# GuanLab/seekmer

Hardware: AMD Instinct MI355X
Metric: paired reads/sec mapped+quantified (higher is better)
Workload: dtype u64+f64; 1 GPU; configs[1]: synthetic ~190k-tx index (stand-in for ENSEMBL GRCh38 cDNA), 10000000 2x100bp synthetic pairs per GPU, map+classes+EM to the reference stop rule; transcripts=190402, kmer_slots=134217728, units_per_gpu=10000000, read_len=100, paired=True, classes=851072, class_map_rows=4208693, parallelism=reads sharded x1, RCCL all-reduce f64[T] per EM step, rccl_ranks=0

## Files before the change

### include/seekmer_hip.h

```cpp
#ifndef SEEKMER_HIP_H
#define SEEKMER_HIP_H

#include <stddef.h>
#include <stdint.h>

#ifdef __cplusplus
extern "C" {
#endif

#define SKM_OK 0
#define SKM_ERR_ARG 1
#define SKM_ERR_HIP 2
#define SKM_ERR_NO_DEVICE 3
#define SKM_ERR_COLLISION 4
#define SKM_ERR_STATE 5
#define SKM_ERR_IO 6
#define SKM_ERR_UNDEFINED 7
#define SKM_ERR_COMM 8

#define SKM_KMER_SIZE 25
#define SKM_MAX_FRAGMENT_LENGTH 2000


const char *skm_last_error(void);
// ... 26 lines not shown
int skm_mapper_create(skm_index *index, skm_mapper **out);
int skm_mapper_destroy(skm_mapper *mapper);

int skm_mapper_map_batch(skm_mapper *mapper, const char *bases,
                         const int64_t *offsets, int64_t n_units, int paired);
int skm_mapper_map_batch_async(skm_mapper *mapper, const char *bases,
                               const int64_t *offsets, int64_t n_units, int paired,
                               int64_t first_unit);
int skm_mapper_map_batch_uniform_async(skm_mapper *mapper, const char *bases, int32_t read_len,
                                       int64_t n_units, int paired, int64_t first_unit);
int skm_mapper_sync(skm_mapper *mapper);
int skm_mapper_expect_units(skm_mapper *mapper, int64_t n_units);
#define SKM_PACKED_CUT (-1)
typedef struct skm_packed_reads {
    int32_t stream;
    int32_t code_words;
    int64_t first_read;
    int64_t n_reads;
    int64_t read_stride;
    int64_t uniform_len;
    const uint64_t *codes;
    const uint32_t *lengths;
    int64_t n_exceptions;
    const uint32_t *exception_reads;
    const uint32_t *exception_masks;
    const char *names;
    const int64_t *name_offsets;
} skm_packed_reads;
int skm_mapper_push_packed(skm_mapper *mapper, const skm_packed_reads *piece, int paired);
typedef int (*skm_packed_source)(void *context, skm_packed_reads *piece);
int skm_mapper_map_packed_source(skm_mapper *mapper, skm_packed_source next, void *context,
                                 int paired, int64_t *n_pieces);
int skm_mapper_map_batch_device(skm_mapper *mapper, const void *d_bases,
                                const void *d_offsets, int64_t n_units,
                                int paired, int32_t max_read_len);
int skm_mapper_last_batch(skm_mapper *mapper, int32_t *begin, int32_t *end,
                          int32_t *anchor_entry, int32_t *anchor_offset,
                          int32_t *counts, int32_t *entries,
                          int64_t cap_entries, int64_t *n_entries);
int skm_mapper_keep_spans(skm_mapper *mapper, int enable);
#define SKM_STRAND_NONE 0
#define SKM_STRAND_FR 1
#define SKM_STRAND_RF 2
int skm_mapper_set_strand(skm_mapper *mapper, int mode);
int skm_mapper_set_length_weights(skm_mapper *mapper, const double *p);
int skm_mapper_set_bias(skm_mapper *mapper, int enable);
int skm_mapper_bias_observed(skm_mapper *mapper, int64_t out[4096]);
int skm_mapper_summary(skm_mapper *mapper, int64_t summary[4]);
int skm_mapper_export(skm_mapper *mapper, int64_t *class_offsets,
                      int32_t *class_targets, int64_t *class_counts,
                      int64_t *first_seen, int64_t *fld);
int skm_mapper_merge(skm_mapper *mapper, int64_t n_classes,
                     const int64_t *class_offsets, const int32_t *class_targets,
                     const int64_t *class_counts, const int64_t *first_seen,
                     int64_t unaligned, const int64_t *fld);
typedef struct skm_device_table {
    int32_t device;
    int64_t n_classes, n_ids;
    const int64_t *class_start;
    const int64_t *class_len;
    const double *class_count;
    const uint64_t *first_seen;
    const int32_t *ids;
    int64_t unaligned, units, first_seen_bound;
    const uint64_t *fld;
} skm_device_table;
int skm_mapper_device_table(skm_mapper *mapper, skm_device_table *out);
int skm_mapper_merge_device(skm_mapper *mapper, const skm_device_table *table);
int skm_mapper_clear(skm_mapper *mapper);
int skm_mapper_reset(skm_mapper *mapper);
int skm_mapper_timing(skm_mapper *mapper, double stats[8]);
int skm_mapper_set_stats(skm_mapper *mapper, int enable);
int skm_mapper_access_stats(skm_mapper *mapper, int64_t out[48]);

typedef struct skm_sample_set skm_sample_set;
int skm_sample_set_create(skm_index *index, int paired, skm_sample_set **out);
int skm_sample_set_destroy(skm_sample_set *set);
int skm_sample_set_set_strand(skm_sample_set *set, int mode);
int skm_sample_set_set_length_weights(skm_sample_set *set, const double *p);
int skm_sample_set_add_packed(skm_sample_set *set, int64_t sample, int64_t first_unit,
                              const skm_packed_reads *mate1, const skm_packed_reads *mate2);
int skm_sample_set_add_batch(skm_sample_set *set, int64_t sample, int64_t first_unit,
                             const char *bases, const int64_t *offsets, int64_t n_units);
int skm_sample_set_sync(skm_sample_set *set);
int skm_sample_set_summary(skm_sample_set *set, int64_t cap_samples, int64_t *n_samples,
                           int64_t *summary);
int skm_sample_set_export(skm_sample_set *set, int64_t *sample_class_offsets,
                          int64_t *class_offsets, int32_t *class_targets, int64_t *class_counts,
                          int64_t *first_seen);
int skm_sample_set_histogram(skm_sample_set *set, int64_t *fld);
int skm_sample_set_keep_histograms(skm_sample_set *set, int enable);
int skm_sample_set_histograms(skm_sample_set *set, int64_t cap_samples, int64_t *fld);
int skm_sample_set_plan(int64_t n_segments, const int32_t *sample, const int64_t *n_units,
                        int64_t max_units, int64_t cap_entries, int64_t *n_entries,
                        int64_t *entry_global, int64_t *entry_local, int32_t *entry_sample);
int skm_sample_set_split(int64_t n_entries, const int64_t *entry_global, const int64_t *entry_local,
                         const int32_t *entry_sample, int64_t n_samples, int64_t n_classes,
                         const int64_t *first_seen, int32_t *class_sample, int64_t *class_local,
                         int64_t *order, int64_t *sample_class_offsets);

int skm_effective_lengths(int device, const int64_t *fld, const double *lengths,
                          int64_t n_tx, double *out);
int skm_effective_lengths_many(int device, int64_t n, const int64_t *fld, const double *lengths,
                               int64_t n_tx, double *out);
int skm_effective_lengths_weights(int device, int64_t n, const double *p, const double *lengths,
                                  int64_t n_tx, double *out);

int skm_bias_correct(skm_index *index, int strand, const int64_t *observed, const double *tpm, const double *eff,
                     int64_t n_tx, double *expected_out, double *b_out, double *eff_out);

typedef struct skm_quant skm_quant;
int skm_quant_create(int device, int64_t n_tx, int64_t n_classes,
                     const int64_t *class_offsets, const int32_t *class_targets,
                     const double *class_counts, skm_quant **out);
int skm_quant_create_from_mapper(skm_mapper *mapper, int64_t n_tx, skm_quant **out);
int skm_quant_destroy(skm_quant *quant);
int skm_quant_em(skm_quant *quant, double *x, const double *l, double rel_tol,
                 double x_floor, int64_t max_iters, int64_t fixed_iters,
                 int64_t *iters);
int skm_quant_bootstrap(skm_quant *quant, int64_t n_boot, uint64_t seed,
                        const double *x0, const double *l, double rel_tol,
                        double x_floor, int64_t max_iters, double *out,
                        int64_t *counts_out, int64_t *iters_out);
int skm_quant_bootstrap_tpm(skm_quant *quant, int64_t n_boot, uint64_t seed,
                            const double *x0, const double *l, double rel_tol,
                            double x_floor, int64_t max_iters, double *out,
                            int64_t *iters_out);
int skm_quant_bootstrap_share_tpm(skm_quant *quant, int64_t n_boot, int64_t first, int64_t step,
                                  uint64_t seed, const double *x0, const double *l, double rel_tol,
                                  double x_floor, int64_t max_iters, double *out,
                                  int64_t *iters_out);
int skm_quant_set_counts(skm_quant *quant, const double *class_counts);
int skm_quant_em_many(skm_quant *quant, int64_t n_sets, const double *counts, const double *x0,
                      const double *l, double rel_tol, double x_floor, int tpm, double *out,
                      int64_t *iters_out);
int skm_quant_em_blend(skm_quant *quant, int64_t n_cells, const int32_t *class_cell,
                       const double *weight, const double *cell_total, const double *x0,
                       const double *l, double rel_tol, double x_floor, int tpm, double *out,
                       int64_t *iters_out, double *counts_out);
int skm_quant_em_tables(int device, int64_t n_tx, int64_t n_tables, const int64_t *table_class_offsets,
                        const int64_t *class_offsets, const int32_t *class_targets,
                        const double *class_counts, const double *x0, const double *l, double rel_tol,
                        double x_floor, int64_t max_iters, int tpm, double *out, int64_t *iters);
int skm_set_quant_groups(int64_t n_tables, int64_t n_tx, const int64_t *table_classes,
                         const int64_t *table_ids, int64_t max_slots, int64_t *n_groups,
                         int64_t *group_first);
int skm_sample_set_quantify(skm_sample_set *set, const double *lengths, int64_t n_tx, double rel_tol,
                            double x_floor, int64_t max_iters, int64_t cap_samples,
                            int64_t *n_samples, double *tpm, double *effective_lengths,
                            int64_t *iters);
int skm_quant_components(skm_quant *quant, int64_t info[8], int32_t *tx_label, int32_t *tx_tile,
                         int32_t *class_tile);
int skm_quant_timing(skm_quant *quant, double timing[4]);

typedef struct skm_comm skm_comm;
int skm_comm_unique_id(void *id128);
int skm_comm_create(int device, const void *id128, int rank, int world, skm_comm **out);
int skm_comm_count(skm_comm *comm, int *count);
int skm_comm_destroy(skm_comm *comm);
int skm_mapper_exchange_tables(skm_mapper *send, int send_to, skm_mapper *recv, int recv_from, skm_comm *comm);
int skm_quant_set_comm(skm_quant *quant, skm_comm *comm);

int skm_quant_infer(skm_mapper *mapper, skm_comm *comm, const double *lengths, int64_t n_tx,
                    double rel_tol, double x_floor, int64_t max_iters,
                    double *tpm, double *effective_lengths, int64_t *iters);


typedef struct skm_built skm_built;
int skm_build_index(const char *pool, const int64_t *seq_offsets, int64_t n_seqs,
                    int n_threads, skm_built **out);
int skm_built_sizes(const skm_built *b, int64_t sizes[4]);
int skm_built_copy(const skm_built *b, void *kmers, void *contigs,
                   char *sequences, void *targets);
int skm_built_free(skm_built *b);

typedef struct skm_fastq skm_fastq;
int skm_fastq_open(const char *const *paths, int n_paths, int paired,
                   int64_t batch_units, skm_fastq **out);
int skm_fastq_set_allocator(skm_fastq *reader, void *(*alloc)(size_t), void (*release)(void *));
int skm_fastq_set_parallel(skm_fastq *reader, int n_threads, int *enabled);
int skm_fastq_set_shard(skm_fastq *reader, int rank, int world);
int skm_fastq_batch_index(const skm_fastq *reader, int64_t *index);
int skm_fastq_batch_read_length(const skm_fastq *reader, int64_t *read_len);
int skm_fastq_next(skm_fastq *reader, int64_t *n_units, const char **bases,
                   const int64_t **offsets, const char **names,
                   const int64_t **name_offsets);
typedef struct skm_fastq_slab skm_fastq_slab;
int skm_fastq_detach(skm_fastq *reader, skm_fastq_slab **slab);
int skm_fastq_recycle(skm_fastq *reader, skm_fastq_slab *slab);
int skm_fastq_close(skm_fastq *reader);

int skm_fastq_cache_bytes(int64_t bytes);
int skm_fastq_wait_unmapped(void);
typedef struct skm_fastq_prefault skm_fastq_prefault;
int skm_fastq_prefault_start(const char *const *paths, int n_paths, int n_threads, skm_fastq_prefault **out);
int skm_fastq_prefault_finish(skm_fastq_prefault *handle);

typedef struct skm_fastq_packed skm_fastq_packed;
int skm_fastq_packed_open(const char *const *paths, int n_paths, int paired, int n_threads,
                          int64_t chunk_bytes, int want_names, skm_fastq_packed **out);
int skm_fastq_packed_open_ranges(const char *const *paths, int n_paths, int paired, int n_threads,
                                 int64_t chunk_bytes, int want_names, const int64_t *begin,
                                 const int64_t *end, int64_t first_unit, skm_fastq_packed **out);
int skm_fastq_count_newlines(const char *path, int64_t chunk_bytes, int64_t first_chunk,
                             int64_t chunk_step, int n_threads, int64_t *counts, int64_t n_chunks,
                             int *last_line_open);
int skm_fastq_locate_line(const char *path, int64_t chunk_bytes, const int64_t *counts,
                          int64_t n_chunks, int64_t line, int64_t *byte_offset);
int skm_fastq_packed_set_allocator(skm_fastq_packed *reader, void *(*alloc)(size_t),
                                   void (*release)(void *));
int skm_fastq_packed_next(void *reader, skm_packed_reads *piece);
int skm_fastq_packed_stats(const skm_fastq_packed *reader, int64_t stats[8]);
int skm_fastq_packed_estimate(const skm_fastq_packed *reader, int64_t *units);
int skm_fastq_packed_close(skm_fastq_packed *reader);
int skm_pack_reads(const char *bases, const int64_t *offsets, int64_t n_reads, int32_t code_words,
                   uint64_t *codes, uint32_t *lengths, uint32_t *exception_reads,
                   uint32_t *exception_masks, int64_t cap_exceptions, int64_t *n_exceptions,
                   int variant);
int skm_pack_set_variant(int variant);

int skm_synth_transcriptome(uint64_t seed, int64_t n_genes, int64_t *n_tx,
                            char **pool, int64_t **offsets);
int skm_synth_free(void *p);
int skm_synth_reads(uint64_t seed, const char *pool, const int64_t *tx_offsets,
                    int64_t n_tx, int64_t first_unit, int64_t n_units,
                    int read_len, int paired, int n_threads, char *bases);

int skm_synth_fastq_write(const char *bases, int64_t n_units, int read_len, int paired,
                          int64_t first_unit, const char *path1, const char *path2,
                          int n_threads);

#ifdef __cplusplus
}
#endif
#endif
```

### seekmer_amd/_native.py

```python
import ctypes
import os

_HERE = os.path.dirname(os.path.abspath(__file__))
HIP_LIB_PATH = os.environ.get('SKM_HIP_LIB') or os.path.join(_HERE, 'libseekmer_hip.so')
HOST_LIB_PATH = os.path.join(_HERE, 'libseekmer_host.so')

SKM_OK = 0
SKM_ERR_ARG = 1
SKM_ERR_HIP = 2
SKM_ERR_NO_DEVICE = 3
SKM_ERR_COLLISION = 4
SKM_ERR_STATE = 5
SKM_ERR_IO = 6
SKM_ERR_UNDEFINED = 7
SKM_ERR_COMM = 8

SKM_STRAND_NONE = 0
SKM_STRAND_FR = 1
SKM_STRAND_RF = 2

c_void_pp = ctypes.POINTER(ctypes.c_void_p)
c_i64p = ctypes.POINTER(ctypes.c_int64)
c_i32p = ctypes.POINTER(ctypes.c_int32)
c_f64p = ctypes.POINTER(ctypes.c_double)
c_i64 = ctypes.c_int64
c_u32p = ctypes.POINTER(ctypes.c_uint32)
c_u64p = ctypes.POINTER(ctypes.c_uint64)


class PackedReads(ctypes.Structure):
    _fields_ = [('stream', ctypes.c_int32), ('code_words', ctypes.c_int32), ('first_read', ctypes.c_int64),
                ('n_reads', ctypes.c_int64), ('read_stride', ctypes.c_int64), ('uniform_len', ctypes.c_int64),
                ('codes', ctypes.c_void_p), ('lengths', ctypes.c_void_p), ('n_exceptions', ctypes.c_int64),
                ('exception_reads', ctypes.c_void_p), ('exception_masks', ctypes.c_void_p),
                ('names', ctypes.c_void_p), ('name_offsets', ctypes.c_void_p)]


class DeviceTable(ctypes.Structure):
    _fields_ = [('device', ctypes.c_int32), ('n_classes', ctypes.c_int64), ('n_ids', ctypes.c_int64),
                ('class_start', ctypes.c_void_p), ('class_len', ctypes.c_void_p), ('class_count', ctypes.c_void_p),
                ('first_seen', ctypes.c_void_p), ('ids', ctypes.c_void_p), ('unaligned', ctypes.c_int64),
                ('units', ctypes.c_int64), ('first_seen_bound', ctypes.c_int64), ('fld', ctypes.c_void_p)]


HIP_SYMBOLS = {
    'skm_last_error': (ctypes.c_char_p, []),
    'skm_device_count': (ctypes.c_int, [ctypes.POINTER(ctypes.c_int)]),
    'skm_device_malloc': (ctypes.c_int, [ctypes.c_int, c_i64, c_void_pp]),
    'skm_device_free': (ctypes.c_int, [ctypes.c_int, ctypes.c_void_p]),
    'skm_device_upload': (ctypes.c_int, [ctypes.c_int, ctypes.c_void_p, ctypes.c_void_p, c_i64]),
    'skm_device_download': (ctypes.c_int, [ctypes.c_int, ctypes.c_void_p, ctypes.c_void_p, c_i64]),
    'skm_device_synchronize': (ctypes.c_int, [ctypes.c_int]),
    'skm_device_gather_ceiling': (ctypes.c_int, [ctypes.c_int, c_i64, ctypes.c_int, ctypes.c_int,
                                                 ctypes.c_int, c_f64p]),
    'skm_pinned_alloc': (ctypes.c_void_p, [ctypes.c_size_t]),
    'skm_pinned_free': (None, [ctypes.c_void_p]),
    'skm_pinned_set_device': (ctypes.c_int, [ctypes.c_int]),
    'skm_index_create': (ctypes.c_int, [ctypes.c_void_p, c_i64, ctypes.c_void_p, c_i64,
                                        ctypes.c_void_p, c_i64, ctypes.c_void_p, c_i64,
                                        ctypes.c_int, c_void_pp]),
    'skm_index_destroy': (ctypes.c_int, [ctypes.c_void_p]),
    'skm_index_info': (ctypes.c_int, [ctypes.c_void_p, c_i64p]),
    'skm_index_layout': (ctypes.c_int, [ctypes.c_void_p, c_i64p]),
    'skm_index_build_transcripts': (ctypes.c_int, [ctypes.c_void_p, c_f64p, c_i64]),
    'skm_index_transcript_bases': (ctypes.c_int, [ctypes.c_void_p, ctypes.c_void_p, ctypes.c_void_p]),
    'skm_mapper_create': (ctypes.c_int, [ctypes.c_void_p, c_void_pp]),
    'skm_mapper_destroy': (ctypes.c_int, [ctypes.c_void_p]),
    'skm_mapper_map_batch': (ctypes.c_int, [ctypes.c_void_p, ctypes.c_void_p, c_i64p, c_i64,
                                            ctypes.c_int]),
    'skm_mapper_map_batch_async': (ctypes.c_int, [ctypes.c_void_p, ctypes.c_void_p, c_i64p, c_i64,
                                                  ctypes.c_int, c_i64]),
    'skm_mapper_map_batch_uniform_async': (ctypes.c_int, [ctypes.c_void_p, ctypes.c_void_p, ctypes.c_int32, c_i64,
                                                          ctypes.c_int, c_i64]),
    'skm_mapper_sync': (ctypes.c_int, [ctypes.c_void_p]),
    'skm_mapper_expect_units': (ctypes.c_int, [ctypes.c_void_p, c_i64]),
    'skm_mapper_push_packed': (ctypes.c_int, [ctypes.c_void_p, ctypes.POINTER(PackedReads), ctypes.c_int]),
    'skm_mapper_map_packed_source': (ctypes.c_int, [ctypes.c_void_p, ctypes.c_void_p, ctypes.c_void_p, ctypes.c_int,
                                                    c_i64p]),
    'skm_mapper_map_batch_device': (ctypes.c_int, [ctypes.c_void_p, ctypes.c_void_p,
                                                   ctypes.c_void_p, c_i64, ctypes.c_int,
                                                   ctypes.c_int32]),
    'skm_mapper_last_batch': (ctypes.c_int, [ctypes.c_void_p, c_i32p, c_i32p, c_i32p, c_i32p,
                                             c_i32p, c_i32p, c_i64, c_i64p]),
    'skm_mapper_keep_spans': (ctypes.c_int, [ctypes.c_void_p, ctypes.c_int]),
    'skm_mapper_set_strand': (ctypes.c_int, [ctypes.c_void_p, ctypes.c_int]),
    'skm_mapper_set_length_weights': (ctypes.c_int, [ctypes.c_void_p, c_f64p]),
    'skm_mapper_set_bias': (ctypes.c_int, [ctypes.c_void_p, ctypes.c_int]),
    'skm_mapper_bias_observed': (ctypes.c_int, [ctypes.c_void_p, c_i64p]),
    'skm_mapper_summary': (ctypes.c_int, [ctypes.c_void_p, c_i64p]),
    'skm_mapper_export': (ctypes.c_int, [ctypes.c_void_p, c_i64p, c_i32p, c_i64p, c_i64p, c_i64p]),
    'skm_mapper_merge': (ctypes.c_int, [ctypes.c_void_p, c_i64, c_i64p, c_i32p, c_i64p, c_i64p,
                                        c_i64, c_i64p]),
    'skm_mapper_device_table': (ctypes.c_int, [ctypes.c_void_p, ctypes.POINTER(DeviceTable)]),
    'skm_mapper_merge_device': (ctypes.c_int, [ctypes.c_void_p, ctypes.POINTER(DeviceTable)]),
    'skm_mapper_clear': (ctypes.c_int, [ctypes.c_void_p]),
    'skm_mapper_reset': (ctypes.c_int, [ctypes.c_void_p]),
    'skm_mapper_timing': (ctypes.c_int, [ctypes.c_void_p, c_f64p]),
    'skm_mapper_set_stats': (ctypes.c_int, [ctypes.c_void_p, ctypes.c_int]),
    'skm_mapper_access_stats': (ctypes.c_int, [ctypes.c_void_p, c_i64p]),
    'skm_effective_lengths': (ctypes.c_int, [ctypes.c_int, c_i64p, c_f64p, c_i64, c_f64p]),
    'skm_effective_lengths_many': (ctypes.c_int, [ctypes.c_int, c_i64, c_i64p, c_f64p, c_i64, c_f64p]),
    'skm_effective_lengths_weights': (ctypes.c_int, [ctypes.c_int, c_i64, c_f64p, c_f64p, c_i64, c_f64p]),
    'skm_bias_correct': (ctypes.c_int, [ctypes.c_void_p, ctypes.c_int, c_i64p, c_f64p, c_f64p, c_i64, c_f64p, c_f64p, c_f64p]),
    'skm_sample_set_create': (ctypes.c_int, [ctypes.c_void_p, ctypes.c_int, c_void_pp]),
    'skm_sample_set_destroy': (ctypes.c_int, [ctypes.c_void_p]),
    'skm_sample_set_set_strand': (ctypes.c_int, [ctypes.c_void_p, ctypes.c_int]),
    'skm_sample_set_set_length_weights': (ctypes.c_int, [ctypes.c_void_p, c_f64p]),
    'skm_sample_set_add_packed': (ctypes.c_int, [ctypes.c_void_p, c_i64, c_i64, ctypes.POINTER(PackedReads),
                                                 ctypes.POINTER(PackedReads)]),
    'skm_sample_set_add_batch': (ctypes.c_int, [ctypes.c_void_p, c_i64, c_i64, ctypes.c_void_p, c_i64p, c_i64]),
    'skm_sample_set_sync': (ctypes.c_int, [ctypes.c_void_p]),
    'skm_sample_set_summary': (ctypes.c_int, [ctypes.c_void_p, c_i64, c_i64p, c_i64p]),
    'skm_sample_set_export': (ctypes.c_int, [ctypes.c_void_p, c_i64p, c_i64p, c_i32p, c_i64p, c_i64p]),
    'skm_sample_set_histogram': (ctypes.c_int, [ctypes.c_void_p, c_i64p]),
    'skm_sample_set_keep_histograms': (ctypes.c_int, [ctypes.c_void_p, ctypes.c_int]),
    'skm_sample_set_histograms': (ctypes.c_int, [ctypes.c_void_p, c_i64, c_i64p]),
    'skm_sample_set_plan': (ctypes.c_int, [c_i64, c_i32p, c_i64p, c_i64, c_i64, c_i64p, c_i64p, c_i64p, c_i32p]),
    'skm_sample_set_split': (ctypes.c_int, [c_i64, c_i64p, c_i64p, c_i32p, c_i64, c_i64, c_i64p, c_i32p, c_i64p, c_i64p,
                                            c_i64p]),
    'skm_quant_create': (ctypes.c_int, [ctypes.c_int, c_i64, c_i64, c_i64p, c_i32p, c_f64p,
                                        c_void_pp]),
    'skm_quant_create_from_mapper': (ctypes.c_int, [ctypes.c_void_p, c_i64, c_void_pp]),
    'skm_quant_destroy': (ctypes.c_int, [ctypes.c_void_p]),
    'skm_quant_em': (ctypes.c_int, [ctypes.c_void_p, c_f64p, c_f64p, ctypes.c_double,
                                    ctypes.c_double, c_i64, c_i64, c_i64p]),
    'skm_quant_bootstrap': (ctypes.c_int, [ctypes.c_void_p, c_i64, ctypes.c_uint64, c_f64p,
                                           c_f64p, ctypes.c_double, ctypes.c_double, c_i64,
                                           c_f64p, c_i64p, c_i64p]),
    'skm_quant_bootstrap_tpm': (ctypes.c_int, [ctypes.c_void_p, c_i64, ctypes.c_uint64, c_f64p,
                                               c_f64p, ctypes.c_double, ctypes.c_double, c_i64,
                                               c_f64p, c_i64p]),
    'skm_quant_bootstrap_share_tpm': (ctypes.c_int, [ctypes.c_void_p, c_i64, c_i64, c_i64, ctypes.c_uint64, c_f64p,
                                                     c_f64p, ctypes.c_double, ctypes.c_double, c_i64,
                                                     c_f64p, c_i64p]),
    'skm_quant_set_counts': (ctypes.c_int, [ctypes.c_void_p, c_f64p]),
    'skm_quant_em_many': (ctypes.c_int, [ctypes.c_void_p, c_i64, c_f64p, c_f64p, c_f64p, ctypes.c_double,
                                         ctypes.c_double, ctypes.c_int, c_f64p, c_i64p]),
    'skm_quant_em_blend': (ctypes.c_int, [ctypes.c_void_p, c_i64, c_i32p, c_f64p, c_f64p, c_f64p, c_f64p,
                                          ctypes.c_double, ctypes.c_double, ctypes.c_int, c_f64p, c_i64p, c_f64p]),
    'skm_quant_em_tables': (ctypes.c_int, [ctypes.c_int, c_i64, c_i64, c_i64p, c_i64p, c_i32p, c_f64p, c_f64p, c_f64p,
                                           ctypes.c_double, ctypes.c_double, c_i64, ctypes.c_int, c_f64p, c_i64p]),
    'skm_set_quant_groups': (ctypes.c_int, [c_i64, c_i64, c_i64p, c_i64p, c_i64, c_i64p, c_i64p]),
    'skm_sample_set_quantify': (ctypes.c_int, [ctypes.c_void_p, c_f64p, c_i64, ctypes.c_double, ctypes.c_double, c_i64,
                                               c_i64, c_i64p, c_f64p, c_f64p, c_i64p]),
    'skm_quant_timing': (ctypes.c_int, [ctypes.c_void_p, c_f64p]),
    'skm_quant_components': (ctypes.c_int, [ctypes.c_void_p, c_i64p, c_i32p, c_i32p, c_i32p]),
    'skm_comm_unique_id': (ctypes.c_int, [ctypes.c_void_p]),
    'skm_comm_create': (ctypes.c_int, [ctypes.c_int, ctypes.c_void_p, ctypes.c_int, ctypes.c_int,
                                       c_void_pp]),
    'skm_comm_count': (ctypes.c_int, [ctypes.c_void_p, ctypes.POINTER(ctypes.c_int)]),
    'skm_comm_destroy': (ctypes.c_int, [ctypes.c_void_p]),
    'skm_mapper_exchange_tables': (ctypes.c_int, [ctypes.c_void_p, ctypes.c_int, ctypes.c_void_p, ctypes.c_int,
                                                  ctypes.c_void_p]),
    'skm_quant_set_comm': (ctypes.c_int, [ctypes.c_void_p, ctypes.c_void_p]),
    'skm_quant_infer': (ctypes.c_int, [ctypes.c_void_p, ctypes.c_void_p, c_f64p, c_i64, ctypes.c_double,
                                       ctypes.c_double, c_i64, c_f64p, c_f64p, c_i64p]),
}

HOST_SYMBOLS = {
    'skm_build_index': (ctypes.c_int, [ctypes.c_void_p, c_i64p, c_i64, ctypes.c_int, c_void_pp]),
    'skm_built_sizes': (ctypes.c_int, [ctypes.c_void_p, c_i64p]),
    'skm_built_copy': (ctypes.c_int, [ctypes.c_void_p, ctypes.c_void_p, ctypes.c_void_p,
                                      ctypes.c_void_p, ctypes.c_void_p]),
    'skm_built_free': (ctypes.c_int, [ctypes.c_void_p]),
    'skm_fastq_open': (ctypes.c_int, [ctypes.POINTER(ctypes.c_char_p), ctypes.c_int, ctypes.c_int,
                                      c_i64, c_void_pp]),
    'skm_fastq_set_allocator': (ctypes.c_int, [ctypes.c_void_p, ctypes.c_void_p, ctypes.c_void_p]),
    'skm_fastq_set_parallel': (ctypes.c_int, [ctypes.c_void_p, ctypes.c_int, ctypes.POINTER(ctypes.c_int)]),
    'skm_fastq_set_shard': (ctypes.c_int, [ctypes.c_void_p, ctypes.c_int, ctypes.c_int]),
    'skm_fastq_batch_read_length': (ctypes.c_int, [ctypes.c_void_p, c_i64p]),
    'skm_fastq_batch_index': (ctypes.c_int, [ctypes.c_void_p, c_i64p]),
    'skm_fastq_next': (ctypes.c_int, [ctypes.c_void_p, c_i64p, c_void_pp, c_void_pp, c_void_pp,
                                      c_void_pp]),
    'skm_fastq_detach': (ctypes.c_int, [ctypes.c_void_p, c_void_pp]),
    'skm_fastq_recycle': (ctypes.c_int, [ctypes.c_void_p, ctypes.c_void_p]),
    'skm_fastq_close': (ctypes.c_int, [ctypes.c_void_p]),
    'skm_fastq_cache_bytes': (ctypes.c_int, [c_i64]),
    'skm_fastq_wait_unmapped': (ctypes.c_int, []),
    'skm_fastq_packed_open': (ctypes.c_int, [ctypes.POINTER(ctypes.c_char_p), ctypes.c_int, ctypes.c_int,
                                             ctypes.c_int, c_i64, ctypes.c_int, c_void_pp]),
    'skm_fastq_packed_open_ranges': (ctypes.c_int, [ctypes.POINTER(ctypes.c_char_p), ctypes.c_int, ctypes.c_int,
                                                    ctypes.c_int, c_i64, ctypes.c_int, c_i64p, c_i64p, c_i64, c_void_pp]),
    'skm_fastq_count_newlines': (ctypes.c_int, [ctypes.c_char_p, c_i64, c_i64, c_i64, ctypes.c_int, c_i64p, c_i64,
                                                ctypes.POINTER(ctypes.c_int)]),
    'skm_fastq_locate_line': (ctypes.c_int, [ctypes.c_char_p, c_i64, c_i64p, c_i64, c_i64, c_i64p]),
    'skm_fastq_packed_set_allocator': (ctypes.c_int, [ctypes.c_void_p, ctypes.c_void_p, ctypes.c_void_p]),
    'skm_fastq_packed_next': (ctypes.c_int, [ctypes.c_void_p, ctypes.POINTER(PackedReads)]),
    'skm_fastq_packed_stats': (ctypes.c_int, [ctypes.c_void_p, c_i64p]),
    'skm_fastq_prefault_start': (ctypes.c_int, [ctypes.POINTER(ctypes.c_char_p), ctypes.c_int, ctypes.c_int, c_void_pp]),
    'skm_fastq_prefault_finish': (ctypes.c_int, [ctypes.c_void_p]),
    'skm_fastq_packed_estimate': (ctypes.c_int, [ctypes.c_void_p, c_i64p]),
    'skm_fastq_packed_close': (ctypes.c_int, [ctypes.c_void_p]),
    'skm_pack_reads': (ctypes.c_int, [ctypes.c_void_p, c_i64p, c_i64, ctypes.c_int32, ctypes.c_void_p,
                                      ctypes.c_void_p, ctypes.c_void_p, ctypes.c_void_p, c_i64, c_i64p,
                                      ctypes.c_int]),
    'skm_pack_set_variant': (ctypes.c_int, [ctypes.c_int]),
    'skm_synth_transcriptome': (ctypes.c_int, [ctypes.c_uint64, c_i64, c_i64p, c_void_pp,
                                               c_void_pp]),
    'skm_synth_free': (ctypes.c_int, [ctypes.c_void_p]),
    'skm_synth_fastq_write': (ctypes.c_int, [ctypes.c_void_p, c_i64, ctypes.c_int, ctypes.c_int, c_i64,
                                             ctypes.c_char_p, ctypes.c_char_p, ctypes.c_int]),
    'skm_synth_reads': (ctypes.c_int, [ctypes.c_uint64, ctypes.c_void_p, c_i64p, c_i64, c_i64,
                                       c_i64, ctypes.c_int, ctypes.c_int, ctypes.c_int,
                                       ctypes.c_void_p]),
}


class NativeError(RuntimeError):

    def __init__(self, code, message):
        super().__init__('seekmer_hip error %d: %s' % (code, message))
        self.code = code


def _bind(path, symbols):
    if not os.path.exists(path):
        raise ImportError(
            '%s is missing: build it with `python -c "import __graft_entry__ as g; g.build()"` '
            'or `make -C seekmer_amd/csrc` (there is no CPU fallback)' % path)
    lib = ctypes.CDLL(path, mode=ctypes.RTLD_GLOBAL)
    for name, (restype, argtypes) in symbols.items():
        fn = getattr(lib, name)
        fn.restype = restype
        fn.argtypes = argtypes
    return lib


_hip = None
_host = None


def hip():
    global _hip
    if _hip is None:
        _hip = _bind(HIP_LIB_PATH, HIP_SYMBOLS)
    return _hip


def host():
    global _host
    if _host is None:
        _host = _bind(HOST_LIB_PATH, HOST_SYMBOLS)
    return _host


def check(code):
    if code == SKM_OK:
        return
    message = hip().skm_last_error().decode(errors='replace')
    if code == SKM_ERR_ARG:
        raise ValueError(message)
    raise NativeError(code, message)


def check_host(code, what):
    if code == SKM_OK:
        return
    if code == SKM_ERR_ARG:
        raise ValueError('%s: bad argument' % what)
    if code == SKM_ERR_IO:
        raise OSError('%s: cannot open input' % what)
    raise NativeError(code, what)


def device_count():
    n = ctypes.c_int(0)
    code = hip().skm_device_count(ctypes.byref(n))
    if code == SKM_ERR_NO_DEVICE:
        return 0
    check(code)
    return n.value


def ptr(array, ctype):
    return array.ctypes.data_as(ctype)
```

### seekmer_amd/csrc/skm_abi.hip

```cpp
#include "../../include/seekmer_hip.h"
#include "skm_kernels.h"
#include "skm_pool.h"
#include "skm_bias.h"

#include <dlfcn.h>
#include <algorithm>
#include <cmath>
#include <cstdarg>
#include <cstdio>
#include <cstdlib>
#include <cstring>
#include <chrono>
#include <condition_variable>
#include <atomic>
#include <deque>
#include <functional>
#include <map>
#include <memory>
#include <unordered_map>
#include <mutex>
#include <thread>
#include <numeric>
#include <string>
#include <utility>
// ... 2783 lines not shown
    std::copy(log.local.begin(), log.local.end(), entry_local);
    std::copy(log.sample.begin(), log.sample.end(), entry_sample);
    return SKM_OK;
}

extern "C" int skm_sample_set_split(int64_t n_entries, const int64_t *entry_global, const int64_t *entry_local,
                                    const int32_t *entry_sample, int64_t n_samples, int64_t n_classes,
                                    const int64_t *first_seen, int32_t *class_sample, int64_t *class_local, int64_t *order,
                                    int64_t *sample_class_offsets)
{
    if (n_entries < 0 || n_samples < 0 || n_classes < 0 || !sample_class_offsets
            || (n_entries && (!entry_global || !entry_local || !entry_sample))
            || (n_classes && (!first_seen || !class_sample || !class_local || !order)))
        return fail(SKM_ERR_ARG, "bad argument");
    if (n_classes && (n_entries == 0 || entry_global[0] != 0)) return fail(SKM_ERR_ARG, "the log does not start at unit 0");
    for (int64_t i = 0; i < n_entries; ++i)
        if (entry_sample[i] < 0 || entry_sample[i] >= n_samples || (i && entry_global[i] <= entry_global[i - 1]))
            return fail(SKM_ERR_ARG, "bad log entry %lld", (long long)i);
    for (int64_t k = 0; k < n_classes; ++k) {
        if (first_seen[k] < 0) return fail(SKM_ERR_ARG, "negative first-seen unit");
        const int64_t e = segment_find(entry_global, n_entries, first_seen[k]);
        class_sample[k] = entry_sample[e];
        class_local[k] = entry_local[e] + (first_seen[k] - entry_global[e]);
    }
    set_split_order(n_samples, n_classes, class_sample, class_local, order, sample_class_offsets);
    return SKM_OK;
}

extern "C" int skm_effective_lengths(int device, const int64_t *fld, const double *lengths,
                                     int64_t n_tx, double *out)
{
    if (!fld || !lengths || !out || n_tx < 0) return fail(SKM_ERR_ARG, "bad argument");
    int n_dev = 0;
    SKM_TRY(skm_device_count(&n_dev));
    if (device < 0 || device >= n_dev) return fail(SKM_ERR_ARG, "device %d out of range", device);
    SKM_TRY(set_device(device));
    if (n_tx == 0) return SKM_OK;
    DBuf<unsigned long long> d_fld; DBuf<double> d_len, d_out;
    auto drain = on_exit([&]() { (void)hipStreamSynchronize(nullptr); });
    SKM_TRY(d_fld.ensure(MAX_FRAGMENT_LENGTH)); SKM_TRY(d_len.ensure(n_tx)); SKM_TRY(d_out.ensure(n_tx));
    HIP_TRY(hipMemcpy(d_fld.p, fld, MAX_FRAGMENT_LENGTH * 8, hipMemcpyHostToDevice));
    HIP_TRY(hipMemcpy(d_len.p, lengths, n_tx * 8, hipMemcpyHostToDevice));
    launch_effective_lengths(d_fld.p, d_len.p, n_tx, d_out.p, nullptr);
    HIP_TRY(hipGetLastError());
    HIP_TRY(hipMemcpy(out, d_out.p, n_tx * 8, hipMemcpyDeviceToHost));
    drain.dismiss();
    return SKM_OK;
}

namespace {

int64_t effective_lengths_group(int64_t n, int64_t n_tx)
{
    int64_t group = std::min<int64_t>((int64_t)(1LL << 25) / n_tx, (int64_t)(1LL << 25) / MAX_FRAGMENT_LENGTH);
    if (const char *v = getenv("SKM_EFF_MANY_GROUP"))
        if (atoll(v) > 0) group = std::min<int64_t>(group, atoll(v));
    return std::max<int64_t>(1, std::min(group, n));
}

}

extern "C" int skm_effective_lengths_many(int device, int64_t n, const int64_t *fld, const double *lengths,
                                          int64_t n_tx, double *out)
{
    if (n < 0 || n_tx < 0 || (n && (!fld || (n_tx && (!lengths || !out))))) return fail(SKM_ERR_ARG, "bad argument");
    int n_dev = 0;
    SKM_TRY(skm_device_count(&n_dev));
    if (device < 0 || device >= n_dev) return fail(SKM_ERR_ARG, "device %d out of range", device);
    SKM_TRY(set_device(device));
    if (n == 0 || n_tx == 0) return SKM_OK;
    const int64_t group = effective_lengths_group(n, n_tx);
    DBuf<unsigned long long> d_fld; DBuf<double> d_len, d_out;
    auto drain = on_exit([&]() { (void)hipStreamSynchronize(nullptr); });
    SKM_TRY(d_fld.ensure((size_t)group * MAX_FRAGMENT_LENGTH)); SKM_TRY(d_len.ensure(n_tx)); SKM_TRY(d_out.ensure((size_t)(group * n_tx)));
    HIP_TRY(hipMemcpy(d_len.p, lengths, n_tx * 8, hipMemcpyHostToDevice));
    for (int64_t first = 0; first < n; first += group) {
        const int64_t here = std::min(group, n - first);
        HIP_TRY(hipMemcpy(d_fld.p, fld + first * MAX_FRAGMENT_LENGTH, (size_t)here * MAX_FRAGMENT_LENGTH * 8, hipMemcpyHostToDevice));
        launch_effective_lengths_many(d_fld.p, here, d_len.p, n_tx, d_out.p, nullptr);
        HIP_TRY(hipGetLastError());
        HIP_TRY(hipMemcpy(out + first * n_tx, d_out.p, (size_t)(here * n_tx) * 8, hipMemcpyDeviceToHost));
    }
    drain.dismiss();
    return SKM_OK;
}

extern "C" int skm_effective_lengths_weights(int device, int64_t n, const double *p, const double *lengths,
                                             int64_t n_tx, double *out)
{
    if (n < 0 || n_tx < 0 || !p || !lengths || !out) return fail(SKM_ERR_ARG, "bad argument");
    if (!length_weights_valid(p, n * MAX_FRAGMENT_LENGTH))
        return fail(SKM_ERR_ARG, "a fragment-length weight is negative or not finite");
    int n_dev = 0;
    SKM_TRY(skm_device_count(&n_dev));
    if (device < 0 || device >= n_dev) return fail(SKM_ERR_ARG, "device %d out of range", device);
    SKM_TRY(set_device(device));
    if (n == 0 || n_tx == 0) return SKM_OK;
    const int64_t group = effective_lengths_group(n, n_tx);
    DBuf<double> d_p, d_len, d_out;
    auto drain = on_exit([&]() { (void)hipStreamSynchronize(nullptr); });
    SKM_TRY(d_p.ensure((size_t)group * MAX_FRAGMENT_LENGTH)); SKM_TRY(d_len.ensure(n_tx)); SKM_TRY(d_out.ensure((size_t)(group * n_tx)));
    HIP_TRY(hipMemcpy(d_len.p, lengths, n_tx * 8, hipMemcpyHostToDevice));
    for (int64_t first = 0; first < n; first += group) {
        const int64_t here = std::min(group, n - first);
        HIP_TRY(hipMemcpy(d_p.p, p + first * MAX_FRAGMENT_LENGTH, (size_t)here * MAX_FRAGMENT_LENGTH * 8, hipMemcpyHostToDevice));
        launch_effective_lengths_weights(d_p.p, here, d_len.p, n_tx, d_out.p, nullptr);
        HIP_TRY(hipGetLastError());
        HIP_TRY(hipMemcpy(out + first * n_tx, d_out.p, (size_t)(here * n_tx) * 8, hipMemcpyDeviceToHost));
    }
    drain.dismiss();
    return SKM_OK;
}

namespace {

bool em_components_enabled() { return getenv("SKM_EM_NO_COMPONENTS") == nullptr; }
bool em_tiles_possible(bool several_ranks)
{
    static const bool unfused = getenv("SKM_EM_UNFUSED") != nullptr;
    return !several_ranks && !unfused && em_components_enabled();
}

int quant_alloc(skm_quant *q, int device, int64_t n_tx, int64_t n_classes, int64_t n_ids, bool several_ranks = false)
{
    STALE_CHECK("quant_alloc entry");
    q->device = device;
    q->n_tx = n_tx;
    q->n_classes = n_classes;
    q->n_ids = n_ids;
    HIP_TRY(pool_stream_acquire(q->stream.out()));
    for (auto &e : q->ev) HIP_TRY(pool_event_acquire(e.out(), true));
    for (auto &e : q->chunk_ev) HIP_TRY(pool_event_acquire(e.out(), false));
    HIP_TRY(pool_pinned_acquire((void **)q->pinned.out()));
    const size_t C = (size_t)std::max<int64_t>(n_classes, 1), M = (size_t)std::max<int64_t>(n_ids, 1);
    const size_t T = (size_t)std::max<int64_t>(n_tx, 1);
    const size_t R = (size_t)quant_rows_upper_bound(n_tx, n_ids);
    SKM_TRY(q->cls_offset.ensure(C + 1));
    SKM_TRY(q->cls_count.ensure(C));
    SKM_TRY(q->inner.ensure(C));
    SKM_TRY(q->ids.ensure(M));
    SKM_TRY(q->perm.ensure(C));
    SKM_TRY(q->tx_cls.ensure(M));
    SKM_TRY(q->tx_row.ensure(T + 1));
    SKM_TRY(q->row_start.ensure(R + 1));
    SKM_TRY(q->row_tx.ensure(R));
    SKM_TRY(q->row_sum.ensure(R));
    SKM_TRY(q->eff_len.ensure(T));
    SKM_TRY(q->x0.ensure(T));
    SKM_TRY(q->x1.ensure(T));
    SKM_TRY(q->acc.ensure(T));
    SKM_TRY(q->ctl.ensure(16));
    SKM_TRY(q->part_max.ensure(EM_FINAL_BLOCKS));
    SKM_TRY(q->part_flags.ensure(EM_FINAL_BLOCKS));
    SKM_TRY(q->arrivals.ensure(T));
    HIP_TRY(hipMemsetAsync(q->arrivals.p, 0, T * sizeof(unsigned int), q->stream));
    if (em_tiles_possible(several_ranks)) {
        auto &t = q->tiles;
        SKM_TRY(t.tile_tx.ensure(T + 2)); SKM_TRY(t.tile_cls.ensure(T + 2));
        SKM_TRY(t.cls_pair.ensure(C + 1)); SKM_TRY(t.tx_pair.ensure(T + 1));
        SKM_TRY(t.tx_list.ensure(T)); SKM_TRY(t.cls_list.ensure(C));
        SKM_TRY(t.tx_label.ensure(T)); SKM_TRY(t.tx_tile.ensure(T)); SKM_TRY(t.cls_tile.ensure(C));
        SKM_TRY(t.cls_tx.ensure(M)); SKM_TRY(t.tx_cls.ensure(M));
    }
    STALE_CHECK("quant_alloc exit");
    return SKM_OK;
}

QuantBuild quant_build_view(skm_quant *q)
{
    QuantBuild b{};
    b.n_tx = q->n_tx;
    b.n_classes = q->n_classes;
    b.n_ids = q->n_ids;
    b.cls_offset = q->cls_offset.p;
    b.ids = q->ids.p;
    b.cls_count = q->cls_count.p;
    b.tx_cls = q->tx_cls.p;
    b.tx_row = q->tx_row.p;
    b.row_start = q->row_start.p;
    b.row_tx = q->row_tx.p;
    b.n_rows_cap = (int64_t)q->row_tx.cap;
    if (q->tiles.tile_tx.p) {
        auto &t = q->tiles;
        b.tile_tx = t.tile_tx.p; b.tile_cls = t.tile_cls.p;
        b.tx_list = t.tx_list.p; b.cls_list = t.cls_list.p;
        b.cls_pair = t.cls_pair.p; b.tx_pair = t.tx_pair.p;
        b.tile_cls_tx = t.cls_tx.p; b.tile_tx_cls = t.tx_cls.p;
        b.tx_label = t.tx_label.p; b.tx_tile = t.tx_tile.p; b.cls_tile = t.cls_tile.p;
    }
    return b;
}

int quant_finish_setup(skm_quant *q, const ClassTable *table, int64_t units_seen = -1)
{
    STALE_CHECK("quant_finish_setup");
    QuantBuild b = quant_build_view(q);
    b.first_seen_bound = units_seen > 0 ? units_seen : 0;
    const int64_t rows = quant_setup(table, b, q->perm.p, q->stream);
    if (rows < 0) return fail(SKM_ERR_HIP, "building the class views failed (%lld): %s", (long long)rows, quant_setup_failure());
    q->n_rows = rows;
    if (b.tile_tx) {
        q->tiles.built = true;
        q->tiles.n_tiles = b.tile_info[0];
        q->tiles.n_oversize = b.tile_info[1];
        if (q->tiles.n_tiles > 0) {
            SKM_TRY(q->tiles.step_max.ensure((size_t)(EM_CHUNK_MAX * q->tiles.n_tiles)));
            SKM_TRY(q->tiles.step_flags.ensure((size_t)(EM_CHUNK_MAX * q->tiles.n_tiles)));
            SKM_TRY(q->tiles.snap.ensure((size_t)EM_CHUNK_MAX * (size_t)q->n_tx));
        }
        if (q->tiles.n_oversize > 0 && q->tiles.n_tiles > 0) {
            auto &r = q->tiles.residual;
            int64_t counts[3] = {0, 0, 0};
            if (quant_residual_count(b, counts, q->stream))
                return fail(SKM_ERR_HIP, "sizing the residual EM problem failed: %s", quant_setup_failure());
            r.n_classes = counts[0]; r.n_ids = counts[1]; r.n_rows = counts[2];
            SKM_TRY(r.cls_offset.ensure((size_t)r.n_classes + 1)); SKM_TRY(r.ids.ensure((size_t)std::max<int64_t>(r.n_ids, 1)));
            SKM_TRY(r.cls_src.ensure((size_t)std::max<int64_t>(r.n_classes, 1)));
            SKM_TRY(r.row_start.ensure((size_t)r.n_rows + 1)); SKM_TRY(r.row_tx.ensure((size_t)std::max<int64_t>(r.n_rows, 1)));
            SKM_TRY(r.tx_cls.ensure((size_t)std::max<int64_t>(r.n_ids, 1))); SKM_TRY(r.tx_row.ensure((size_t)q->n_tx + 1));
            SKM_TRY(r.cls_count.ensure((size_t)std::max<int64_t>(r.n_classes, 1)));
            SKM_TRY(r.inner.ensure((size_t)std::max<int64_t>(r.n_classes, 1)));
            SKM_TRY(r.row_sum.ensure((size_t)std::max<int64_t>(r.n_rows, 1)));
            QuantResidual out{};
            out.n_classes = r.n_classes; out.n_ids = r.n_ids; out.n_rows = r.n_rows;
            out.cls_offset = r.cls_offset.p; out.ids = r.ids.p; out.cls_src = r.cls_src.p;
            out.row_start = r.row_start.p; out.row_tx = r.row_tx.p; out.tx_cls = r.tx_cls.p; out.tx_row = r.tx_row.p;
            if (quant_residual_build(b, out, q->stream))
                return fail(SKM_ERR_HIP, "building the residual EM problem failed: %s", quant_setup_failure());
            r.built = true;
        }
    }
    return SKM_OK;
}

struct Rccl {
    void *lib = nullptr;
    int (*GetUniqueId)(void *) = nullptr;
    int (*AllReduce)(const void *, void *, size_t, int, int, void *, hipStream_t) = nullptr;
    int (*CommDestroy)(void *) = nullptr;
    int (*CommCount)(void *, int *) = nullptr;
    const char *(*GetErrorString)(int) = nullptr;
    int (*Send)(const void *, size_t, int, int, void *, hipStream_t) = nullptr;
    int (*Recv)(void *, size_t, int, int, void *, hipStream_t) = nullptr;
    int (*GroupStart)() = nullptr;
    int (*GroupEnd)() = nullptr;
};
struct UniqueId { char internal[128]; };
typedef int (*comm_init_fn)(void **, int, UniqueId, int);
Rccl g_rccl;
comm_init_fn g_comm_init = nullptr;

int load_rccl()
{
    if (g_rccl.lib) return SKM_OK;
    void *lib = dlopen("librccl.so", RTLD_NOW | RTLD_GLOBAL);
    if (!lib) lib = dlopen("librccl.so.1", RTLD_NOW | RTLD_GLOBAL);
    if (!lib) lib = dlopen("/opt/rocm/lib/librccl.so", RTLD_NOW | RTLD_GLOBAL);
    if (!lib) return fail(SKM_ERR_COMM, "cannot load librccl.so: %s", dlerror());
    g_rccl.GetUniqueId = (int (*)(void *))dlsym(lib, "ncclGetUniqueId");
    g_comm_init = (comm_init_fn)dlsym(lib, "ncclCommInitRank");
    g_rccl.AllReduce = (int (*)(const void *, void *, size_t, int, int, void *, hipStream_t))dlsym(lib, "ncclAllReduce");
    g_rccl.CommDestroy = (int (*)(void *))dlsym(lib, "ncclCommDestroy");
    g_rccl.CommCount = (int (*)(void *, int *))dlsym(lib, "ncclCommCount");
    g_rccl.GetErrorString = (const char *(*)(int))dlsym(lib, "ncclGetErrorString");
    g_rccl.Send = (int (*)(const void *, size_t, int, int, void *, hipStream_t))dlsym(lib, "ncclSend");
    g_rccl.Recv = (int (*)(void *, size_t, int, int, void *, hipStream_t))dlsym(lib, "ncclRecv");
    g_rccl.GroupStart = (int (*)())dlsym(lib, "ncclGroupStart");
    g_rccl.GroupEnd = (int (*)())dlsym(lib, "ncclGroupEnd");
    if (!g_rccl.GetUniqueId || !g_comm_init || !g_rccl.AllReduce || !g_rccl.CommDestroy)
        return fail(SKM_ERR_COMM, "librccl.so lacks a required symbol");
    g_rccl.lib = lib;
    return SKM_OK;
}

constexpr int NCCL_FLOAT64 = 8, NCCL_UINT64 = 5, NCCL_INT32 = 2, NCCL_SUM = 0;

#define NCCL_TRY(call)                                                                   \
    do {                                                                                 \
        int r_ = (call);                                                                 \
        if (r_ != 0)                                                                     \
            return fail(SKM_ERR_COMM, "%s failed: %s", #call,                            \
                        g_rccl.GetErrorString ? g_rccl.GetErrorString(r_) : "?");        \
    } while (0)

EmProblem em_problem(skm_quant *q, double rel_tol, double x_floor, int64_t max_iters,
                     int64_t fixed_iters)
{
    EmProblem p{};
    p.n_tx = q->n_tx;
    p.n_classes = q->n_classes;
    p.n_rows = q->n_rows;
    p.cls_offset = q->cls_offset.p;
    p.ids = q->ids.p;
    p.cls_count = q->cls_count.p;
    p.inner = q->inner.p;
    p.row_start = q->row_start.p;
    p.row_tx = q->row_tx.p;
    p.tx_cls = q->tx_cls.p;
    p.tx_row = q->tx_row.p;
    p.row_sum = q->row_sum.p;
    p.eff_len = q->eff_len.p;
    p.x[0] = q->x0.p;
    p.x[1] = q->x1.p;
    p.acc = q->acc.p;
    p.n_total = q->n_total;
    p.rel_tol = rel_tol;
    p.x_floor = x_floor;
    p.ctl = q->ctl.p;
    p.part_max = q->part_max.p;
    p.part_flags = q->part_flags.p;
    p.max_iters = max_iters;
    p.fixed_iters = fixed_iters;
    static const bool unfused = getenv("SKM_EM_UNFUSED") != nullptr;
    p.fused = q->comm || unfused ? 0 : 1;
    p.arrivals = q->arrivals.p;
    return p;
}

bool em_uses_tiles(const skm_quant *q)
{
    return em_tiles_possible(q->comm != nullptr) && q->tiles.built && q->tiles.n_tiles > 0 &&
           (q->tiles.n_oversize == 0 || q->tiles.residual.built);
}
// ... 21 lines not shown
    auto &t = q->tiles;
    EmTiles tl{};
    tl.n_tiles = t.n_tiles;
    tl.tile_tx = t.tile_tx.p; tl.tile_cls = t.tile_cls.p;
    tl.tx_list = t.tx_list.p; tl.cls_list = t.cls_list.p;
    tl.cls_pair = t.cls_pair.p; tl.tx_pair = t.tx_pair.p;
    tl.cls_tx = t.cls_tx.p; tl.tx_cls = t.tx_cls.p;
    tl.step_max = t.step_max.p; tl.step_flags = t.step_flags.p;
    tl.snap = t.snap.p;
    const bool mixed = t.n_oversize > 0;
    EmProblem pr = p;
    if (mixed) {
        auto &r = t.residual;
        pr.n_classes = r.n_classes; pr.n_rows = r.n_rows;
        pr.cls_offset = r.cls_offset.p; pr.ids = r.ids.p; pr.cls_count = r.cls_count.p; pr.inner = r.inner.p;
        pr.row_start = r.row_start.p; pr.row_tx = r.row_tx.p; pr.tx_cls = r.tx_cls.p; pr.tx_row = r.tx_row.p;
        pr.row_sum = r.row_sum.p;
        pr.fused = 1;
        pr.extra_max = t.step_max.p; pr.extra_flags = t.step_flags.p; pr.n_extra = t.n_tiles;
        launch_permute_f64(q->cls_count.p, r.cls_src.p, r.n_classes, r.cls_count.p, false, q->stream);
    }
    int64_t queued = 0;
    auto enqueue_chunk = [&](int slot) -> int {
        launch_em_local_chunk(p, tl, queued == 0 ? q->x0.p : t.snap.p + (chunk - 1) * q->n_tx, (int)chunk, queued * chunk, q->stream);
        if (mixed) {
            pr.extra_first = queued * chunk;
            for (int64_t i = 0, k = queued * chunk; i < chunk; ++i, ++k) {
                launch_em_inner(pr, (int)(k & 1), i > 0, k, q->stream);
                launch_em_rows_finalize(pr, (int)(k & 1), q->stream);
            }
            launch_em_decide(pr, (queued + 1) * chunk, q->stream);
            q->launches += 2 * chunk + 2;
        } else {
            launch_em_local_decide(p, tl, queued * chunk, (int)chunk, q->stream);
            q->launches += 2;
        }
        ++queued;
        HIP_TRY(hipGetLastError());
        HIP_TRY(hipMemcpyAsync(q->pinned + 8 * slot, q->ctl.p, 8 * sizeof(unsigned long long),
                               hipMemcpyDeviceToHost, q->stream));
        return SKM_OK;
    };
    unsigned long long ctl[8] = {0};
    SKM_TRY(em_run_chunks_ahead(q, ctl, enqueue_chunk, em_ctl_done));
    if (ctl[CTL_TILE_FAULT]) {
        HIP_TRY(hipStreamSynchronize(q->stream));
        return fail(SKM_ERR_STATE, "a component tile exceeds the tile capacity: the class views of this handle are damaged");
    }
    const int64_t steps = (int64_t)ctl[CTL_ITERS];
    HIP_TRY(hipEventRecord(q->ev[1], q->stream));
    HIP_TRY(hipEventSynchronize(q->ev[1]));
    float ms = 0;
    HIP_TRY(hipEventElapsedTime(&ms, q->ev[0], q->ev[1]));
    q->t_em_ns += ms * 1e6;
    q->iters_total += (double)steps;
    if (iters_out) *iters_out = steps;
    if (ctl[CTL_UNDEFINED]) return fail(SKM_ERR_UNDEFINED, "no abundance above x_floor: numpy raises on max() of an empty selection");
    return SKM_OK;
}

int em_run(skm_quant *q, double rel_tol, double x_floor, int64_t max_iters, int64_t fixed_iters,
           int64_t *iters_out, int64_t chunk_steps = 16)
{
    double n_total = q->n_total;
    if (q->comm && !q->n_total_reduced) {
        HIP_TRY(hipMemcpyAsync(q->acc.p, &n_total, 8, hipMemcpyHostToDevice, q->stream));
        NCCL_TRY(g_rccl.AllReduce(q->acc.p, q->acc.p, 1, NCCL_FLOAT64, NCCL_SUM, q->comm, q->stream));
        HIP_TRY(hipMemcpyAsync(&n_total, q->acc.p, 8, hipMemcpyDeviceToHost, q->stream));
        HIP_TRY(hipStreamSynchronize(q->stream));
    }
    EmProblem p = em_problem(q, rel_tol, x_floor, max_iters, fixed_iters);
    p.n_total = n_total;
    HIP_TRY(hipMemsetAsync(q->ctl.p, 0, 16 * 8, q->stream));
    int64_t k = 0;
    const int64_t chunk = fixed_iters > 0 ? std::min<int64_t>(fixed_iters, chunk_steps) : chunk_steps;
    HIP_TRY(hipEventRecord(q->ev[0], q->stream));
    if (em_uses_tiles(q) && chunk <= EM_CHUNK_MAX) return em_run_tiles(q, p, chunk, iters_out);
    static const bool unfused_rows = getenv("SKM_EM_UNFUSED") != nullptr;
    auto enqueue_chunk = [&](int slot) -> int {
        for (int64_t i = 0; i < chunk; ++i, ++k) {
            launch_em_inner(p, (int)(k & 1), i > 0, k, q->stream);
            if (q->comm) {
                if (unfused_rows) {
                    launch_em_rows(p, (int)(k & 1), q->stream);
                    launch_em_rows_to_acc(p, q->stream);
                } else {
                    launch_em_rows_acc(p, (int)(k & 1), q->stream);
                }
                NCCL_TRY(g_rccl.AllReduce(q->acc.p, q->acc.p, (size_t)q->n_tx, NCCL_FLOAT64, NCCL_SUM,
                                          q->comm, q->stream));
                launch_em_finalize(p, (int)(k & 1), true, q->stream);
            } else if (p.fused) {
                launch_em_rows_finalize(p, (int)(k & 1), q->stream);
            } else {
                launch_em_rows(p, (int)(k & 1), q->stream);
                launch_em_finalize(p, (int)(k & 1), false, q->stream);
            }
            q->launches += q->comm ? (unfused_rows ? 4 : 3) : (p.fused ? 2 : 3);
        }
        launch_em_decide(p, k, q->stream);
        q->launches += 1;
        HIP_TRY(hipGetLastError());
        HIP_TRY(hipMemcpyAsync(q->pinned + 8 * slot, q->ctl.p, 8 * sizeof(unsigned long long),
                               hipMemcpyDeviceToHost, q->stream));
        return SKM_OK;
    };
    unsigned long long ctl[8] = {0};
    SKM_TRY(em_run_chunks_ahead(q, ctl, enqueue_chunk, em_ctl_done));
    HIP_TRY(hipStreamSynchronize(q->stream));
    HIP_TRY(hipEventRecord(q->ev[1], q->stream));
    HIP_TRY(hipEventSynchronize(q->ev[1]));
    float ms = 0;
    HIP_TRY(hipEventElapsedTime(&ms, q->ev[0], q->ev[1]));
    q->t_em_ns += ms * 1e6;
    q->iters_total += (double)ctl[CTL_ITERS];
    if (iters_out) *iters_out = (int64_t)ctl[CTL_ITERS];
    if (ctl[CTL_UNDEFINED]) return fail(SKM_ERR_UNDEFINED, "no abundance above x_floor: numpy raises on max() of an empty selection");
    return SKM_OK;
}

}

namespace {

double np_pairwise_host(const double *a, int64_t n)
{
    if (n < 8) {
        double r = 0.0;
        for (int64_t i = 0; i < n; ++i) r += a[i];
        return r;
    }
    if (n <= 128) {
        double r[8];
        for (int j = 0; j < 8; ++j) r[j] = a[j];
        int64_t i = 8;
        for (; i < n - (n % 8); i += 8)
            for (int j = 0; j < 8; ++j) r[j] += a[i + j];
        double res = ((r[0] + r[1]) + (r[2] + r[3])) + ((r[4] + r[5]) + (r[6] + r[7]));
        for (; i < n; ++i) res += a[i];
        return res;
    }
    int64_t n2 = n / 2;
    n2 -= n2 % 8;
    return np_pairwise_host(a, n2) + np_pairwise_host(a + n2, n - n2);
}

double np_sum_host(const double *a, int64_t n)
{
    double acc = 0.0;
    for (int64_t i = 0; i < n; i += 8192) acc += np_pairwise_host(a + i, std::min<int64_t>(8192, n - i));
    return acc;
}

}

extern "C" int skm_quant_create(int device, int64_t n_tx, int64_t n_classes,
                                const int64_t *class_offsets, const int32_t *class_targets,
                                const double *class_counts, skm_quant **out)
{
    if (!out || n_tx <= 0 || n_classes < 0) return fail(SKM_ERR_ARG, "bad argument");
    if (n_classes && (!class_offsets || !class_targets || !class_counts))
        return fail(SKM_ERR_ARG, "NULL class arrays");
    int n_dev = 0;
    SKM_TRY(skm_device_count(&n_dev));
    if (device < 0 || device >= n_dev) return fail(SKM_ERR_ARG, "device %d out of range", device);
    const int64_t M = n_classes ? class_offsets[n_classes] - class_offsets[0] : 0;
    for (int64_t c = 0; c < n_classes; ++c)
        if (class_offsets[c + 1] < class_offsets[c]) return fail(SKM_ERR_ARG, "class offsets are not monotone");
    const double total = np_sum_host(class_counts, n_classes);
    for (int64_t j = 0; j < M; ++j) {
        const int32_t t = class_targets[class_offsets[0] + j];
        if (t < 0 || t >= n_tx) return fail(SKM_ERR_ARG, "class target %d outside [0, n_tx)", t);
    }
    SKM_TRY(set_device(device));
    std::unique_ptr<skm_quant> q(new skm_quant());
    SKM_TRY(quant_alloc(q.get(), device, n_tx, n_classes, M));
    std::vector<int64_t> rebased(n_classes + 1, 0);
    for (int64_t c = 0; c <= n_classes && n_classes; ++c) rebased[c] = class_offsets[c] - class_offsets[0];
    HIP_TRY(hipMemcpy(q->cls_offset.p, rebased.data(), (n_classes + 1) * 8, hipMemcpyHostToDevice));
    if (n_classes) {
        HIP_TRY(hipMemcpy(q->cls_count.p, class_counts, n_classes * 8, hipMemcpyHostToDevice));
        if (M) HIP_TRY(hipMemcpy(q->ids.p, class_targets + class_offsets[0], M * 4, hipMemcpyHostToDevice));
    }
    q->n_total = total;
    SKM_TRY(quant_finish_setup(q.get(), nullptr));
    *out = q.release();
    return SKM_OK;
}

extern "C" int skm_quant_create_from_mapper(skm_mapper *m, int64_t n_tx, skm_quant **out)
{
    if (!m || !out || n_tx <= 0) return fail(SKM_ERR_ARG, "bad argument");
    SKM_TRY(wait_jobs(m, 0, false));
    std::lock_guard<std::mutex> lock(m->mu);
    SKM_TRY(set_device(m->ix->device));
    const int64_t C = m->host_classes, M = m->host_arena_used;
    std::unique_ptr<skm_quant> q(new skm_quant());
    SKM_TRY(quant_alloc(q.get(), m->ix->device, n_tx, C, M));
    unsigned long long ctr[4];
    HIP_TRY(hipMemcpy(ctr, m->counters.p, sizeof(ctr), hipMemcpyDeviceToHost));
    q->n_total = (double)(ctr[CTR_UNITS] - ctr[CTR_UNALIGNED]);
    SKM_TRY(quant_finish_setup(q.get(), &m->t, m->first_seen_bound));
    *out = q.release();
    return SKM_OK;
}

extern "C" int skm_quant_infer(skm_mapper *m, skm_comm *comm, const double *lengths, int64_t n_tx,
                               double rel_tol, double x_floor, int64_t max_iters,
                               double *tpm, double *effective_lengths, int64_t *iters)
{
    if (!m || !lengths || n_tx <= 0) return fail(SKM_ERR_ARG, "bad argument");
    SKM_TRY(wait_jobs(m, 0, false));
    std::lock_guard<std::mutex> lock(m->mu);
    if (comm && comm->device != m->ix->device)
        return fail(SKM_ERR_ARG, "communicator and mapper live on different GPUs");
    SKM_TRY(set_device(m->ix->device));
    const int64_t C = m->host_classes, M = m->host_arena_used;
    static const bool trace = getenv("SKM_TRACE_INFER") != nullptr;
    auto t_last = std::chrono::steady_clock::now();
    auto lap = [&](const char *what) {
        if (!trace) return;
        const auto now = std::chrono::steady_clock::now();
        fprintf(stderr, "[skm_quant_infer] %-12s %8.1f us\n", what,
                std::chrono::duration<double, std::micro>(now - t_last).count());
        t_last = now;
    };
    DBuf<unsigned long long> fld;
    DBuf<double> sums;
    std::unique_ptr<skm_quant> q(new skm_quant());
    SKM_TRY(quant_alloc(q.get(), m->ix->device, n_tx, C, M, comm != nullptr));
    if (comm) { q->comm = comm->comm; q->rank = comm->rank; q->world = comm->world; }
    lap("alloc");
    const int64_t n_blocks = (n_tx + 8191) / 8192;
    SKM_TRY(fld.ensure(MAX_FRAGMENT_LENGTH + 1));
    SKM_TRY(sums.ensure(n_blocks + 2));
    double *const total = sums.p + n_blocks;
    unsigned long long ctr[4] = {0, 0, m->host_unaligned, m->host_units};
    if (!m->host_totals_valid)
        HIP_TRY(hipMemcpy(ctr, m->counters.p, sizeof(ctr), hipMemcpyDeviceToHost));
    unsigned long long aligned = ctr[CTR_UNITS] - ctr[CTR_UNALIGNED];
    HIP_TRY(hipMemcpyAsync(fld.p, m->counters.p + CTR_FLD, MAX_FRAGMENT_LENGTH * 8,
                           hipMemcpyDeviceToDevice, q->stream));
    if (q->comm) {
        q->pinned[32] = aligned;
        HIP_TRY(hipMemcpyAsync(fld.p + MAX_FRAGMENT_LENGTH, q->pinned + 32, 8, hipMemcpyHostToDevice, q->stream));
        NCCL_TRY(g_rccl.AllReduce(fld.p, fld.p, MAX_FRAGMENT_LENGTH + 1, NCCL_UINT64, NCCL_SUM, q->comm,
                                  q->stream));
        HIP_TRY(hipMemcpyAsync(q->pinned + 32, fld.p + MAX_FRAGMENT_LENGTH, 8, hipMemcpyDeviceToHost, q->stream));
        HIP_TRY(hipStreamSynchronize(q->stream));
        aligned = q->pinned[32];
        q->n_total_reduced = true;
        if (const char *v = getenv("SKM_TEST_ALIGNED_GLOBAL")) aligned += strtoull(v, nullptr, 10);
    }
    q->n_total = (double)aligned;
    HIP_TRY(hipMemcpyAsync(q->x1.p, lengths, n_tx * 8, hipMemcpyHostToDevice, q->stream));
    if (m->use_length_weights)
        launch_effective_lengths_weights(m->length_weights.p, 1, q->x1.p, n_tx, q->eff_len.p, q->stream);
    else
        launch_effective_lengths(fld.p, q->x1.p, n_tx, q->eff_len.p, q->stream);
    if (q->comm ? aligned == 0 : C == 0) {
        if (effective_lengths)
            HIP_TRY(hipMemcpyAsync(effective_lengths, q->eff_len.p, n_tx * 8, hipMemcpyDeviceToHost, q->stream));
        HIP_TRY(hipStreamSynchronize(q->stream));
        if (tpm) memset(tpm, 0, (size_t)n_tx * 8);
        if (iters) *iters = 0;
        return SKM_OK;
    }
    launch_reciprocal(q->eff_len.p, n_tx, q->x0.p, q->stream);
    launch_np_sum(q->x0.p, n_tx, 1.0, sums.p, total, q->stream);
    launch_divide(q->x0.p, n_tx, total, false, 0.0, q->stream);
    lap("start vector");
    SKM_TRY(quant_finish_setup(q.get(), &m->t, m->first_seen_bound));
    lap("setup");
    if (trace) fprintf(stderr, "[skm_quant_infer] %lld classes, %lld transcripts, %lld rows\n", (long long)C, (long long)n_tx,
                       (long long)q->n_rows);
    int64_t it = 0;
    SKM_TRY(em_run(q.get(), rel_tol, x_floor, max_iters, 0, &it));
    lap("em");
    m->t_em_ns += q->t_em_ns;
    m->em_iters += (double)it;
    double *const x = (it & 1) ? q->x1.p : q->x0.p;
    launch_np_sum(x, n_tx, 1000000.0, sums.p, total, q->stream);
    launch_divide(x, n_tx, total + 1, true, 0.001, q->stream);
    launch_np_sum(x, n_tx, 1000000.0, sums.p, total, q->stream);
    launch_divide(x, n_tx, total + 1, false, 0.0, q->stream);
    HIP_TRY(hipGetLastError());
    if (tpm) HIP_TRY(hipMemcpyAsync(tpm, x, n_tx * 8, hipMemcpyDeviceToHost, q->stream));
    if (effective_lengths)
        HIP_TRY(hipMemcpyAsync(effective_lengths, q->eff_len.p, n_tx * 8, hipMemcpyDeviceToHost, q->stream));
    HIP_TRY(hipStreamSynchronize(q->stream));
    lap("tpm");
    if (iters) *iters = it;
    q.reset();
    lap("destroy");
    return SKM_OK;
}

extern "C" int skm_quant_destroy(skm_quant *q)
{
    if (!q) return SKM_OK;
    STALE_CHECK("quant_destroy entry");
    delete q;
    STALE_CHECK("quant_destroy exit");
    return SKM_OK;
}

extern "C" int skm_quant_em(skm_quant *q, double *x, const double *l, double rel_tol, double x_floor,
                            int64_t max_iters, int64_t fixed_iters, int64_t *iters)
{
    if (!q || !x || !l) return fail(SKM_ERR_ARG, "NULL argument");
    std::lock_guard<std::mutex> lock(q->mu);
    SKM_TRY(set_device(q->device));
    HIP_TRY(hipMemcpyAsync(q->x0.p, x, q->n_tx * 8, hipMemcpyHostToDevice, q->stream));
    HIP_TRY(hipMemcpyAsync(q->eff_len.p, l, q->n_tx * 8, hipMemcpyHostToDevice, q->stream));
    int64_t it = 0;
    SKM_TRY(em_run(q, rel_tol, x_floor, max_iters, fixed_iters, &it));
    HIP_TRY(hipMemcpy(x, (it & 1) ? q->x1.p : q->x0.p, q->n_tx * 8, hipMemcpyDeviceToHost));
    if (iters) *iters = it;
    return SKM_OK;
}

extern "C" int skm_quant_components(skm_quant *q, int64_t info[8], int32_t *tx_label, int32_t *tx_tile,
                                    int32_t *class_tile)
{
    if (!q || !info) return fail(SKM_ERR_ARG, "NULL argument");
    std::lock_guard<std::mutex> lock(q->mu);
    SKM_TRY(set_device(q->device));
    const auto &t = q->tiles;
    info[0] = t.built ? 1 : 0;
    info[1] = t.n_tiles;
    info[2] = t.n_oversize;
    info[3] = em_uses_tiles(q) ? 1 : 0;
    info[4] = EM_TILE_PAIRS; info[5] = EM_TILE_CLASSES; info[6] = EM_TILE_TX; info[7] = 0;
    if (!t.built) {
        if (tx_label || tx_tile || class_tile) return fail(SKM_ERR_ARG, "no component tiles were built for this handle");
        return SKM_OK;
    }
    HIP_TRY(hipStreamSynchronize(q->stream));
    if (tx_label) HIP_TRY(hipMemcpy(tx_label, t.tx_label.p, q->n_tx * 4, hipMemcpyDeviceToHost));
    if (tx_tile) HIP_TRY(hipMemcpy(tx_tile, t.tx_tile.p, q->n_tx * 4, hipMemcpyDeviceToHost));
    if (class_tile && q->n_classes) {
        std::vector<int32_t> tile(q->n_classes), perm(q->n_classes);
        HIP_TRY(hipMemcpy(tile.data(), t.cls_tile.p, q->n_classes * 4, hipMemcpyDeviceToHost));
        HIP_TRY(hipMemcpy(perm.data(), q->perm.p, q->n_classes * 4, hipMemcpyDeviceToHost));
        for (int64_t k = 0; k < q->n_classes; ++k) class_tile[perm[k]] = tile[k];
    }
    return SKM_OK;
}

extern "C" int skm_quant_set_counts(skm_quant *q, const double *class_counts)
{
    if (!q || (!class_counts && q->n_classes)) return fail(SKM_ERR_ARG, "NULL argument");
    std::lock_guard<std::mutex> lock(q->mu);
    SKM_TRY(set_device(q->device));
    const double total = np_sum_host(class_counts, q->n_classes);
    if (q->n_classes) {
        SKM_TRY(q->cls_count_saved.ensure(q->n_classes));
        HIP_TRY(hipMemcpyAsync(q->cls_count_saved.p, class_counts, q->n_classes * 8, hipMemcpyHostToDevice, q->stream));
        launch_permute_f64(q->cls_count_saved.p, q->perm.p, q->n_classes, q->cls_count.p, false, q->stream);
        HIP_TRY(hipGetLastError());
        HIP_TRY(hipStreamSynchronize(q->stream));
    }
    q->n_total = total;
    return SKM_OK;
}

namespace {

template <class Fill>
int em_group_run(skm_quant *q, int64_t n_problems, Fill &&fill, bool batched, int64_t slot_cap, const double *x0,
                 const double *l, double rel_tol, double x_floor, int64_t max_iters, double *out, int64_t *iters_out,
                 bool tpm)
{
    const int64_t C = q->n_classes, T = q->n_tx;
    skm_quant::Batch &w = q->batch;
    const int64_t group = std::max<int64_t>(1, std::min<int64_t>(n_problems, (int64_t)(1LL << 28) / T));
    const int64_t by_counts = std::max<int64_t>(1, (int64_t)((1LL << 31) / (8 * std::max<int64_t>(C, 1))));
    int64_t slots = batched ? std::max<int64_t>(1, std::min(group, by_counts)) : 1;
    if (slot_cap > 0) slots = std::min(slots, slot_cap);
    SKM_TRY(q->cls_count_saved.ensure(C));
    SKM_TRY(q->x_start.ensure(T));
    SKM_TRY(q->boot_out.ensure((size_t)(slots * T)));
    SKM_TRY(w.totals.ensure((size_t)(2 * slots)));
    HIP_TRY(hipMemcpyAsync(q->cls_count_saved.p, q->cls_count.p, C * 8, hipMemcpyDeviceToDevice, q->stream));
    HIP_TRY(hipMemcpyAsync(q->eff_len.p, l, T * 8, hipMemcpyHostToDevice, q->stream));
    HIP_TRY(hipMemcpyAsync(q->x_start.p, x0, T * 8, hipMemcpyHostToDevice, q->stream));
    const double saved_total = q->n_total;
    int rc = SKM_OK;
    DBuf<double> sums;
    auto restore = on_exit([&]() {
        (void)hipMemcpyAsync(q->cls_count.p, q->cls_count_saved.p, C * 8, hipMemcpyDeviceToDevice, q->stream);
        (void)hipStreamSynchronize(q->stream);
        q->n_total = saved_total;
    });
    auto problem_checked = [&](int64_t b, int64_t *it_out, double *dst) -> int {
        SKM_TRY(fill(b, (int64_t)1, q->cls_count.p, w.totals.p));
        HIP_TRY(hipGetLastError());
        double total = 0.0;
        HIP_TRY(hipMemcpyAsync(&total, w.totals.p, 8, hipMemcpyDeviceToHost, q->stream));
        HIP_TRY(hipMemcpyAsync(q->x0.p, q->x_start.p, T * 8, hipMemcpyDeviceToDevice, q->stream));
        HIP_TRY(hipStreamSynchronize(q->stream));
        q->n_total = total;
        SKM_TRY(em_run(q, rel_tol, x_floor, max_iters, 0, it_out, 8));
        HIP_TRY(hipMemcpyAsync(dst, (*it_out & 1) ? q->x1.p : q->x0.p, T * 8, hipMemcpyDeviceToDevice, q->stream));
        if (iters_out) iters_out[b] = *it_out;
        return SKM_OK;
    };
    auto scale = [&](double *results, int64_t count) -> int {
        if (!tpm || count <= 0) return SKM_OK;
        const int64_t n_blocks = (T + 8191) / 8192;
        SKM_TRY(sums.ensure((size_t)(count * (n_blocks + 2))));
        double *const totals = sums.p + count * n_blocks;
        launch_np_sum_many(results, T, count, T, 1000000.0, sums.p, totals, q->stream);
        launch_divide_many(results, T, count, T, totals + 1, true, 0.001, q->stream);
        launch_np_sum_many(results, T, count, T, 1000000.0, sums.p, totals, q->stream);
        launch_divide_many(results, T, count, T, totals + 1, false, 0.0, q->stream);
        HIP_TRY(hipGetLastError());
        return SKM_OK;
    };
    auto send_home = [&](int64_t first, int64_t count) -> int {
        if (count <= 0) return SKM_OK;
        SKM_TRY(scale(q->boot_out.p, count));
        HIP_TRY(hipMemcpyAsync(out + first * T, q->boot_out.p, (size_t)count * T * 8, hipMemcpyDeviceToHost, q->stream));
        HIP_TRY(hipStreamSynchronize(q->stream));
        return SKM_OK;
    };
    if (!batched) {
        for (int64_t b = 0; b < n_problems; ++b) {
            int64_t it = 0;
            SKM_TRY(problem_checked(b, &it, q->boot_out.p));
            SKM_TRY(send_home(b, 1));
        }
        return rc;
    }
    SKM_TRY(w.cls_count.ensure((size_t)C * EM_BATCH)); SKM_TRY(w.inner.ensure((size_t)C * EM_BATCH));
    SKM_TRY(w.row_sum.ensure((size_t)std::max<int64_t>(q->n_rows, 1) * EM_BATCH));
    SKM_TRY(w.x0.ensure((size_t)T * EM_BATCH)); SKM_TRY(w.x1.ensure((size_t)T * EM_BATCH));
// ... 767 lines not shown
```

### seekmer_amd/csrc/skm_em.hip

```cpp
#include "skm_em_core.h"

namespace skm {

__device__ bool em_evaluate(const EmProblem &p, int n_parts, int64_t steps_done, bool publish);

struct EmWholeTable {
    const EmProblem &p;
    __device__ __forceinline__ int64_t cls_first() const { return 0; }
    __device__ __forceinline__ int64_t cls_end() const { return p.n_classes; }
    __device__ __forceinline__ int64_t row_first() const { return 0; }
    __device__ __forceinline__ int64_t row_end() const { return p.n_rows; }
    __device__ __forceinline__ double n_total() const { return p.n_total; }
    __device__ __forceinline__ bool done() const { return p.ctl[CTL_DONE] != 0; }
    __device__ __forceinline__ bool judge(int eval_parts, int64_t steps_done) const { return em_evaluate(p, eval_parts, steps_done, true); }
    __device__ __forceinline__ int64_t part() const { return blockIdx.x; }
};

__global__ void __launch_bounds__(256)
em_inner_kernel(EmProblem p, int parity, int eval_parts, int64_t steps_done)
{
    em_inner_body(p, EmWholeTable{p}, parity, eval_parts > 0 && blockIdx.x == 0, eval_parts, steps_done, blockIdx.x * (int64_t)blockDim.x + threadIdx.x,
                  (int64_t)gridDim.x * blockDim.x);
}

// ... 453 lines not shown
    __syncthreads();
    const uint32_t mass = local_cum[n - 1];
    const unsigned int draws = tile_total[blockIdx.x];
    if (draws) {
        const int shift = MnGuide::shift_for(mass);
        mn_fill_guide(local_cum, n, shift, guide);
        __syncthreads();
        const uint32_t reject_below = (uint32_t)(0u - mass) % mass;
        MnStream rng(seed, stream_id, 1 + blockIdx.x);
        const unsigned int n_pairs = (unsigned int)(((unsigned long long)draws + 1) >> 1);
        for (unsigned int p = threadIdx.x; p < n_pairs; p += blockDim.x) {
            const uint64_t w = rng.words(p);
            const uint32_t r0 = mn_bounded((uint32_t)(w >> 32), mass, reject_below, rng, p, 0u);
            atomicAdd(&count[mn_find(local_cum, guide, shift, r0)], 1u);
            if (2ull * p + 1 < draws) {
                const uint32_t r1 = mn_bounded((uint32_t)w, mass, reject_below, rng, p, 1u);
                atomicAdd(&count[mn_find(local_cum, guide, shift, r1)], 1u);
            }
        }
        __syncthreads();
    }
    for (int i = threadIdx.x; i < n; i += blockDim.x) counts[(first_class + i) * stride] = (double)count[i];
}

__global__ void __launch_bounds__(256)
em_result_kernel(const unsigned long long *__restrict__ ctl, const double *__restrict__ x0,
                 const double *__restrict__ x1, int64_t n, double *__restrict__ out)
{
    const double *__restrict__ x = (ctl[CTL_ITERS] & 1ULL) ? x1 : x0;
    for (int64_t i = blockIdx.x * (int64_t)blockDim.x + threadIdx.x; i < n;
         i += (int64_t)gridDim.x * blockDim.x) out[i] = x[i];
}

__global__ void __launch_bounds__(256)
permute_f64_kernel(const double *__restrict__ x, const int32_t *__restrict__ perm, int64_t n,
                   double *__restrict__ y, bool scatter)
{
    for (int64_t i = blockIdx.x * (int64_t)blockDim.x + threadIdx.x; i < n;
         i += (int64_t)gridDim.x * blockDim.x) {
        if (scatter) y[perm[i]] = x[i]; else y[i] = x[perm[i]];
    }
}

__global__ void __launch_bounds__(256)
u64_to_double_kernel(const unsigned long long *__restrict__ in, int64_t n, double *__restrict__ out)
{
    for (int64_t i = blockIdx.x * (int64_t)blockDim.x + threadIdx.x; i < n;
         i += (int64_t)gridDim.x * blockDim.x)
        out[i] = (double)in[i];
}

__global__ void __launch_bounds__(256)
double_to_cum_u64_kernel(const double *__restrict__ in, int64_t n, unsigned long long *__restrict__ out)
{
    for (int64_t i = blockIdx.x * (int64_t)blockDim.x + threadIdx.x; i < n;
         i += (int64_t)gridDim.x * blockDim.x)
        out[i] = (unsigned long long)in[i];
}

__global__ void __launch_bounds__(256)
pack_sequences_kernel(const char *__restrict__ bases, int64_t n_bases, uint64_t *__restrict__ seq2,
                      int64_t n_words)
{
    for (int64_t w = blockIdx.x * (int64_t)blockDim.x + threadIdx.x; w < n_words;
         w += (int64_t)gridDim.x * blockDim.x) {
        uint64_t c = 0;
        const int64_t first = w * 32;
        for (int i = 0; i < 32 && first + i < n_bases; ++i)
            c |= (uint64_t)two_bit_encode((uint8_t)bases[first + i]) << (62 - 2 * i);
        seq2[w] = c;
    }
}

static inline unsigned grid_for(int64_t n, int64_t cap = 256 * 16)
{
    int64_t blocks = (n + 255) / 256;
    if (blocks < 1) blocks = 1;
    if (blocks > cap) blocks = cap;
    return (unsigned)blocks;
}

static inline unsigned chip_grid(int64_t work_items, int items_per_block)
{
    int64_t blocks = (work_items + items_per_block - 1) / items_per_block;
    if (blocks < 1) blocks = 1;
    if (blocks > 256 * 8) blocks = 256 * 8;
    return (unsigned)blocks;
}

int em_final_blocks(const EmProblem &p)
{
    int64_t blocks = p.fused ? (p.n_rows + 31) / 32 : (p.n_tx + 255) / 256;
    if (blocks < 1) blocks = 1;
    if (blocks > EM_FINAL_BLOCKS) blocks = EM_FINAL_BLOCKS;
    return (int)blocks;
}

void launch_em_inner(const EmProblem &p, int parity, bool judge_previous, int64_t steps_done, hipStream_t stream)
{
    hipLaunchKernelGGL(em_inner_kernel, dim3(chip_grid(p.n_classes, 256)), dim3(256), 0, stream, p, parity,
                       judge_previous ? em_final_blocks(p) : 0, steps_done);
}

void launch_em_decide(const EmProblem &p, int64_t steps_done, hipStream_t stream)
{
    hipLaunchKernelGGL(em_decide_kernel, dim3(1), dim3(256), 0, stream, p, em_final_blocks(p), steps_done);
}

void launch_em_rows(const EmProblem &p, int parity, hipStream_t stream)
{
    hipLaunchKernelGGL(em_rows_kernel, dim3(chip_grid(p.n_rows, 32)), dim3(256), 0, stream, p, parity);
}

void launch_em_rows_finalize(const EmProblem &p, int parity, hipStream_t stream)
{
    hipLaunchKernelGGL(em_rows_finalize_kernel<false>, dim3((unsigned)em_final_blocks(p)), dim3(256), 0, stream, p, parity);
}

void launch_em_rows_acc(const EmProblem &p, int parity, hipStream_t stream)
{
    EmProblem fused = p;
    fused.fused = 1;
    hipLaunchKernelGGL(em_rows_finalize_kernel<true>, dim3((unsigned)em_final_blocks(fused)), dim3(256), 0, stream, p, parity);
}

void launch_em_local_chunk(const EmProblem &p, const EmTiles &tiles, const double *x_in, int n_steps, int64_t first_step,
                           hipStream_t stream)
{
    if (tiles.n_tiles <= 0 || n_steps <= 0) return;
    hipLaunchKernelGGL(em_local_chunk_kernel, dim3((unsigned)tiles.n_tiles), dim3(256), 0, stream, p, tiles, x_in,
                       std::min(n_steps, EM_CHUNK_MAX), first_step);
}

void launch_em_local_decide(const EmProblem &p, const EmTiles &tiles, int64_t first_step, int n_steps, hipStream_t stream)
{
    hipLaunchKernelGGL(em_local_decide_kernel, dim3(1), dim3(64 * EM_CHUNK_MAX), 0, stream, p, tiles, first_step,
                       std::min(n_steps, EM_CHUNK_MAX));
}

void launch_em_rows_to_acc(const EmProblem &p, hipStream_t stream)
{
    hipLaunchKernelGGL(em_rows_to_acc_kernel, dim3(chip_grid(p.n_tx, 256)), dim3(256), 0, stream, p);
}

void launch_em_finalize(const EmProblem &p, int parity, bool from_acc, hipStream_t stream)
{
    const int blocks = em_final_blocks(p);
    if (from_acc)
        hipLaunchKernelGGL(em_finalize_kernel<true>, dim3((unsigned)blocks), dim3(256), 0, stream, p, parity);
    else
        hipLaunchKernelGGL(em_finalize_kernel<false>, dim3((unsigned)blocks), dim3(256), 0, stream, p, parity);
}

constexpr int NP_MAX_LEAVES = 160;

__device__ __forceinline__ double np_leaf_sum(const double *a, int n)
{
    if (n < 8) {
        double r = 0.0;
        for (int i = 0; i < n; ++i) r += a[i];
        return r;
    }
    double r[8];
    for (int j = 0; j < 8; ++j) r[j] = a[j];
    int i = 8;
    for (; i < n - (n % 8); i += 8)
        for (int j = 0; j < 8; ++j) r[j] += a[i + j];
    double res = ((r[0] + r[1]) + (r[2] + r[3])) + ((r[4] + r[5]) + (r[6] + r[7]));
    for (; i < n; ++i) res += a[i];
    return res;
}

template <int LEVELS>
__device__ __attribute__((noinline)) void np_list_leaves(int lo, int n, int *leaf_lo, int *leaf_n, int *count)
{
    if (n <= 128) {
        if (*count < NP_MAX_LEAVES) { leaf_lo[*count] = lo; leaf_n[*count] = n; }
        ++*count;
        return;
    }
    int n2 = n / 2;
    n2 -= n2 % 8;
    np_list_leaves<LEVELS - 1>(lo, n2, leaf_lo, leaf_n, count);
    np_list_leaves<LEVELS - 1>(lo + n2, n - n2, leaf_lo, leaf_n, count);
}
template <>
__device__ __attribute__((noinline)) void np_list_leaves<0>(int, int, int *, int *, int *count)
{
    *count = NP_MAX_LEAVES + 1;
}

template <int LEVELS>
__device__ __attribute__((noinline)) double np_combine(int n, const double *leaf_sum, int *next)
{
    if (n <= 128) return leaf_sum[(*next)++];
    int n2 = n / 2;
    n2 -= n2 % 8;
    const double left = np_combine<LEVELS - 1>(n2, leaf_sum, next);
    const double right = np_combine<LEVELS - 1>(n - n2, leaf_sum, next);
    return left + right;
}
template <>
__device__ __attribute__((noinline)) double np_combine<0>(int, const double *, int *) { return 0.0; }

__device__ __forceinline__ void np_sum_full_block(const double *__restrict__ a, double *__restrict__ out)
{
    __shared__ double leaf[64];
    const int l = threadIdx.x >> 3, j = threadIdx.x & 7;
    const double *p = a + l * 128 + j;
    double r = p[0];
#pragma unroll
    for (int i = 1; i < 16; ++i) r += p[8 * i];
    r += __shfl_xor(r, 1, 8);
    r += __shfl_xor(r, 2, 8);
    r += __shfl_xor(r, 4, 8);
    if (j == 0) leaf[l] = r;
    __syncthreads();
    if (threadIdx.x < 64) {
        double s = leaf[threadIdx.x];
        for (int d = 1; d < 64; d <<= 1) s += __shfl_xor(s, d, 64);
        if (threadIdx.x == 0) *out = s;
    }
}

__global__ void __launch_bounds__(512)
np_sum_blocks_kernel(const double *__restrict__ a, int64_t n, double *__restrict__ block_sums, int64_t stride)
{
    a += blockIdx.y * stride;
    block_sums += blockIdx.y * (int64_t)gridDim.x;
    const int64_t first = blockIdx.x * (int64_t)8192;
    const int len = (int)min((int64_t)8192, n - first);
    if (len == 8192) {
        np_sum_full_block(a + first, block_sums + blockIdx.x);
        return;
    }
    __shared__ double staged[8192];
    __shared__ int leaf_lo[NP_MAX_LEAVES], leaf_n[NP_MAX_LEAVES], n_leaves;
    __shared__ double leaf_sum[NP_MAX_LEAVES];
    for (int i = threadIdx.x; i < len; i += blockDim.x) staged[i] = a[first + i];
    if (threadIdx.x == 0) {
        int count = 0;
        np_list_leaves<8>(0, len, leaf_lo, leaf_n, &count);
        n_leaves = count;
    }
    __syncthreads();
    if (n_leaves > NP_MAX_LEAVES) {
        if (threadIdx.x == 0) {
            double r = 0.0;
            for (int i = 0; i < len; ++i) r += staged[i];
            block_sums[blockIdx.x] = r;
        }
        return;
    }
    if ((int)threadIdx.x < n_leaves)
        leaf_sum[threadIdx.x] = np_leaf_sum(staged + leaf_lo[threadIdx.x], leaf_n[threadIdx.x]);
    __syncthreads();
    if (threadIdx.x == 0) {
        int next = 0;
        block_sums[blockIdx.x] = np_combine<8>(len, leaf_sum, &next);
    }
}

__global__ void np_sum_final_kernel(const double *block_sums, int64_t n_blocks, double divisor, double *out)
{
    if (threadIdx.x != 0) return;
    block_sums += blockIdx.x * n_blocks;
    out += blockIdx.x * 2;
    double acc = 0.0;
    for (int64_t b = 0; b < n_blocks; ++b) acc += block_sums[b];
    out[0] = acc;
    out[1] = acc / divisor;
}

__global__ void __launch_bounds__(256)
reciprocal_kernel(const double *__restrict__ l, int64_t n, double *__restrict__ x)
{
    for (int64_t i = blockIdx.x * (int64_t)blockDim.x + threadIdx.x; i < n;
         i += (int64_t)gridDim.x * blockDim.x) x[i] = 1.0 / l[i];
}

__global__ void __launch_bounds__(256)
divide_kernel(double *__restrict__ x, int64_t n, const double *__restrict__ s, bool threshold, double floor,
              int64_t stride)
{
    x += blockIdx.y * stride;
    const double d = s[blockIdx.y * 2];
    for (int64_t i = blockIdx.x * (int64_t)blockDim.x + threadIdx.x; i < n;
         i += (int64_t)gridDim.x * blockDim.x) {
        double v = x[i] / d;
        if (threshold && v < floor) v = 0.0;
        x[i] = v;
    }
}

void launch_np_sum(const double *a, int64_t n, double divisor, double *block_sums, double *out,
                   hipStream_t stream)
{
    const int64_t n_blocks = (n + 8191) / 8192;
    if (n_blocks)
        hipLaunchKernelGGL(np_sum_blocks_kernel, dim3((unsigned)n_blocks), dim3(512), 0, stream,
                           a, n, block_sums, (int64_t)0);
    hipLaunchKernelGGL(np_sum_final_kernel, dim3(1), dim3(1), 0, stream, block_sums, n_blocks, divisor, out);
}

void launch_np_sum_many(const double *a, int64_t n, int64_t count, int64_t stride, double divisor,
                        double *block_sums, double *out, hipStream_t stream)
{
    const int64_t n_blocks = (n + 8191) / 8192;
    for (int64_t v0 = 0; v0 < count; v0 += 32768) {
        const unsigned here = (unsigned)std::min<int64_t>(32768, count - v0);
        if (n_blocks)
            hipLaunchKernelGGL(np_sum_blocks_kernel, dim3((unsigned)n_blocks, here), dim3(512), 0, stream,
                               a + v0 * stride, n, block_sums + v0 * n_blocks, stride);
        hipLaunchKernelGGL(np_sum_final_kernel, dim3(here), dim3(1), 0, stream, block_sums + v0 * n_blocks, n_blocks,
                           divisor, out + 2 * v0);
    }
}

void launch_reciprocal(const double *l, int64_t n, double *x, hipStream_t stream)
{
    hipLaunchKernelGGL(reciprocal_kernel, dim3(grid_for(n)), dim3(256), 0, stream, l, n, x);
}

void launch_divide(double *x, int64_t n, const double *s, bool threshold, double floor, hipStream_t stream)
{
    hipLaunchKernelGGL(divide_kernel, dim3(grid_for(n)), dim3(256), 0, stream, x, n, s, threshold, floor, (int64_t)0);
}

void launch_divide_many(double *x, int64_t n, int64_t count, int64_t stride, const double *s, bool threshold,
                        double floor, hipStream_t stream)
{
    for (int64_t v0 = 0; v0 < count; v0 += 32768) {
        const unsigned here = (unsigned)std::min<int64_t>(32768, count - v0);
        hipLaunchKernelGGL(divide_kernel, dim3(std::min<unsigned>(grid_for(n), 64u), here), dim3(256), 0, stream,
                           x + v0 * stride, n, s + 2 * v0, threshold, floor, stride);
    }
}

void launch_effective_lengths(const unsigned long long *fld, const double *lengths, int64_t n_tx,
                              double *out, hipStream_t stream)
{
    hipLaunchKernelGGL(effective_lengths_kernel, dim3(grid_for(n_tx)), dim3(256), 0, stream, fld,
                       lengths, n_tx, out);
}

static unsigned effective_lengths_blocks_per_row(int64_t n, int64_t n_tx)
{
    return std::min<unsigned>(grid_for(n_tx), n >= 64 ? 16u : 256u);
}

void launch_effective_lengths_many(const unsigned long long *fld, int64_t n, const double *lengths, int64_t n_tx,
                                   double *out, hipStream_t stream)
{
    hipLaunchKernelGGL(effective_lengths_kernel, dim3(effective_lengths_blocks_per_row(n, n_tx), (unsigned)n), dim3(256), 0,
                       stream, fld, lengths, n_tx, out);
}

void launch_effective_lengths_weights(const double *p, int64_t n, const double *lengths, int64_t n_tx, double *out,
                                      hipStream_t stream)
{
    const unsigned per_row = n == 1 ? (unsigned)grid_for(n_tx) : effective_lengths_blocks_per_row(n, n_tx);
    hipLaunchKernelGGL(effective_lengths_weights_kernel, dim3(per_row, (unsigned)n), dim3(256), 0, stream, p, lengths, n_tx, out);
}

int multinomial_tile(int64_t n_classes)
{
    int tile = 1;
    while ((n_classes + tile - 1) / tile > MN_TILES) tile <<= 1;
    return tile;
}

bool launch_multinomial(const unsigned long long *cum, int64_t n_classes, int64_t n_draws,
                        uint64_t seed, uint64_t stream_id, unsigned int *tile_total, double *counts,
                        int stride, hipStream_t stream)
{
    if (n_classes <= 0) return true;
    const int tile = multinomial_tile(n_classes);
    if (tile > MN_TILES || n_draws >= (1LL << 32)) return false;
    const int n_tiles = (int)((n_classes + tile - 1) / tile);
    (void)hipMemsetAsync(tile_total, 0, MN_TILES * sizeof(unsigned int), stream);
    if (n_draws > 0)
        hipLaunchKernelGGL(multinomial_tiles_kernel, dim3(512), dim3(1024), 0, stream, cum, n_classes, tile,
                           n_tiles, n_draws, seed, stream_id, tile_total);
    hipLaunchKernelGGL(multinomial_classes_kernel, dim3((unsigned)n_tiles), dim3(1024), 0, stream, cum, n_classes,
                       tile, tile_total, seed, stream_id, counts, stride);
    return true;
}

void launch_em_result(const unsigned long long *ctl, const double *x0, const double *x1, int64_t n, double *out,
                      hipStream_t stream)
{
    hipLaunchKernelGGL(em_result_kernel, dim3(grid_for(n)), dim3(256), 0, stream, ctl, x0, x1, n, out);
}

void launch_permute_f64(const double *x, const int32_t *perm, int64_t n, double *y, bool scatter,
                        hipStream_t stream)
{
    if (n <= 0) return;
    hipLaunchKernelGGL(permute_f64_kernel, dim3(grid_for(n)), dim3(256), 0, stream, x, perm, n, y, scatter);
}

void launch_u64_to_double(const unsigned long long *in, int64_t n, double *out, hipStream_t stream)
{
    if (n <= 0) return;
    hipLaunchKernelGGL(u64_to_double_kernel, dim3(grid_for(n)), dim3(256), 0, stream, in, n, out);
}

void launch_double_to_u64(const double *in, int64_t n, unsigned long long *out, hipStream_t stream)
{
    if (n <= 0) return;
    hipLaunchKernelGGL(double_to_cum_u64_kernel, dim3(grid_for(n)), dim3(256), 0, stream, in, n, out);
}

void launch_pack_sequences(const char *bases, int64_t n_bases, uint64_t *seq2, int64_t n_words,
                           hipStream_t stream)
{
    hipLaunchKernelGGL(pack_sequences_kernel, dim3(grid_for(n_words)), dim3(256), 0, stream, bases,
                       n_bases, seq2, n_words);
}

void warm_code_em()
{
    hipFuncAttributes attributes;
    (void)hipFuncGetAttributes(&attributes, reinterpret_cast<const void *>(&em_inner_kernel));
}

}

namespace skm {
__global__ void __launch_bounds__(256)
gather_probe_kernel(const uint4 *__restrict__ table, uint64_t slot_mask, int per_lane, int chain,
                    unsigned long long *sink)
{
    uint64_t x = mix64(blockIdx.x * (uint64_t)blockDim.x + threadIdx.x + 1);
    unsigned long long acc = 0;
    if (chain) {
        for (int i = 0; i < per_lane; ++i) {
            const uint4 v = table[x & slot_mask];
            acc += v.x;
            x = mix64(x + v.y + i);
        }
    } else {
        for (int i = 0; i < per_lane; i += 4) {
            const uint64_t a = mix64(x + i), b2 = mix64(x + i + 1), c = mix64(x + i + 2), d = mix64(x + i + 3);
            const uint4 v0 = table[a & slot_mask], v1 = table[b2 & slot_mask], v2 = table[c & slot_mask],
                        v3 = table[d & slot_mask];
            acc += v0.x + v1.x + v2.x + v3.x;
        }
    }
    if (acc == 0x123456789ULL) *sink = acc;
}

void launch_gather_probe(const void *table, uint64_t n_slots, int blocks, int per_lane, int chain,
                         unsigned long long *sink, hipStream_t stream)
{
    hipLaunchKernelGGL(gather_probe_kernel, dim3(blocks), dim3(256), 0, stream, (const uint4 *)table,
                       n_slots - 1, per_lane, chain, sink);
}
}
```

### seekmer_amd/csrc/skm_kernels.h

```cpp
#pragma once
#include "skm_device.h"

namespace skm {

struct MapBatch {
    const uint32_t *records;
    int64_t n_units;
    int32_t words_per_read;
    int32_t record_words;
    int32_t paired;
    int32_t *workspace;
    int32_t *rec_unit;
    uint64_t *rec_key;
    unsigned long long *rec_tuple;
    int32_t keep_spans;
    int32_t *unit_begin, *unit_end;
    Coord *unit_anchor;
    int32_t *unit_entries;
    int64_t ids_capacity;
    unsigned long long *ids_cursor;
    unsigned long long *fld;
    unsigned long long *stats;
    int32_t vote[8];
};
// ... 132 lines not shown
    const int64_t *tx_row;
    double *row_sum;
    const double *eff_len;
    double *x[2];
    double *acc;
    double n_total;
    double rel_tol, x_floor;
    unsigned long long *ctl;
    double *part_max;
    unsigned int *part_flags;
    int64_t max_iters, fixed_iters;
    int fused;
    unsigned int *arrivals;
    const double *extra_max;
    const unsigned int *extra_flags;
    int64_t n_extra, extra_first;
};
enum { CTL_DONE = 0, CTL_ITERS = 1, CTL_UNDEFINED = 3, CTL_TILE_FAULT = 4 };
#ifndef SKM_EM_FINAL_BLOCKS
#define SKM_EM_FINAL_BLOCKS 2048
#endif
constexpr int EM_FINAL_BLOCKS = SKM_EM_FINAL_BLOCKS;
void launch_em_inner(const EmProblem &p, int parity, bool judge_previous, int64_t steps_done, hipStream_t stream);
void launch_em_decide(const EmProblem &p, int64_t steps_done, hipStream_t stream);
void launch_em_rows(const EmProblem &p, int parity, hipStream_t stream);
void launch_em_rows_finalize(const EmProblem &p, int parity, hipStream_t stream);
void launch_em_rows_acc(const EmProblem &p, int parity, hipStream_t stream);
void launch_em_rows_to_acc(const EmProblem &p, hipStream_t stream);
void launch_em_finalize(const EmProblem &p, int parity, bool from_acc, hipStream_t stream);
void launch_em_result(const unsigned long long *ctl, const double *x0, const double *x1, int64_t n, double *out,
                      hipStream_t stream);

constexpr int EM_TILE_PAIRS = 2048, EM_TILE_CLASSES = 512, EM_TILE_TX = 128;
#ifndef SKM_EM_TILE_SEGMENT
#define SKM_EM_TILE_SEGMENT 128
#endif
constexpr int EM_TILE_SEGMENT = SKM_EM_TILE_SEGMENT;
constexpr int EM_CHUNK_MAX = 16;
constexpr int EM_TILE_CLASS_BATCH = 4;
struct EmTiles {
    int64_t n_tiles;
    const int64_t *tile_tx;
    const int64_t *tile_cls;
    const int32_t *tx_list;
    const int32_t *cls_list;
    const int64_t *cls_pair;
    const int64_t *tx_pair;
    const uint16_t *cls_tx;
    const uint16_t *tx_cls;
    double *step_max;
    unsigned int *step_flags;
    double *snap;
};
void launch_em_local_chunk(const EmProblem &p, const EmTiles &tiles, const double *x_in, int n_steps, int64_t first_step,
                           hipStream_t stream);
void launch_em_local_decide(const EmProblem &p, const EmTiles &tiles, int64_t first_step, int n_steps, hipStream_t stream);

constexpr int EM_BATCH = 8;
struct EmBatchProblem {
    int64_t n_tx, n_classes, n_rows;
    const int64_t *cls_offset;
    const int32_t *ids;
    const int64_t *row_start;
    const int32_t *row_tx;
    const int32_t *tx_cls;
    const int64_t *tx_row;
    const double *eff_len;
    const double *cls_count;
    double *inner;
    double *row_sum;
    double *x[2];
    double *place_total;
    double rel_tol, x_floor;
    unsigned long long *ctl;
    double *part_max;
    unsigned int *part_flags;
    int managed;
    unsigned long long *mgr;
    int64_t *iters_out;
    int fused;
    unsigned int *arrivals;
};
enum { BCTL_ALL_DONE = 0, BCTL_LAST_STEP = 1, BCTL_DONE = 8, BCTL_ITERS = 16, BCTL_UNDEFINED = 24 };
enum { MGR_NEXT = 0, MGR_COUNT = 1, MGR_FINISHED = 2, MGR_UNDEFINED = 3, MGR_REP = 8, MGR_SINCE = 16, MGR_TAKE = 24,
       MGR_PUT = 32 };
void launch_em_batch_manage_init(const EmBatchProblem &p, unsigned long long *mgr, unsigned long long *host_pinned64,
                                 int64_t n_reps, const double *counts_all, const double *totals, const double *x_start,
                                 double *out_all, hipStream_t stream);
void launch_em_batch_manage(const EmBatchProblem &p, unsigned long long *mgr, const double *counts_all, const double *totals,
                            const double *x_start, double *out_all, int64_t *iters_out, int64_t step, bool planned,
                            hipStream_t stream);
void launch_em_batch_step(const EmBatchProblem &p, int64_t step, hipStream_t stream);
void launch_em_batch_decide(const EmBatchProblem &p, int64_t steps_done, hipStream_t stream);
void launch_em_batch_take(const double *x, int64_t n_tx, int r, double *out, hipStream_t stream);
void launch_em_batch_ctl(unsigned long long *ctl, unsigned int idle, hipStream_t stream);
void launch_blend_counts(const double *own, const int32_t *class_cell, const double *weight, const double *cell_total,
                         int64_t n_cells, int64_t first, int64_t n_rows, int64_t n_classes, double *rows, hipStream_t stream);
void launch_permute_rows_f64(const double *x, const int32_t *perm, int64_t n, int64_t n_rows, double *y, hipStream_t stream);
struct EmSetSlot {
    int64_t cls_first, cls_end;
    int64_t row_first, row_end;
    double n_total;
    unsigned long long done;
    unsigned long long iters;
    unsigned long long undefined;
};
struct EmSetProblem {
    const int64_t *cls_offset;
    const int32_t *ids;
    const double *cls_count;
    double *inner;
    const int64_t *row_start;
    const int32_t *row_tx;
    const int32_t *tx_cls;
    const int64_t *tx_row;
    double *row_sum;
    const double *eff_len;
    double *x[2];
    double rel_tol, x_floor;
    int64_t max_iters;
    EmSetSlot *slots;
    int n_slots;
    int n_parts;
    double *part_max;
    unsigned int *part_flags;
    unsigned int *arrivals;
};
int em_set_parts(int64_t largest_rows);
void launch_em_set_step(const EmSetProblem &p, int64_t largest_classes, int64_t step, bool judge_previous, hipStream_t stream);
void launch_em_set_decide(const EmSetProblem &p, int64_t steps_done, unsigned long long *running, hipStream_t stream);
void launch_em_set_result(const EmSetSlot *slots, int n_slots, const double *x0, const double *x1, int64_t n_tx, double *out,
                          hipStream_t stream);
void launch_stack_tuples(const int64_t *src, const int64_t *dst, const int32_t *add, int64_t n_classes, const int32_t *arena,
                         int32_t *ids, hipStream_t stream);
void launch_repeat_row(double *x, int64_t n_tx, int64_t n, hipStream_t stream);

struct QuantBuild {
    int64_t n_tx, n_classes, n_ids;
    int64_t *cls_offset;
    int32_t *ids;
    double *cls_count;
    int32_t *tx_cls;
    int64_t *tx_row;
    int64_t *row_start;
    int32_t *row_tx;
    int64_t n_rows_cap;
    int64_t first_seen_bound;
    int64_t *tile_tx, *tile_cls;
    int32_t *tx_list, *cls_list;
    int64_t *cls_pair, *tx_pair;
    uint16_t *tile_cls_tx, *tile_tx_cls;
    int32_t *tx_label, *tx_tile, *cls_tile;
    int64_t tile_info[2];
};
int64_t quant_setup(const ClassTable *table, QuantBuild &q, int32_t *perm, hipStream_t stream);
struct QuantResidual {
    int64_t n_classes, n_ids, n_rows;
    int64_t *cls_offset;
    int32_t *ids;
    int32_t *cls_src;
    int64_t *row_start;
    int32_t *row_tx;
    int32_t *tx_cls;
    int64_t *tx_row;
};
int quant_residual_count(const QuantBuild &q, int64_t counts[3], hipStream_t stream);
int quant_residual_build(const QuantBuild &q, QuantResidual &r, hipStream_t stream);
void launch_permute_f64(const double *x, const int32_t *perm, int64_t n, double *y, bool scatter,
                        hipStream_t stream);
const char *quant_setup_failure();
int64_t quant_rows_upper_bound(int64_t n_tx, int64_t n_ids);

void launch_np_sum(const double *a, int64_t n, double divisor, double *block_sums, double *out,
                   hipStream_t stream);
void launch_np_sum_many(const double *a, int64_t n, int64_t count, int64_t stride, double divisor,
                        double *block_sums, double *out, hipStream_t stream);
void launch_reciprocal(const double *l, int64_t n, double *x, hipStream_t stream);
void launch_divide(double *x, int64_t n, const double *s, bool threshold, double floor, hipStream_t stream);
void launch_divide_many(double *x, int64_t n, int64_t count, int64_t stride, const double *s, bool threshold,
                        double floor, hipStream_t stream);
void launch_effective_lengths(const unsigned long long *fld, const double *lengths, int64_t n_tx,
                              double *out, hipStream_t stream);
void launch_effective_lengths_many(const unsigned long long *fld, int64_t n, const double *lengths, int64_t n_tx,
                                   double *out, hipStream_t stream);
void launch_effective_lengths_weights(const double *p, int64_t n, const double *lengths, int64_t n_tx, double *out,
                                      hipStream_t stream);
bool launch_multinomial(const unsigned long long *cum, int64_t n_classes, int64_t n_draws,
                        uint64_t seed, uint64_t stream_id, unsigned int *tile_total, double *counts,
                        int stride, hipStream_t stream);
void launch_u64_to_double(const unsigned long long *in, int64_t n, double *out, hipStream_t stream);
void launch_double_to_u64(const double *in, int64_t n, unsigned long long *out, hipStream_t stream);

void warm_code_map();
void warm_code_classes();
void warm_code_em();
void warm_code_em_batch();
void warm_code_em_set();
void warm_code_quant_setup();

}
```

### seekmer_amd/csrc/skm_quant_setup.hip

```cpp
#include "skm_kernels.h"
#include "skm_pool.h"

#include <algorithm>
#include <cstdio>
#include <vector>

namespace skm {

namespace {

struct Scratch {
    hipStream_t stream;
    std::vector<void *> held;
    explicit Scratch(hipStream_t s) : stream(s) {}
    template <class T>
    T *alloc(size_t n)
    {
        void *p = nullptr;
        if (pool_alloc(&p, std::max<size_t>(n, 1) * sizeof(T)) != hipSuccess) return nullptr;
        held.push_back(p);
        return static_cast<T *>(p);
    }
    ~Scratch()
    {
        (void)hipStreamSynchronize(stream);
        for (void *p : held) pool_free(p);
    }
};
thread_local char g_setup_failure[160] = "";
#define QB_ALLOC(var, type, n) type *var = scratch.alloc<type>(n); \
    if (!var) { snprintf(g_setup_failure, sizeof(g_setup_failure), "no memory for %s", #var); return -1; }

#define QB_TRY(call) do { const hipError_t qb_e = (call); if (qb_e != hipSuccess) { \
    snprintf(g_setup_failure, sizeof(g_setup_failure), "%s: %s", #call, hipGetErrorString(qb_e)); return -1; } } while (0)

__global__ void __launch_bounds__(256)
iota_kernel(int32_t *out, int64_t n)
{
    for (int64_t i = blockIdx.x * (int64_t)blockDim.x + threadIdx.x; i < n;
         i += (int64_t)gridDim.x * blockDim.x) out[i] = (int32_t)i;
}

__global__ void __launch_bounds__(256)
table_dump_kernel(ClassTable t, int64_t n_classes, int64_t *arena_off, int64_t *len, double *count,
                  unsigned long long *first_seen, uint32_t *min_id)
{
    for (int64_t k = blockIdx.x * (int64_t)blockDim.x + threadIdx.x; k < n_classes;
         k += (int64_t)gridDim.x * blockDim.x) {
        const int64_t i = t.class_list[k];
        const ClassSlot s = t.slots[i];
        const int64_t off = s.tuple < 0 ? -1 : tuple_offset(s.tuple);
        const int64_t n = s.tuple < 0 ? 0 : tuple_len(s.tuple);
        arena_off[k] = off;
        len[k] = n;
        count[k] = (double)s.count;
        first_seen[k] = s.first_seen;
        if (min_id) {
            uint32_t m = 0xffffffffu;
            for (int64_t j = 0; j < n; ++j) m = min(m, (uint32_t)t.arena[off + j]);
            min_id[k] = m;
        }
    }
}

__global__ void __launch_bounds__(256)
mark_first_seen_kernel(const unsigned long long *first_seen, int64_t n_classes, uint64_t bound,
                       uint32_t *bits, unsigned int *duplicate)
{
    for (int64_t k = blockIdx.x * (int64_t)blockDim.x + threadIdx.x; k < n_classes;
         k += (int64_t)gridDim.x * blockDim.x) {
        const unsigned long long f = first_seen[k];
        if (f >= bound) { atomicOr(duplicate, 2u); continue; }
        const uint32_t bit = 1u << (f & 31);
        if (atomicOr(&bits[f >> 5], bit) & bit) atomicOr(duplicate, 1u);
    }
}

__global__ void __launch_bounds__(256)
word_popcount_kernel(const uint32_t *bits, int64_t n_words, int64_t *count)
{
    for (int64_t w = blockIdx.x * (int64_t)blockDim.x + threadIdx.x; w < n_words;
         w += (int64_t)gridDim.x * blockDim.x) count[w] = __popc(bits[w]);
}

__global__ void __launch_bounds__(256)
first_seen_rank_kernel(const unsigned long long *first_seen, const uint32_t *min_id, int64_t n_classes,
                       uint64_t bound, const uint32_t *bits, const int64_t *word_base, int32_t *by_rank,
                       uint32_t *key_by_rank)
{
    for (int64_t k = blockIdx.x * (int64_t)blockDim.x + threadIdx.x; k < n_classes;
         k += (int64_t)gridDim.x * blockDim.x) {
        const unsigned long long f = first_seen[k];
        if (f >= bound) continue;
        const int64_t r = word_base[f >> 5] + __popc(bits[f >> 5] & ((1u << (f & 31)) - 1u));
        if (r >= n_classes) continue;
        by_rank[r] = (int32_t)k;
        key_by_rank[r] = min_id[k];
    }
}

__global__ void __launch_bounds__(256)
gather_by_rank_kernel(const int32_t *perm, const int32_t *by_rank, int64_t n, const int64_t *len_in,
                      const double *count_in, const int64_t *arena_off_in, int64_t *len_out,
                      double *count_out, int64_t *arena_off_out)
{
    for (int64_t j = blockIdx.x * (int64_t)blockDim.x + threadIdx.x; j < n;
         j += (int64_t)gridDim.x * blockDim.x) {
        const int32_t k = by_rank[perm[j]];
        len_out[j] = len_in[k];
        count_out[j] = count_in[k];
        arena_off_out[j] = arena_off_in[k];
    }
}

__global__ void __launch_bounds__(256)
copy_tuples_direct_kernel(int64_t n, const int64_t *src_off, const int32_t *arena, const int64_t *cls_offset,
                          int32_t *ids)
{
    for (int64_t j = blockIdx.x * (int64_t)blockDim.x + threadIdx.x; j < n;
         j += (int64_t)gridDim.x * blockDim.x) {
        const int64_t src = src_off[j];
        const int64_t dst = cls_offset[j];
        const int64_t len = cls_offset[j + 1] - dst;
        for (int64_t i = 0; i < len; i += 8) {
            int32_t v[8];
#pragma unroll
            for (int k = 0; k < 8; ++k) v[k] = i + k < len ? arena[src + i + k] : 0;
#pragma unroll
            for (int k = 0; k < 8; ++k) if (i + k < len) ids[dst + i + k] = v[k];
        }
    }
}

__global__ void __launch_bounds__(256)
gather_classes_kernel(const int32_t *perm, int64_t n, const int64_t *len_in, const double *count_in,
                      int64_t *len_out, double *count_out)
{
    for (int64_t k = blockIdx.x * (int64_t)blockDim.x + threadIdx.x; k < n;
         k += (int64_t)gridDim.x * blockDim.x) {
        const int32_t src = perm[k];
        len_out[k] = len_in[src];
        count_out[k] = count_in[src];
    }
}

__global__ void __launch_bounds__(256)
copy_tuples_kernel(const int32_t *perm, int64_t n, const int64_t *arena_off, const int32_t *arena,
                   const int64_t *cls_offset, int32_t *ids)
{
    for (int64_t k = blockIdx.x * (int64_t)blockDim.x + threadIdx.x; k < n;
         k += (int64_t)gridDim.x * blockDim.x) {
        const int64_t src = arena_off[perm[k]];
        const int64_t dst = cls_offset[k];
        const int64_t len = cls_offset[k + 1] - dst;
        for (int64_t j = 0; j < len; ++j) ids[dst + j] = arena[src + j];
    }
}

__global__ void __launch_bounds__(256)
set_last_offset_kernel(int64_t *offsets, const int64_t *lens, int64_t n)
{
    if (blockIdx.x == 0 && threadIdx.x == 0) offsets[n] = n ? offsets[n - 1] + lens[n - 1] : 0;
}

__global__ void __launch_bounds__(256)
pair_class_kernel(const int64_t *cls_offset, int64_t n_classes, int32_t *pair_cls)
{
    for (int64_t c = blockIdx.x * (int64_t)blockDim.x + threadIdx.x; c < n_classes;
         c += (int64_t)gridDim.x * blockDim.x)
        for (int64_t j = cls_offset[c]; j < cls_offset[c + 1]; ++j) pair_cls[j] = (int32_t)c;
}

__global__ void __launch_bounds__(256)
segment_starts_kernel(const int32_t *sorted_tx, int64_t n_pairs, int64_t n_tx, int64_t *tx_offset)
{
    for (int64_t j = blockIdx.x * (int64_t)blockDim.x + threadIdx.x; j <= n_pairs;
         j += (int64_t)gridDim.x * blockDim.x) {
        const int64_t lo = j == 0 ? -1 : sorted_tx[j - 1];
        const int64_t hi = j == n_pairs ? n_tx : sorted_tx[j];
        for (int64_t t = lo + 1; t <= hi; ++t) tx_offset[t] = j;
    }
}

__global__ void __launch_bounds__(256)
row_count_kernel(const int64_t *tx_offset, int64_t n_tx, int64_t *rows)
{
    for (int64_t t = blockIdx.x * (int64_t)blockDim.x + threadIdx.x; t < n_tx;
         t += (int64_t)gridDim.x * blockDim.x) {
        const int64_t degree = tx_offset[t + 1] - tx_offset[t];
        rows[t] = degree > 0 ? (degree + EM_ROW_CAP - 1) / EM_ROW_CAP : 1;
    }
}

__global__ void __launch_bounds__(256)
row_fill_kernel(const int64_t *tx_offset, const int64_t *tx_row, int64_t n_tx, int64_t n_pairs,
                int64_t *row_start, int32_t *row_tx)
{
    for (int64_t t = blockIdx.x * (int64_t)blockDim.x + threadIdx.x; t < n_tx;
         t += (int64_t)gridDim.x * blockDim.x) {
        int64_t pos = tx_offset[t];
        for (int64_t r = tx_row[t]; r < tx_row[t + 1]; ++r) {
            row_start[r] = pos;
            row_tx[r] = (int32_t)t;
            pos += EM_ROW_CAP;
        }
        if (t == n_tx - 1) row_start[tx_row[n_tx]] = n_pairs;
    }
}

__global__ void __launch_bounds__(256)
class_min_id_kernel(const int64_t *cls_offset, const int32_t *ids, int64_t n_classes, uint32_t *key,
                    int64_t *len)
{
    for (int64_t c = blockIdx.x * (int64_t)blockDim.x + threadIdx.x; c < n_classes;
         c += (int64_t)gridDim.x * blockDim.x) {
        uint32_t m = 0xffffffffu;
        for (int64_t j = cls_offset[c]; j < cls_offset[c + 1]; ++j) m = min(m, (uint32_t)ids[j]);
        key[c] = m;
        len[c] = cls_offset[c + 1] - cls_offset[c];
    }
}

__global__ void __launch_bounds__(256)
copy_tuples_by_offset_kernel(const int32_t *perm, int64_t n, const int64_t *src_offset, const int32_t *src,
                             const int64_t *dst_offset, int32_t *dst)
{
    for (int64_t k = blockIdx.x * (int64_t)blockDim.x + threadIdx.x; k < n;
         k += (int64_t)gridDim.x * blockDim.x) {
        const int64_t from = src_offset[perm[k]];
        const int64_t to = dst_offset[k];
        const int64_t len = dst_offset[k + 1] - to;
        for (int64_t j = 0; j < len; ++j) dst[to + j] = src[from + j];
    }
}

inline unsigned blocks_for(int64_t n)
{
    int64_t b = (n + 255) / 256;
    if (b < 1) b = 1;
    if (b > 256 * 16) b = 256 * 16;
    return (unsigned)b;
}

constexpr int SCAN_TILE = 2048;

template <class T>
__global__ void __launch_bounds__(256)
scan_tile_sums_kernel(const T *__restrict__ in, int64_t n, T *__restrict__ tile_sums)
{
    __shared__ T s_wave[4];
    const int64_t base = blockIdx.x * (int64_t)SCAN_TILE + threadIdx.x * 8;
    T sum = 0;
#pragma unroll
    for (int k = 0; k < 8; ++k) sum += base + k < n ? in[base + k] : (T)0;
    for (int d = 32; d > 0; d >>= 1) sum += __shfl_xor(sum, d, 64);
    if ((threadIdx.x & 63) == 0) s_wave[threadIdx.x >> 6] = sum;
    __syncthreads();
    if (threadIdx.x == 0) tile_sums[blockIdx.x] = s_wave[0] + s_wave[1] + s_wave[2] + s_wave[3];
}

template <class T>
__global__ void __launch_bounds__(1024)
scan_of_sums_kernel(T *tile_sums, int64_t n_tiles, T *total)
{
    __shared__ T s_part[1024];
    const int64_t per = (n_tiles + 1023) / 1024;
    const int64_t first = threadIdx.x * per, last = min(n_tiles, first + per);
    T sum = 0;
    for (int64_t i = first; i < last; ++i) sum += tile_sums[i];
    s_part[threadIdx.x] = sum;
    __syncthreads();
    for (int step = 1; step < 1024; step <<= 1) {
        const T add = (int)threadIdx.x >= step ? s_part[threadIdx.x - step] : (T)0;
        __syncthreads();
        s_part[threadIdx.x] += add;
        __syncthreads();
    }
    T at = s_part[threadIdx.x] - sum;
    for (int64_t i = first; i < last; ++i) { const T v = tile_sums[i]; tile_sums[i] = at; at += v; }
    if (total && threadIdx.x == 1023) *total = s_part[1023];
}

template <class T>
__global__ void __launch_bounds__(256)
scan_tiles_kernel(const T *__restrict__ in, int64_t n, const T *__restrict__ tile_base, T *__restrict__ out)
{
    __shared__ T s_wave[4];
    const int64_t base = blockIdx.x * (int64_t)SCAN_TILE + threadIdx.x * 8;
    T v[8], sum = 0;
#pragma unroll
    for (int k = 0; k < 8; ++k) { v[k] = base + k < n ? in[base + k] : (T)0; sum += v[k]; }
    T incl = sum;
    const int lane = threadIdx.x & 63, wave = threadIdx.x >> 6;
#pragma unroll
    for (int d = 1; d < 64; d <<= 1) {
        const T up = __shfl_up(incl, d, 64);
        if (lane >= d) incl += up;
    }
    if (lane == 63) s_wave[wave] = incl;
    __syncthreads();
    T at = tile_base[blockIdx.x] + incl - sum;
    for (int w = 0; w < wave; ++w) at += s_wave[w];
#pragma unroll
    for (int k = 0; k < 8; ++k) {
        if (base + k < n) out[base + k] = at;
        at += v[k];
    }
}

template <class T>
int exclusive_scan(Scratch &scratch, const T *in, T *out, int64_t n, T *total)
{
    hipStream_t stream = scratch.stream;
    if (n <= 0) {
        if (total) QB_TRY(hipMemsetAsync(total, 0, sizeof(T), stream));
        return 0;
    }
    const int64_t n_tiles = (n + SCAN_TILE - 1) / SCAN_TILE;
    QB_ALLOC(tile_sums, T, n_tiles);
    hipLaunchKernelGGL(scan_tile_sums_kernel<T>, dim3((unsigned)n_tiles), dim3(256), 0, stream, in, n, tile_sums);
    hipLaunchKernelGGL(scan_of_sums_kernel<T>, dim3(1), dim3(1024), 0, stream, tile_sums, n_tiles, total);
    hipLaunchKernelGGL(scan_tiles_kernel<T>, dim3((unsigned)n_tiles), dim3(256), 0, stream, in, n, tile_sums, out);
    return 0;
}

int exclusive_scan_with_total(Scratch &scratch, const int64_t *in, int64_t *out, int64_t n)
{
    if (n >= (1LL << 40)) return -2;
    return exclusive_scan<int64_t>(scratch, in, out, n, out + n);
}

constexpr int RS_BITS = 9, RS_BINS = 1 << RS_BITS, RS_ITEMS = 16, RS_TILE = 256 * RS_ITEMS;

template <class K>
__global__ void __launch_bounds__(256)
radix_hist_kernel(const K *__restrict__ keys, int64_t n, int shift, uint32_t *__restrict__ hist, int64_t n_tiles)
{
    __shared__ uint32_t h[RS_BINS];
    for (int d = threadIdx.x; d < RS_BINS; d += 256) h[d] = 0;
    __syncthreads();
    const int64_t base = blockIdx.x * (int64_t)RS_TILE;
#pragma unroll 4
    for (int i = 0; i < RS_ITEMS; ++i) {
        const int64_t at = base + i * 256 + threadIdx.x;
        if (at < n) atomicAdd(&h[(uint32_t)((unsigned long long)keys[at] >> shift) & (RS_BINS - 1)], 1u);
    }
    __syncthreads();
    for (int d = threadIdx.x; d < RS_BINS; d += 256) hist[d * n_tiles + blockIdx.x] = h[d];
}

__global__ void __launch_bounds__(256)
radix_digit_scan_kernel(uint32_t *hist, int64_t n_tiles, uint32_t *digit_total)
{
    __shared__ uint32_t s_wave[4];
    __shared__ uint32_t s_carry;
    uint32_t *row = hist + blockIdx.x * n_tiles;
    const int lane = threadIdx.x & 63, wave = threadIdx.x >> 6;
    if (threadIdx.x == 0) s_carry = 0;
    __syncthreads();
    for (int64_t base = 0; base < n_tiles; base += 256 * 4) {
        const int64_t at = base + threadIdx.x * 4;
        uint32_t v[4], sum = 0;
#pragma unroll
        for (int k = 0; k < 4; ++k) { v[k] = at + k < n_tiles ? row[at + k] : 0u; sum += v[k]; }
        uint32_t incl = sum;
#pragma unroll
        for (int d = 1; d < 64; d <<= 1) {
            const uint32_t up = __shfl_up(incl, d, 64);
            if (lane >= d) incl += up;
        }
        if (lane == 63) s_wave[wave] = incl;
        __syncthreads();
        uint32_t run = s_carry + incl - sum;
        for (int w = 0; w < wave; ++w) run += s_wave[w];
#pragma unroll
        for (int k = 0; k < 4; ++k) {
            if (at + k < n_tiles) row[at + k] = run;
            run += v[k];
        }
        __syncthreads();
        if (threadIdx.x == 255) s_carry = run;
        __syncthreads();
    }
    if (threadIdx.x == 0) digit_total[blockIdx.x] = s_carry;
}

template <class K>
__global__ void __launch_bounds__(256)
radix_scatter_kernel(const K *__restrict__ keys_in, const int32_t *__restrict__ vals_in, K *__restrict__ keys_out,
                     int32_t *__restrict__ vals_out, int64_t n, int shift, const uint32_t *__restrict__ offsets,
                     const uint32_t *__restrict__ digit_total, int64_t n_tiles)
{
    __shared__ uint32_t wave_base[4][RS_BINS];
    __shared__ uint32_t tile_start[RS_BINS + 1];
    __shared__ uint32_t s_scan[256];
    __shared__ uint32_t digit_base[RS_BINS];
    __shared__ K s_keys[RS_TILE];
    __shared__ int32_t s_vals[RS_TILE];
    const int lane = threadIdx.x & 63, wave = threadIdx.x >> 6;
    for (int d = threadIdx.x; d < 4 * RS_BINS; d += 256) (&wave_base[0][0])[d] = 0;
    {
        const uint32_t t0 = digit_total[2 * threadIdx.x], t1 = digit_total[2 * threadIdx.x + 1];
        uint32_t incl = t0 + t1;
#pragma unroll
        for (int d = 1; d < 64; d <<= 1) {
            const uint32_t up = __shfl_up(incl, d, 64);
            if (lane >= d) incl += up;
        }
        if (lane == 63) s_scan[wave] = incl;
        __syncthreads();
        uint32_t at = incl - (t0 + t1);
        for (int w = 0; w < wave; ++w) at += s_scan[w];
        digit_base[2 * threadIdx.x] = at;
        digit_base[2 * threadIdx.x + 1] = at + t0;
    }
    __syncthreads();
    const int64_t first = blockIdx.x * (int64_t)RS_TILE + wave * (RS_TILE / 4);
    K key[RS_ITEMS];
    int32_t val[RS_ITEMS];
    uint32_t digit[RS_ITEMS];
#pragma unroll
    for (int c = 0; c < RS_ITEMS; ++c) {
        const int64_t at = first + c * 64 + lane;
        const bool valid = at < n;
        key[c] = valid ? keys_in[at] : (K)0;
        val[c] = valid ? vals_in[at] : 0;
        digit[c] = (uint32_t)((unsigned long long)key[c] >> shift) & (RS_BINS - 1);
        if (valid) atomicAdd(&wave_base[wave][digit[c]], 1u);
    }
    __syncthreads();
    const int d0 = 2 * threadIdx.x;
    const uint32_t c0 = wave_base[0][d0] + wave_base[1][d0] + wave_base[2][d0] + wave_base[3][d0];
    const uint32_t c1 = wave_base[0][d0 + 1] + wave_base[1][d0 + 1] + wave_base[2][d0 + 1] + wave_base[3][d0 + 1];
    uint32_t incl = c0 + c1;
#pragma unroll
    for (int d = 1; d < 64; d <<= 1) {
        const uint32_t up = __shfl_up(incl, d, 64);
        if (lane >= d) incl += up;
    }
    if (lane == 63) s_scan[wave] = incl;
    __syncthreads();
    uint32_t at0 = incl - (c0 + c1);
    for (int w = 0; w < wave; ++w) at0 += s_scan[w];
    tile_start[d0] = at0;
    tile_start[d0 + 1] = at0 + c0;
    if (threadIdx.x == 255) tile_start[RS_BINS] = at0 + c0 + c1;
    uint32_t run0 = at0, run1 = at0 + c0;
#pragma unroll
    for (int w = 0; w < 4; ++w) {
        const uint32_t n0 = wave_base[w][d0], n1 = wave_base[w][d0 + 1];
        wave_base[w][d0] = run0; wave_base[w][d0 + 1] = run1;
        run0 += n0; run1 += n1;
    }
    __syncthreads();
#pragma unroll
    for (int c = 0; c < RS_ITEMS; ++c) {
        const bool valid = first + c * 64 + lane < n;
        unsigned long long same = __ballot(valid);
#pragma unroll
        for (int b = 0; b < RS_BITS; ++b) {
            const bool bit = (digit[c] >> b) & 1u;
            const unsigned long long with = __ballot(valid && bit);
            same &= bit ? with : ~with;
        }
        if (valid) {
            const uint32_t before = (uint32_t)__popcll(same & ((1ULL << lane) - 1ULL));
            const uint32_t place = wave_base[wave][digit[c]] + before;
            s_keys[place] = key[c];
            s_vals[place] = val[c];
            if (before == 0) wave_base[wave][digit[c]] += (uint32_t)__popcll(same);
        }
        __builtin_amdgcn_fence(__ATOMIC_RELEASE, "wavefront");
        __builtin_amdgcn_fence(__ATOMIC_ACQUIRE, "wavefront");
    }
    __syncthreads();
    const int64_t tile_first = blockIdx.x * (int64_t)RS_TILE;
    const uint32_t tile_n = (uint32_t)min((int64_t)RS_TILE, n - tile_first);
#pragma unroll 4
    for (int i = 0; i < RS_ITEMS; ++i) {
        const uint32_t j = i * 256 + threadIdx.x;
        if (j >= tile_n) continue;
        const K k = s_keys[j];
        const uint32_t d = (uint32_t)((unsigned long long)k >> shift) & (RS_BINS - 1);
        const int64_t to = (int64_t)digit_base[d] + offsets[d * n_tiles + blockIdx.x] + (j - tile_start[d]);
        keys_out[to] = k;
        vals_out[to] = s_vals[j];
    }
}

template <class K>
int sort_pairs(Scratch &scratch, const K *keys_in, K *keys_out, const int32_t *vals_in, int32_t *vals_out,
               int64_t n, int end_bit)
{
    hipStream_t stream = scratch.stream;
    if (n <= 0) return 0;
    if (n >= (1LL << 32)) return -2;
    const int passes = std::max(1, (end_bit + RS_BITS - 1) / RS_BITS);
    const int64_t n_tiles = (n + RS_TILE - 1) / RS_TILE;
    QB_ALLOC(hist, uint32_t, RS_BINS * n_tiles);
    QB_ALLOC(digit_total, uint32_t, RS_BINS);
    K *tmp_keys = nullptr;
    int32_t *tmp_vals = nullptr;
    if (passes > 1) {
        QB_ALLOC(tk, K, n); QB_ALLOC(tv, int32_t, n);
        tmp_keys = tk; tmp_vals = tv;
    }
    const K *src_k = keys_in;
    const int32_t *src_v = vals_in;
    for (int pass = 0; pass < passes; ++pass) {
        const bool to_out = ((passes - 1 - pass) & 1) == 0;
        K *dst_k = to_out ? keys_out : tmp_keys;
        int32_t *dst_v = to_out ? vals_out : tmp_vals;
        const int shift = pass * RS_BITS;
        hipLaunchKernelGGL(radix_hist_kernel<K>, dim3((unsigned)n_tiles), dim3(256), 0, stream, src_k, n, shift, hist, n_tiles);
        hipLaunchKernelGGL(radix_digit_scan_kernel, dim3(RS_BINS), dim3(256), 0, stream, hist, n_tiles, digit_total);
        hipLaunchKernelGGL(radix_scatter_kernel<K>, dim3((unsigned)n_tiles), dim3(256), 0, stream, src_k, src_v, dst_k, dst_v, n,
                           shift, hist, digit_total, n_tiles);
        src_k = dst_k;
        src_v = dst_v;
    }
    return 0;
}

}

int64_t quant_rows_upper_bound(int64_t n_tx, int64_t n_ids)
{
    return n_tx + n_ids / EM_ROW_CAP + 1;
}

namespace {

int build_from_table(Scratch &scratch, const ClassTable &t, QuantBuild &q)
{
    hipStream_t stream = scratch.stream;
    const int64_t n_classes = q.n_classes;
    if (n_classes == 0) {
        QB_TRY(hipMemsetAsync(q.cls_offset, 0, sizeof(int64_t), stream));
        return 0;
    }
    if (n_classes >= (1LL << 31) || q.n_ids >= (1LL << 31)) return -2;
    QB_ALLOC(arena_off, int64_t, n_classes); QB_ALLOC(len, int64_t, n_classes);
    QB_ALLOC(len_sorted, int64_t, n_classes); QB_ALLOC(count, double, n_classes);
    QB_ALLOC(first, unsigned long long, n_classes); QB_ALLOC(first_sorted, unsigned long long, n_classes);
    QB_ALLOC(iota, int32_t, n_classes); QB_ALLOC(perm, int32_t, n_classes);
    hipLaunchKernelGGL(table_dump_kernel, dim3(blocks_for(n_classes)), dim3(256), 0, stream,
                       t, n_classes, arena_off, len, count, first, (uint32_t *)nullptr);
    hipLaunchKernelGGL(iota_kernel, dim3(blocks_for(n_classes)), dim3(256), 0, stream, iota, n_classes);
    int first_bits = 64;
    if (q.first_seen_bound > 0) {
        first_bits = 1;
        while (first_bits < 63 && (1LL << first_bits) <= q.first_seen_bound) ++first_bits;
    }
    if (sort_pairs(scratch, first, first_sorted, iota, perm, n_classes, first_bits)) return -1;
    hipLaunchKernelGGL(gather_classes_kernel, dim3(blocks_for(n_classes)), dim3(256), 0, stream, perm,
                       n_classes, len, count, len_sorted, q.cls_count);
    if (exclusive_scan_with_total(scratch, len_sorted, q.cls_offset, n_classes)) return -1;
    hipLaunchKernelGGL(copy_tuples_kernel, dim3(blocks_for(n_classes)), dim3(256), 0, stream, perm,
                       n_classes, arena_off, t.arena, q.cls_offset, q.ids);
    return 0;
}

constexpr int64_t RANK_BITMAP_MAX_UNITS = 1LL << 31;

int build_from_table_ranked(Scratch &scratch, const ClassTable &t, QuantBuild &q, int32_t *perm)
{
    hipStream_t stream = scratch.stream;
    const int64_t C = q.n_classes;
    if (C == 0) {
        QB_TRY(hipMemsetAsync(q.cls_offset, 0, sizeof(int64_t), stream));
        return 0;
    }
    if (C >= (1LL << 31) || q.n_ids >= (1LL << 31)) return -2;
    const uint64_t bound = (uint64_t)q.first_seen_bound;
    const int64_t n_words = (int64_t)((bound + 31) / 32);
    QB_ALLOC(arena_off, int64_t, C); QB_ALLOC(len, int64_t, C); QB_ALLOC(count, double, C);
    QB_ALLOC(first, unsigned long long, C); QB_ALLOC(min_id, uint32_t, C);
    QB_ALLOC(bits, uint32_t, n_words); QB_ALLOC(duplicate, unsigned int, 1);
    QB_TRY(hipMemsetAsync(bits, 0, n_words * sizeof(uint32_t), stream));
    QB_TRY(hipMemsetAsync(duplicate, 0, sizeof(unsigned int), stream));
    hipLaunchKernelGGL(table_dump_kernel, dim3(blocks_for(C)), dim3(256), 0, stream, t, C, arena_off, len, count,
                       first, min_id);
    hipLaunchKernelGGL(mark_first_seen_kernel, dim3(blocks_for(C)), dim3(256), 0, stream, first, C, bound, bits,
                       duplicate);
    unsigned int shared_first_seen = 0;
    QB_TRY(hipMemcpyAsync(&shared_first_seen, duplicate, sizeof(unsigned int), hipMemcpyDeviceToHost, stream));
    QB_TRY(hipStreamSynchronize(stream));
    if (shared_first_seen) return 1;

    QB_ALLOC(word_count, int64_t, n_words); QB_ALLOC(word_base, int64_t, n_words + 1);
    QB_ALLOC(by_rank, int32_t, C); QB_ALLOC(key_by_rank, uint32_t, C); QB_ALLOC(key_sorted, uint32_t, C);
    QB_ALLOC(iota, int32_t, C); QB_ALLOC(len_sorted, int64_t, C); QB_ALLOC(src_off, int64_t, C);
    hipLaunchKernelGGL(word_popcount_kernel, dim3(blocks_for(n_words)), dim3(256), 0, stream, bits, n_words,
                       word_count);
    if (exclusive_scan_with_total(scratch, word_count, word_base, n_words)) return -1;
    hipLaunchKernelGGL(first_seen_rank_kernel, dim3(blocks_for(C)), dim3(256), 0, stream, first, min_id, C, bound,
                       bits, word_base, by_rank, key_by_rank);
    hipLaunchKernelGGL(iota_kernel, dim3(blocks_for(C)), dim3(256), 0, stream, iota, C);
    int end_bit = 1;
    while ((1LL << end_bit) < q.n_tx && end_bit < 32) ++end_bit;
    if (sort_pairs(scratch, key_by_rank, key_sorted, iota, perm, C, end_bit)) return -1;
    hipLaunchKernelGGL(gather_by_rank_kernel, dim3(blocks_for(C)), dim3(256), 0, stream, perm, by_rank, C, len,
                       count, arena_off, len_sorted, q.cls_count, src_off);
    if (exclusive_scan_with_total(scratch, len_sorted, q.cls_offset, C)) return -1;
    hipLaunchKernelGGL(copy_tuples_direct_kernel, dim3(blocks_for(C)), dim3(256), 0, stream, C, src_off, t.arena,
                       q.cls_offset, q.ids);
    return 0;
}

int localize(Scratch &scratch, QuantBuild &q, int32_t *perm)
{
    hipStream_t stream = scratch.stream;
    const int64_t C = q.n_classes, M = q.n_ids;
    if (C == 0) return 0;
    if (C >= (1LL << 31) || M >= (1LL << 31)) return -2;
    QB_ALLOC(key, uint32_t, C); QB_ALLOC(key_sorted, uint32_t, C); QB_ALLOC(iota, int32_t, C);
    QB_ALLOC(ids_copy, int32_t, M); QB_ALLOC(len, int64_t, C); QB_ALLOC(len_sorted, int64_t, C);
    QB_ALLOC(old_offset, int64_t, C + 1); QB_ALLOC(count_copy, double, C);
    hipLaunchKernelGGL(class_min_id_kernel, dim3(blocks_for(C)), dim3(256), 0, stream, q.cls_offset, q.ids, C,
                       key, len);
    hipLaunchKernelGGL(iota_kernel, dim3(blocks_for(C)), dim3(256), 0, stream, iota, C);
    int end_bit = 1;
    while ((1LL << end_bit) < q.n_tx && end_bit < 32) ++end_bit;
    if (sort_pairs(scratch, key, key_sorted, iota, perm, C, end_bit)) return -1;
    QB_TRY(hipMemcpyAsync(old_offset, q.cls_offset, (C + 1) * 8, hipMemcpyDeviceToDevice, stream));
    QB_TRY(hipMemcpyAsync(ids_copy, q.ids, M * 4, hipMemcpyDeviceToDevice, stream));
    QB_TRY(hipMemcpyAsync(count_copy, q.cls_count, C * 8, hipMemcpyDeviceToDevice, stream));
    hipLaunchKernelGGL(gather_classes_kernel, dim3(blocks_for(C)), dim3(256), 0, stream, perm, C, len,
                       count_copy, len_sorted, q.cls_count);
    if (exclusive_scan_with_total(scratch, len_sorted, q.cls_offset, C)) return -1;
    hipLaunchKernelGGL(copy_tuples_by_offset_kernel, dim3(blocks_for(C)), dim3(256), 0, stream, perm, C,
                       old_offset, ids_copy, q.cls_offset, q.ids);
    return 0;
}

int transpose(Scratch &scratch, QuantBuild &q)
{
    hipStream_t stream = scratch.stream;
    const int64_t C = q.n_classes, M = q.n_ids, T = q.n_tx;
    if (M >= (1LL << 31) || C >= (1LL << 31)) return -2;
    QB_ALLOC(pair_cls, int32_t, M); QB_ALLOC(sorted_tx, int32_t, M);
    QB_ALLOC(tx_offset, int64_t, T + 1); QB_ALLOC(rows, int64_t, T);
    if (M > 0) {
        hipLaunchKernelGGL(pair_class_kernel, dim3(blocks_for(C)), dim3(256), 0, stream, q.cls_offset, C,
                           pair_cls);
        int end_bit = 1;
        while ((1LL << end_bit) < T && end_bit < 31) ++end_bit;
        if (sort_pairs(scratch, q.ids, sorted_tx, pair_cls, q.tx_cls, M, end_bit)) return -1;
    }
    hipLaunchKernelGGL(segment_starts_kernel, dim3(blocks_for(M + 1)), dim3(256), 0, stream, sorted_tx, M,
                       T, tx_offset);
    hipLaunchKernelGGL(row_count_kernel, dim3(blocks_for(T)), dim3(256), 0, stream, tx_offset, T, rows);
    if (exclusive_scan_with_total(scratch, rows, q.tx_row, T)) return -1;
    hipLaunchKernelGGL(row_fill_kernel, dim3(blocks_for(T)), dim3(256), 0, stream, tx_offset, q.tx_row, T,
                       M, q.row_start, q.row_tx);
    return 0;
}

__device__ __forceinline__ int32_t cc_root(const int32_t *parent, int32_t v)
{
    int32_t p;
    while ((p = parent[v]) != v) v = p;
    return v;
}

__device__ __forceinline__ int32_t cc_root_halving(int32_t *parent, int32_t v)
{
    int32_t p = parent[v];
    while (p != v) {
        const int32_t g = parent[p];
        if (g != p) atomicMin(&parent[v], g);
        v = p;
        p = g;
    }
    return v;
}

__global__ void __launch_bounds__(256)
cc_hook_kernel(const int64_t *cls_offset, const int32_t *ids, int64_t n_classes, int32_t *parent)
{
    for (int64_t c = blockIdx.x * (int64_t)blockDim.x + threadIdx.x; c < n_classes;
         c += (int64_t)gridDim.x * blockDim.x) {
        const int64_t begin = cls_offset[c], end = cls_offset[c + 1];
        if (begin == end) continue;
        int32_t b = cc_root_halving(parent, ids[begin]);
        for (int64_t j = begin + 1; j < end; ++j) {
            int32_t a = cc_root_halving(parent, ids[j]);
            while (a != b) {
                if (a < b) { const int32_t s = a; a = b; b = s; }
                const int32_t old = atomicCAS(&parent[a], a, b);
                if (old == a) break;
                a = cc_root_halving(parent, old);
            }
            b = a < b ? a : b;
        }
    }
}

__global__ void __launch_bounds__(256)
cc_label_kernel(int32_t *parent, const int64_t *tx_row, const int64_t *row_start, int64_t n_tx,
                int32_t *label, int32_t *comp)
{
    const int lane = threadIdx.x & 63;
    const int64_t stride = (int64_t)gridDim.x * blockDim.x;
    for (int64_t t0 = blockIdx.x * (int64_t)blockDim.x + threadIdx.x - lane; t0 < n_tx; t0 += stride) {
        const int64_t t = t0 + lane;
        int32_t r = -1, degree = 0;
        if (t < n_tx) {
            r = cc_root_halving(parent, (int32_t)t);
            label[t] = r;
            degree = (int32_t)(row_start[tx_row[t + 1]] - row_start[tx_row[t]]);
        }
        unsigned long long todo = __ballot(r >= 0);
        while (todo) {
            const int leader = __ffsll((long long)todo) - 1;
            const int32_t r0 = __shfl(r, leader, 64);
            const bool mine = r == r0;
            const unsigned long long same = __ballot(mine);
            int sum = mine ? degree : 0;
            for (int d = 32; d > 0; d >>= 1) sum += __shfl_xor(sum, d, 64);
            if (lane == leader) {
                atomicAdd(&comp[3 * (int64_t)r0], (int)__popcll(same));
                atomicAdd(&comp[3 * (int64_t)r0 + 1], sum);
            }
            todo &= ~same;
        }
    }
}

__global__ void __launch_bounds__(256)
cc_classes_kernel(const int64_t *cls_offset, const int32_t *ids, int64_t n_classes, const int32_t *label,
                  int32_t *comp)
{
    const int lane = threadIdx.x & 63;
    const int64_t stride = (int64_t)gridDim.x * blockDim.x;
    for (int64_t c0 = blockIdx.x * (int64_t)blockDim.x + threadIdx.x - lane; c0 < n_classes; c0 += stride) {
        const int64_t c = c0 + lane;
        int32_t r = -1;
        if (c < n_classes) {
            const int64_t begin = cls_offset[c];
            r = label[begin < cls_offset[c + 1] ? ids[begin] : 0];
        }
        const int32_t before = __shfl_up(r, 1, 64);
        const unsigned long long heads = __ballot(lane == 0 || before != r);
        if (r >= 0 && ((heads >> lane) & 1ULL)) {
            const unsigned long long later = lane == 63 ? 0ULL : heads >> (lane + 1);
            const int run = later ? __ffsll((long long)later) : 64 - lane;
            atomicAdd(&comp[3 * (int64_t)r + 2], run);
        }
    }
}

__global__ void __launch_bounds__(256)
tile_pack_kernel(const int32_t *__restrict__ comp, int64_t n_tx, int64_t n_segments, int32_t *__restrict__ root_tile,
                 int64_t *__restrict__ seg_tiles, unsigned long long *__restrict__ oversize)
{
    for (int64_t g = blockIdx.x * (int64_t)blockDim.x + threadIdx.x; g < n_segments;
         g += (int64_t)gridDim.x * blockDim.x) {
        int tx = 0, pairs = 0, classes = 0, n = 0;
        const int64_t last = min(n_tx, (g + 1) * EM_TILE_SEGMENT);
        for (int64_t t0 = g * EM_TILE_SEGMENT; t0 < last; t0 += 8) {
            int size[24];
#pragma unroll
            for (int k = 0; k < 24; ++k) size[k] = 3 * t0 + k < 3 * n_tx ? comp[3 * t0 + k] : 0;
#pragma unroll
            for (int k = 0; k < 8; ++k) {
                const int64_t t = t0 + k;
                if (t >= last) break;
                const int c_tx = size[3 * k], c_pairs = size[3 * k + 1], c_classes = size[3 * k + 2];
                if (c_tx == 0) { root_tile[t] = -1; continue; }
                if (c_tx > EM_TILE_TX || c_pairs > EM_TILE_PAIRS || c_classes > EM_TILE_CLASSES) {
                    root_tile[t] = -2;
                    atomicAdd(oversize, 1ULL);
                    continue;
                }
                if (n == 0 || tx + c_tx > EM_TILE_TX || pairs + c_pairs > EM_TILE_PAIRS ||
                    classes + c_classes > EM_TILE_CLASSES) {
                    ++n;
                    tx = pairs = classes = 0;
                }
                tx += c_tx; pairs += c_pairs; classes += c_classes;
                root_tile[t] = n - 1;
            }
        }
        seg_tiles[g] = n;
    }
}

__global__ void __launch_bounds__(256)
tx_tile_kernel(const int32_t *label, const int32_t *root_tile, const int64_t *seg_base, int64_t n_tx,
               const int64_t *tx_row, const int64_t *row_start, int degree_bits, int32_t *tx_tile, int32_t *key)
{
    for (int64_t t = blockIdx.x * (int64_t)blockDim.x + threadIdx.x; t < n_tx;
         t += (int64_t)gridDim.x * blockDim.x) {
        const int32_t r = label[t], at = root_tile[r];
        const int32_t tile = at < 0 ? (int32_t)n_tx : (int32_t)(seg_base[r / EM_TILE_SEGMENT] + at);
        tx_tile[t] = tile;
        const int64_t turns = (row_start[tx_row[t + 1]] - row_start[tx_row[t]] + 7) >> 3;
        const int32_t longest = (1 << degree_bits) - 1;
        key[t] = (tile << degree_bits) | (longest - (int32_t)min(turns, (int64_t)longest));
    }
}

#ifndef SKM_EM_CLASS_ORDER
#define SKM_EM_CLASS_ORDER 1
#endif
__global__ void __launch_bounds__(256)
cls_tile_kernel(const int64_t *cls_offset, const int32_t *ids, int64_t n_classes, const int32_t *tx_tile,
                int length_bits, int32_t *cls_tile, int32_t *key)
{
    for (int64_t c = blockIdx.x * (int64_t)blockDim.x + threadIdx.x; c < n_classes;
         c += (int64_t)gridDim.x * blockDim.x) {
        const int64_t begin = cls_offset[c], end = cls_offset[c + 1];
        const int32_t tile = tx_tile[begin < end ? ids[begin] : 0];
        cls_tile[c] = tile;
        const int64_t turns = (end - begin + EM_TILE_CLASS_BATCH - 1) / EM_TILE_CLASS_BATCH;
        const int32_t longest = (1 << length_bits) - 1;
        key[c] = (tile << length_bits) | (longest - (int32_t)min(turns, (int64_t)longest));
    }
}

__global__ void __launch_bounds__(256)
tile_starts_kernel(const int32_t *sorted_tile, int shift, int64_t n, const int64_t *n_tiles, int64_t *first)
{
    const int64_t tiles = *n_tiles;
    for (int64_t j = blockIdx.x * (int64_t)blockDim.x + threadIdx.x; j <= n;
         j += (int64_t)gridDim.x * blockDim.x) {
        const int64_t lo = j == 0 ? -1 : min((int64_t)(sorted_tile[j - 1] >> shift), tiles);
        const int64_t hi = j == n ? tiles : min((int64_t)(sorted_tile[j] >> shift), tiles);
        for (int64_t t = lo + 1; t <= hi; ++t) first[t] = j;
    }
}

__global__ void __launch_bounds__(256)
tile_local_tx_kernel(const int32_t *list, const int32_t *tile_sorted, int shift, const int64_t *first, const int64_t *n_tiles, int64_t n,
                     const int64_t *tx_row, const int64_t *row_start, int32_t *local, int64_t *len)
{
    for (int64_t i = blockIdx.x * (int64_t)blockDim.x + threadIdx.x; i < n;
         i += (int64_t)gridDim.x * blockDim.x) {
        const int32_t t = list[i];
        local[t] = (int32_t)(i - first[min((int64_t)(tile_sorted[i] >> shift), *n_tiles)]);
        len[i] = row_start[tx_row[t + 1]] - row_start[tx_row[t]];
    }
}

__global__ void __launch_bounds__(256)
tile_local_cls_kernel(const int32_t *list, const int32_t *tile_sorted, int shift, const int64_t *first, const int64_t *n_tiles, int64_t n,
                      const int64_t *cls_offset, int32_t *local, int64_t *len)
{
    for (int64_t k = blockIdx.x * (int64_t)blockDim.x + threadIdx.x; k < n;
         k += (int64_t)gridDim.x * blockDim.x) {
        const int32_t c = list[k];
        local[c] = (int32_t)(k - first[min((int64_t)(tile_sorted[k] >> shift), *n_tiles)]);
        len[k] = cls_offset[c + 1] - cls_offset[c];
    }
}

__global__ void __launch_bounds__(256)
tile_fill_cls_kernel(const int32_t *cls_list, int64_t n_classes, const int64_t *cls_offset, const int32_t *ids,
                     const int32_t *tx_local, const int64_t *cls_pair, const int32_t *cls_tile, int32_t residual_tile,
                     uint16_t *out)
{
    for (int64_t k = blockIdx.x * (int64_t)blockDim.x + threadIdx.x; k < n_classes;
         k += (int64_t)gridDim.x * blockDim.x) {
        const int32_t c = cls_list[k];
        if (cls_tile[c] == residual_tile) continue;
        const int64_t src = cls_offset[c], n = cls_offset[c + 1] - src, dst = cls_pair[k];
        for (int64_t j = 0; j < n; ++j) out[dst + j] = (uint16_t)tx_local[ids[src + j]];
    }
}

__global__ void __launch_bounds__(256)
tile_fill_tx_kernel(const int32_t *tx_list, int64_t n_tx, const int64_t *tx_row, const int64_t *row_start,
                    const int32_t *tx_cls, const int32_t *cls_local, const int64_t *tx_pair, const int32_t *tx_tile,
                    uint16_t *out)
{
    const int sub = threadIdx.x & 7;
    for (int64_t i = (blockIdx.x * (int64_t)blockDim.x + threadIdx.x) >> 3; i < n_tx;
         i += ((int64_t)gridDim.x * blockDim.x) >> 3) {
        const int32_t t = tx_list[i];
        if (tx_tile[t] == (int32_t)n_tx) continue;
        const int64_t src = row_start[tx_row[t]], n = row_start[tx_row[t + 1]] - src, dst = tx_pair[i];
        for (int64_t j = sub; j < n; j += 8) out[dst + j] = (uint16_t)cls_local[tx_cls[src + j]];
    }
}

int build_tiles(Scratch &scratch, QuantBuild &q)
{
    hipStream_t stream = scratch.stream;
    const int64_t C = q.n_classes, M = q.n_ids, T = q.n_tx;
    if (M >= (1LL << 31) || C >= (1LL << 31) || T >= (1LL << 31) - 2) return -2;
    const int64_t n_segments = (T + EM_TILE_SEGMENT - 1) / EM_TILE_SEGMENT;
    QB_ALLOC(parent, int32_t, T); QB_ALLOC(comp, int32_t, 3 * T); QB_ALLOC(root_tile, int32_t, T);
    QB_ALLOC(seg_tiles, int64_t, n_segments); QB_ALLOC(seg_base, int64_t, n_segments + 1);
    QB_ALLOC(oversize, unsigned long long, 1);
    QB_ALLOC(iota, int32_t, std::max(T, C)); QB_ALLOC(sorted_tile, int32_t, std::max(T, C));
    QB_ALLOC(tx_local, int32_t, T); QB_ALLOC(cls_local, int32_t, C);
    QB_ALLOC(len, int64_t, std::max(T, C));
    QB_TRY(hipMemsetAsync(comp, 0, 3 * T * sizeof(int32_t), stream));
    QB_TRY(hipMemsetAsync(oversize, 0, sizeof(unsigned long long), stream));
    hipLaunchKernelGGL(iota_kernel, dim3(blocks_for(T)), dim3(256), 0, stream, parent, T);
    hipLaunchKernelGGL(cc_hook_kernel, dim3(blocks_for(C)), dim3(256), 0, stream, q.cls_offset, q.ids, C, parent);
    hipLaunchKernelGGL(cc_label_kernel, dim3(blocks_for(T)), dim3(256), 0, stream, parent, q.tx_row, q.row_start, T,
                       q.tx_label, comp);
    hipLaunchKernelGGL(cc_classes_kernel, dim3(blocks_for(C)), dim3(256), 0, stream, q.cls_offset, q.ids, C,
                       q.tx_label, comp);
    hipLaunchKernelGGL(tile_pack_kernel, dim3(blocks_for(n_segments)), dim3(256), 0, stream, comp, T, n_segments,
                       root_tile, seg_tiles, oversize);
    if (exclusive_scan_with_total(scratch, seg_tiles, seg_base, n_segments)) return -1;
    int end_bit = 1;
    while ((1LL << end_bit) < T + 1 && end_bit < 31) ++end_bit;
    const int degree_bits = end_bit + 5 <= 31 ? 5 : 0;
    QB_ALLOC(tx_key, int32_t, T);
    hipLaunchKernelGGL(tx_tile_kernel, dim3(blocks_for(T)), dim3(256), 0, stream, q.tx_label, root_tile, seg_base, T,
                       q.tx_row, q.row_start, degree_bits, q.tx_tile, tx_key);
    hipLaunchKernelGGL(iota_kernel, dim3(blocks_for(std::max(T, C))), dim3(256), 0, stream, iota, std::max(T, C));
    if (sort_pairs(scratch, tx_key, sorted_tile, iota, q.tx_list, T, end_bit + degree_bits)) return -1;
    hipLaunchKernelGGL(tile_starts_kernel, dim3(blocks_for(T + 1)), dim3(256), 0, stream, sorted_tile, degree_bits, T,
                       seg_base + n_segments, q.tile_tx);
    hipLaunchKernelGGL(tile_local_tx_kernel, dim3(blocks_for(T)), dim3(256), 0, stream, q.tx_list, sorted_tile, degree_bits,
                       q.tile_tx, seg_base + n_segments, T, q.tx_row, q.row_start, tx_local, len);
    if (exclusive_scan_with_total(scratch, len, q.tx_pair, T)) return -1;
    const int length_bits = SKM_EM_CLASS_ORDER ? degree_bits : 0;
    QB_ALLOC(cls_key, int32_t, C);
    hipLaunchKernelGGL(cls_tile_kernel, dim3(blocks_for(C)), dim3(256), 0, stream, q.cls_offset, q.ids, C, q.tx_tile,
                       length_bits, q.cls_tile, cls_key);
    if (sort_pairs(scratch, cls_key, sorted_tile, iota, q.cls_list, C, end_bit + length_bits)) return -1;
    hipLaunchKernelGGL(tile_starts_kernel, dim3(blocks_for(C + 1)), dim3(256), 0, stream, sorted_tile, length_bits, C,
                       seg_base + n_segments, q.tile_cls);
    hipLaunchKernelGGL(tile_local_cls_kernel, dim3(blocks_for(C)), dim3(256), 0, stream, q.cls_list, sorted_tile, length_bits,
                       q.tile_cls, seg_base + n_segments, C, q.cls_offset, cls_local, len);
    if (exclusive_scan_with_total(scratch, len, q.cls_pair, C)) return -1;
    hipLaunchKernelGGL(tile_fill_cls_kernel, dim3(blocks_for(C)), dim3(256), 0, stream, q.cls_list, C, q.cls_offset,
                       q.ids, tx_local, q.cls_pair, q.cls_tile, (int32_t)T, q.tile_cls_tx);
    hipLaunchKernelGGL(tile_fill_tx_kernel, dim3(blocks_for(8 * T)), dim3(256), 0, stream, q.tx_list, T, q.tx_row,
                       q.row_start, q.tx_cls, cls_local, q.tx_pair, q.tx_tile, q.tile_tx_cls);
    QB_TRY(hipMemcpyAsync(&q.tile_info[0], seg_base + n_segments, sizeof(int64_t), hipMemcpyDeviceToHost, stream));
    QB_TRY(hipMemcpyAsync(&q.tile_info[1], oversize, sizeof(int64_t), hipMemcpyDeviceToHost, stream));
    return 0;
}

}

int64_t quant_setup(const ClassTable *table, QuantBuild &q, int32_t *perm, hipStream_t stream)
{
    const bool can_rank = table && q.first_seen_bound > 0 && q.first_seen_bound <= RANK_BITMAP_MAX_UNITS;
    for (int attempt = can_rank ? 0 : 1; attempt < 2; ++attempt) {
        int64_t n_rows = -1;
        {
            Scratch scratch(stream);
            if (attempt == 0) {
                const int rc = build_from_table_ranked(scratch, *table, q, perm);
                if (rc == 1) continue;
                if (rc) return -1;
            } else {
                if (table && build_from_table(scratch, *table, q)) return -1;
                if (localize(scratch, q, perm)) return -1;
            }
            if (transpose(scratch, q)) return -1;
            if (q.tile_tx && build_tiles(scratch, q)) return -1;
            QB_TRY(hipGetLastError());
            QB_TRY(hipMemcpyAsync(&n_rows, q.tx_row + q.n_tx, sizeof(int64_t), hipMemcpyDeviceToHost, stream));
        }
        if (n_rows > q.n_rows_cap) return -3;
        return n_rows;
    }
    return -1;
}

namespace {

__global__ void __launch_bounds__(256)
residual_count_kernel(const int32_t *cls_tile, const int64_t *cls_offset, int64_t n_classes, const int32_t *tx_tile,
                      const int64_t *tx_row, int64_t n_tx, unsigned long long *counts)
{
    unsigned long long classes = 0, pairs = 0, rows = 0;
    for (int64_t i = blockIdx.x * (int64_t)blockDim.x + threadIdx.x; i < max(n_classes, n_tx);
         i += (int64_t)gridDim.x * blockDim.x) {
        if (i < n_classes && cls_tile[i] == (int32_t)n_tx) { ++classes; pairs += cls_offset[i + 1] - cls_offset[i]; }
        if (i < n_tx && tx_tile[i] == (int32_t)n_tx) rows += tx_row[i + 1] - tx_row[i];
    }
    if (classes) atomicAdd(&counts[0], classes);
    if (pairs) atomicAdd(&counts[1], pairs);
    if (rows) atomicAdd(&counts[2], rows);
}

__global__ void __launch_bounds__(256)
residual_class_sizes_kernel(const int32_t *cls_tile, const int64_t *cls_offset, int64_t n_classes, int32_t residual_tile,
                            int64_t *keep, int64_t *len)
{
    for (int64_t c = blockIdx.x * (int64_t)blockDim.x + threadIdx.x; c < n_classes;
         c += (int64_t)gridDim.x * blockDim.x) {
        const bool mine = cls_tile[c] == residual_tile;
        keep[c] = mine ? 1 : 0;
        len[c] = mine ? cls_offset[c + 1] - cls_offset[c] : 0;
    }
}

__global__ void __launch_bounds__(256)
residual_tx_sizes_kernel(const int32_t *tx_tile, const int64_t *tx_row, const int64_t *row_start, int64_t n_tx,
                         int64_t *rows, int64_t *len)
{
    for (int64_t t = blockIdx.x * (int64_t)blockDim.x + threadIdx.x; t < n_tx;
         t += (int64_t)gridDim.x * blockDim.x) {
        const bool mine = tx_tile[t] == (int32_t)n_tx;
        rows[t] = mine ? tx_row[t + 1] - tx_row[t] : 0;
        len[t] = mine ? row_start[tx_row[t + 1]] - row_start[tx_row[t]] : 0;
    }
}

__global__ void __launch_bounds__(256)
residual_fill_cls_kernel(const int32_t *cls_tile, int64_t n_classes, int32_t residual_tile, const int64_t *rank,
                         const int64_t *cls_offset, const int32_t *ids, const int64_t *new_offset,
                         int64_t *out_offset, int32_t *out_ids, int32_t *out_src, int64_t n_residual)
{
    for (int64_t c = blockIdx.x * (int64_t)blockDim.x + threadIdx.x; c < n_classes;
         c += (int64_t)gridDim.x * blockDim.x) {
        if (cls_tile[c] != residual_tile) continue;
        const int64_t k = rank[c], src = cls_offset[c], n = cls_offset[c + 1] - src, dst = new_offset[c];
        out_offset[k] = dst;
        if (k == n_residual - 1) out_offset[n_residual] = dst + n;
        out_src[k] = (int32_t)c;
        for (int64_t j = 0; j < n; ++j) out_ids[dst + j] = ids[src + j];
    }
}

__global__ void __launch_bounds__(256)
residual_fill_tx_kernel(const int32_t *tx_tile, int64_t n_tx, const int64_t *tx_row, const int64_t *row_start,
                        const int32_t *tx_cls, const int64_t *rank, const int64_t *new_pair, int32_t *out)
{
    const int sub = threadIdx.x & 7;
    for (int64_t t = (blockIdx.x * (int64_t)blockDim.x + threadIdx.x) >> 3; t < n_tx;
         t += ((int64_t)gridDim.x * blockDim.x) >> 3) {
        if (tx_tile[t] != (int32_t)n_tx) continue;
        const int64_t src = row_start[tx_row[t]], n = row_start[tx_row[t + 1]] - src, dst = new_pair[t];
        for (int64_t j = sub; j < n; j += 8) out[dst + j] = (int32_t)rank[tx_cls[src + j]];
    }
}

}

int quant_residual_count(const QuantBuild &q, int64_t counts[3], hipStream_t stream)
{
    Scratch scratch(stream);
    QB_ALLOC(sums, unsigned long long, 3);
    QB_TRY(hipMemsetAsync(sums, 0, 3 * sizeof(unsigned long long), stream));
    hipLaunchKernelGGL(residual_count_kernel, dim3(blocks_for(std::max(q.n_classes, q.n_tx))), dim3(256), 0, stream,
                       q.cls_tile, q.cls_offset, q.n_classes, q.tx_tile, q.tx_row, q.n_tx, sums);
    QB_TRY(hipGetLastError());
    QB_TRY(hipMemcpyAsync(counts, sums, 3 * sizeof(int64_t), hipMemcpyDeviceToHost, stream));
    QB_TRY(hipStreamSynchronize(stream));
    return 0;
}

int quant_residual_build(const QuantBuild &q, QuantResidual &r, hipStream_t stream)
{
    Scratch scratch(stream);
    const int64_t C = q.n_classes, T = q.n_tx;
    QB_ALLOC(keep, int64_t, C); QB_ALLOC(rank, int64_t, C + 1);
    QB_ALLOC(len, int64_t, std::max(C, T)); QB_ALLOC(new_offset, int64_t, C + 1);
    QB_ALLOC(rows, int64_t, T); QB_ALLOC(new_pair, int64_t, T + 1);
    hipLaunchKernelGGL(residual_class_sizes_kernel, dim3(blocks_for(C)), dim3(256), 0, stream, q.cls_tile, q.cls_offset, C,
                       (int32_t)T, keep, len);
    if (exclusive_scan_with_total(scratch, keep, rank, C)) return -1;
    if (exclusive_scan_with_total(scratch, len, new_offset, C)) return -1;
    hipLaunchKernelGGL(residual_fill_cls_kernel, dim3(blocks_for(C)), dim3(256), 0, stream, q.cls_tile, C, (int32_t)T, rank,
                       q.cls_offset, q.ids, new_offset, r.cls_offset, r.ids, r.cls_src, r.n_classes);
    hipLaunchKernelGGL(residual_tx_sizes_kernel, dim3(blocks_for(T)), dim3(256), 0, stream, q.tx_tile, q.tx_row,
                       q.row_start, T, rows, len);
    if (exclusive_scan_with_total(scratch, rows, r.tx_row, T)) return -1;
    if (exclusive_scan_with_total(scratch, len, new_pair, T)) return -1;
    hipLaunchKernelGGL(row_fill_kernel, dim3(blocks_for(T)), dim3(256), 0, stream, new_pair, r.tx_row, T, r.n_ids,
                       r.row_start, r.row_tx);
    hipLaunchKernelGGL(residual_fill_tx_kernel, dim3(blocks_for(8 * T)), dim3(256), 0, stream, q.tx_tile, T, q.tx_row,
                       q.row_start, q.tx_cls, rank, new_pair, r.tx_cls);
    QB_TRY(hipGetLastError());
    return 0;
}

const char *quant_setup_failure() { return g_setup_failure; }

void warm_code_quant_setup()
{
    hipFuncAttributes attributes;
    (void)hipFuncGetAttributes(&attributes, reinterpret_cast<const void *>(&iota_kernel));
    (void)hipFuncGetAttributes(&attributes, reinterpret_cast<const void *>(&table_dump_kernel));
}

}
```

Baseline: 966.3 million pairs/s.

## Fuse reduction and scan finals into last-block tickets, drop iota arrays, parallelize tile packing

The np_sum reduction now uses an atomic ticket so the last block does the final combine, which removes the separate final kernel launch. Its recursive leaf-listing is replaced by a fixed index-based tree computed per thread, and a host export is added to check that tree. Exclusive scans get a one-block path for small inputs and fold the scan of tile sums into the last tile-sums block via a ticket word. Tile packing now runs one wave per segment with LDS staging, and iota buffers are dropped in favour of null values to sort_pairs. The changes target launch count and setup latency, but they rely on a ticket word that resets correctly and on the fixed-order final sum staying bit-identical to the old tree.

Result: faster. 979.2 million pairs/s, median of 6 (+1.3%).

```diff
diff --git a/include/seekmer_hip.h b/include/seekmer_hip.h
--- a/include/seekmer_hip.h
+++ b/include/seekmer_hip.h
@@ -202,6 +202,7 @@
 int skm_quant_components(skm_quant *quant, int64_t info[8], int32_t *tx_label, int32_t *tx_tile,
                          int32_t *class_tile);
 int skm_quant_timing(skm_quant *quant, double timing[4]);
+int skm_np_sum_tree(int64_t block_len, int64_t cap_nodes, int32_t *lo, int32_t *n, int32_t *depth);
 
 typedef struct skm_comm skm_comm;
 int skm_comm_unique_id(void *id128);
diff --git a/seekmer_amd/_native.py b/seekmer_amd/_native.py
--- a/seekmer_amd/_native.py
+++ b/seekmer_amd/_native.py
@@ -145,6 +145,7 @@
                                                c_i64, c_i64p, c_f64p, c_f64p, c_i64p]),
     'skm_quant_timing': (ctypes.c_int, [ctypes.c_void_p, c_f64p]),
     'skm_quant_components': (ctypes.c_int, [ctypes.c_void_p, c_i64p, c_i32p, c_i32p, c_i32p]),
+    'skm_np_sum_tree': (ctypes.c_int, [c_i64, c_i64, c_i32p, c_i32p, c_i32p]),
     'skm_comm_unique_id': (ctypes.c_int, [ctypes.c_void_p]),
     'skm_comm_create': (ctypes.c_int, [ctypes.c_int, ctypes.c_void_p, ctypes.c_int, ctypes.c_int,
                                        c_void_pp]),
diff --git a/seekmer_amd/csrc/skm_abi.hip b/seekmer_amd/csrc/skm_abi.hip
--- a/seekmer_amd/csrc/skm_abi.hip
+++ b/seekmer_amd/csrc/skm_abi.hip
@@ -2959,8 +2959,8 @@
     SKM_TRY(q->ctl.ensure(16));
     SKM_TRY(q->part_max.ensure(EM_FINAL_BLOCKS));
     SKM_TRY(q->part_flags.ensure(EM_FINAL_BLOCKS));
-    SKM_TRY(q->arrivals.ensure(T));
-    HIP_TRY(hipMemsetAsync(q->arrivals.p, 0, T * sizeof(unsigned int), q->stream));
+    SKM_TRY(q->arrivals.ensure(T + 1));
+    HIP_TRY(hipMemsetAsync(q->arrivals.p, 0, (T + 1) * sizeof(unsigned int), q->stream));
     if (em_tiles_possible(several_ranks)) {
         auto &t = q->tiles;
         SKM_TRY(t.tile_tx.ensure(T + 2)); SKM_TRY(t.tile_cls.ensure(T + 2));
@@ -2973,9 +2973,12 @@
     return SKM_OK;
 }
 
+unsigned int *quant_ticket(skm_quant *q) { return q->arrivals.p + std::max<int64_t>(q->n_tx, 1); }
+
 QuantBuild quant_build_view(skm_quant *q)
 {
     QuantBuild b{};
+    b.ticket = quant_ticket(q);
     b.n_tx = q->n_tx;
     b.n_classes = q->n_classes;
     b.n_ids = q->n_ids;
@@ -3303,6 +3306,19 @@
     return acc;
 }
 
+}
+
+extern "C" int skm_np_sum_tree(int64_t block_len, int64_t cap_nodes, int32_t *lo, int32_t *n, int32_t *depth)
+{
+    if (block_len < 1 || block_len > 8192 || !lo || !n || !depth) return fail(SKM_ERR_ARG, "bad argument");
+    if (cap_nodes < NP_TREE_NODES) return fail(SKM_ERR_ARG, "room for %d nodes is needed", NP_TREE_NODES);
+    lo[0] = n[0] = 0;
+    depth[0] = -1;
+    for (int i = 1; i < NP_TREE_NODES; ++i) {
+        const NpTreeNode node = np_tree_node((int)block_len, i);
+        lo[i] = node.lo; n[i] = node.n; depth[i] = node.depth;
+    }
+    return SKM_OK;
 }
 
 extern "C" int skm_quant_create(int device, int64_t n_tx, int64_t n_classes,
@@ -3418,7 +3434,7 @@
         return SKM_OK;
     }
     launch_reciprocal(q->eff_len.p, n_tx, q->x0.p, q->stream);
-    launch_np_sum(q->x0.p, n_tx, 1.0, sums.p, total, q->stream);
+    launch_np_sum(q->x0.p, n_tx, 1.0, sums.p, total, q->stream, quant_ticket(q.get()));
     launch_divide(q->x0.p, n_tx, total, false, 0.0, q->stream);
     lap("start vector");
     SKM_TRY(quant_finish_setup(q.get(), &m->t, m->first_seen_bound));
@@ -3431,9 +3447,9 @@
     m->t_em_ns += q->t_em_ns;
     m->em_iters += (double)it;
     double *const x = (it & 1) ? q->x1.p : q->x0.p;
-    launch_np_sum(x, n_tx, 1000000.0, sums.p, total, q->stream);
+    launch_np_sum(x, n_tx, 1000000.0, sums.p, total, q->stream, quant_ticket(q.get()));
     launch_divide(x, n_tx, total + 1, true, 0.001, q->stream);
-    launch_np_sum(x, n_tx, 1000000.0, sums.p, total, q->stream);
+    launch_np_sum(x, n_tx, 1000000.0, sums.p, total, q->stream, quant_ticket(q.get()));
     launch_divide(x, n_tx, total + 1, false, 0.0, q->stream);
     HIP_TRY(hipGetLastError());
     if (tpm) HIP_TRY(hipMemcpyAsync(tpm, x, n_tx * 8, hipMemcpyDeviceToHost, q->stream));
diff --git a/seekmer_amd/csrc/skm_em.hip b/seekmer_amd/csrc/skm_em.hip
--- a/seekmer_amd/csrc/skm_em.hip
+++ b/seekmer_amd/csrc/skm_em.hip
@@ -629,8 +629,6 @@
         hipLaunchKernelGGL(em_finalize_kernel<false>, dim3((unsigned)blocks), dim3(256), 0, stream, p, parity);
 }
 
-constexpr int NP_MAX_LEAVES = 160;
-
 __device__ __forceinline__ double np_leaf_sum(const double *a, int n)
 {
     if (n < 8) {
@@ -647,38 +645,6 @@
     for (; i < n; ++i) res += a[i];
     return res;
 }
-
-template <int LEVELS>
-__device__ __attribute__((noinline)) void np_list_leaves(int lo, int n, int *leaf_lo, int *leaf_n, int *count)
-{
-    if (n <= 128) {
-        if (*count < NP_MAX_LEAVES) { leaf_lo[*count] = lo; leaf_n[*count] = n; }
-        ++*count;
-        return;
-    }
-    int n2 = n / 2;
-    n2 -= n2 % 8;
-    np_list_leaves<LEVELS - 1>(lo, n2, leaf_lo, leaf_n, count);
-    np_list_leaves<LEVELS - 1>(lo + n2, n - n2, leaf_lo, leaf_n, count);
-}
-template <>
-__device__ __attribute__((noinline)) void np_list_leaves<0>(int, int, int *, int *, int *count)
-{
-    *count = NP_MAX_LEAVES + 1;
-}
-
-template <int LEVELS>
-__device__ __attribute__((noinline)) double np_combine(int n, const double *leaf_sum, int *next)
-{
-    if (n <= 128) return leaf_sum[(*next)++];
-    int n2 = n / 2;
-    n2 -= n2 % 8;
-    const double left = np_combine<LEVELS - 1>(n2, leaf_sum, next);
-    const double right = np_combine<LEVELS - 1>(n - n2, leaf_sum, next);
-    return left + right;
-}
-template <>
-__device__ __attribute__((noinline)) double np_combine<0>(int, const double *, int *) { return 0.0; }
 
 __device__ __forceinline__ void np_sum_full_block(const double *__restrict__ a, double *__restrict__ out)
 {
@@ -701,40 +667,52 @@
 }
 
 __global__ void __launch_bounds__(512)
-np_sum_blocks_kernel(const double *__restrict__ a, int64_t n, double *__restrict__ block_sums, int64_t stride)
+np_sum_blocks_kernel(const double *__restrict__ a, int64_t n, double *block_sums, int64_t stride,
+                     unsigned int *ticket, double divisor, double *out)
 {
     a += blockIdx.y * stride;
     block_sums += blockIdx.y * (int64_t)gridDim.x;
     const int64_t first = blockIdx.x * (int64_t)8192;
     const int len = (int)min((int64_t)8192, n - first);
+    __shared__ double staged[8192];
+    __shared__ double node_sum[NP_TREE_NODES];
+    __shared__ bool s_last;
     if (len == 8192) {
         np_sum_full_block(a + first, block_sums + blockIdx.x);
-        return;
-    }
-    __shared__ double staged[8192];
-    __shared__ int leaf_lo[NP_MAX_LEAVES], leaf_n[NP_MAX_LEAVES], n_leaves;
-    __shared__ double leaf_sum[NP_MAX_LEAVES];
-    for (int i = threadIdx.x; i < len; i += blockDim.x) staged[i] = a[first + i];
+    } else {
+        for (int i = threadIdx.x; i < len; i += blockDim.x) staged[i] = a[first + i];
+        const int me = threadIdx.x;
+        NpTreeNode node{0, 0, -1};
+        if (me >= 1 && me < NP_TREE_NODES) node = np_tree_node(len, me);
+        const bool leaf = node.depth >= 0 && (node.n <= 128 || node.depth == NP_TREE_DEPTH);
+        __syncthreads();
+        if (leaf) node_sum[me] = np_leaf_sum(staged + node.lo, node.n);
+        __syncthreads();
+        for (int d = NP_TREE_DEPTH - 1; d >= 0; --d) {
+            if (node.depth == d && !leaf) node_sum[me] = node_sum[2 * me] + node_sum[2 * me + 1];
+            __syncthreads();
+        }
+        if (threadIdx.x == 0) block_sums[blockIdx.x] = node_sum[1];
+    }
+    if (!ticket) return;
     if (threadIdx.x == 0) {
-        int count = 0;
-        np_list_leaves<8>(0, len, leaf_lo, leaf_n, &count);
-        n_leaves = count;
+        __threadfence();
+        s_last = atomicInc(ticket, gridDim.x - 1) == gridDim.x - 1;
     }
     __syncthreads();
-    if (n_leaves > NP_MAX_LEAVES) {
-        if (threadIdx.x == 0) {
-            double r = 0.0;
-            for (int i = 0; i < len; ++i) r += staged[i];
-            block_sums[blockIdx.x] = r;
-        }
-        return;
-    }
-    if ((int)threadIdx.x < n_leaves)
-        leaf_sum[threadIdx.x] = np_leaf_sum(staged + leaf_lo[threadIdx.x], leaf_n[threadIdx.x]);
-    __syncthreads();
+    if (!s_last) return;
+    __threadfence();
+    double acc = 0.0;
+    for (int64_t b0 = 0; b0 < (int64_t)gridDim.x; b0 += NP_TREE_NODES) {
+        const int here = (int)min((int64_t)NP_TREE_NODES, (int64_t)gridDim.x - b0);
+        if ((int)threadIdx.x < here) node_sum[threadIdx.x] = block_sums[b0 + threadIdx.x];
+        __syncthreads();
+        if (threadIdx.x == 0) for (int k = 0; k < here; ++k) acc += node_sum[k];
+        __syncthreads();
+    }
     if (threadIdx.x == 0) {
-        int next = 0;
-        block_sums[blockIdx.x] = np_combine<8>(len, leaf_sum, &next);
+        out[0] = acc;
+        out[1] = acc / divisor;
     }
 }
 
@@ -771,13 +749,14 @@
 }
 
 void launch_np_sum(const double *a, int64_t n, double divisor, double *block_sums, double *out,
-                   hipStream_t stream)
+                   hipStream_t stream, unsigned int *ticket)
 {
     const int64_t n_blocks = (n + 8191) / 8192;
     if (n_blocks)
         hipLaunchKernelGGL(np_sum_blocks_kernel, dim3((unsigned)n_blocks), dim3(512), 0, stream,
-                           a, n, block_sums, (int64_t)0);
-    hipLaunchKernelGGL(np_sum_final_kernel, dim3(1), dim3(1), 0, stream, block_sums, n_blocks, divisor, out);
+                           a, n, block_sums, (int64_t)0, ticket, divisor, out);
+    if (!n_blocks || !ticket)
+        hipLaunchKernelGGL(np_sum_final_kernel, dim3(1), dim3(1), 0, stream, block_sums, n_blocks, divisor, out);
 }
 
 void launch_np_sum_many(const double *a, int64_t n, int64_t count, int64_t stride, double divisor,
@@ -788,7 +767,8 @@
         const unsigned here = (unsigned)std::min<int64_t>(32768, count - v0);
         if (n_blocks)
             hipLaunchKernelGGL(np_sum_blocks_kernel, dim3((unsigned)n_blocks, here), dim3(512), 0, stream,
-                               a + v0 * stride, n, block_sums + v0 * n_blocks, stride);
+                               a + v0 * stride, n, block_sums + v0 * n_blocks, stride, (unsigned int *)nullptr, divisor,
+                               (double *)nullptr);
         hipLaunchKernelGGL(np_sum_final_kernel, dim3(here), dim3(1), 0, stream, block_sums + v0 * n_blocks, n_blocks,
                            divisor, out + 2 * v0);
     }
diff --git a/seekmer_amd/csrc/skm_kernels.h b/seekmer_amd/csrc/skm_kernels.h
--- a/seekmer_amd/csrc/skm_kernels.h
+++ b/seekmer_amd/csrc/skm_kernels.h
@@ -308,6 +308,7 @@
     uint16_t *tile_cls_tx, *tile_tx_cls;
     int32_t *tx_label, *tx_tile, *cls_tile;
     int64_t tile_info[2];
+    unsigned int *ticket;
 };
 int64_t quant_setup(const ClassTable *table, QuantBuild &q, int32_t *perm, hipStream_t stream);
 struct QuantResidual {
@@ -328,7 +329,27 @@
 int64_t quant_rows_upper_bound(int64_t n_tx, int64_t n_ids);
 
 void launch_np_sum(const double *a, int64_t n, double divisor, double *block_sums, double *out,
-                   hipStream_t stream);
+                   hipStream_t stream, unsigned int *ticket = nullptr);
+
+constexpr int NP_TREE_DEPTH = 7, NP_TREE_NODES = 1 << (NP_TREE_DEPTH + 1);
+struct NpTreeNode { int lo, n, depth; };
+#if defined(__HIPCC__)
+__host__ __device__
+#endif
+inline NpTreeNode np_tree_node(int len, int i)
+{
+    int depth = 0;
+    while ((i >> (depth + 1)) != 0) ++depth;
+    int lo = 0, n = len;
+    for (int d = depth - 1; d >= 0; --d) {
+        if (n <= 128) return NpTreeNode{0, 0, -1};
+        int n2 = n / 2;
+        n2 -= n2 % 8;
+        if ((i >> d) & 1) { lo += n2; n -= n2; }
+        else n = n2;
+    }
+    return NpTreeNode{lo, n, depth};
+}
 void launch_np_sum_many(const double *a, int64_t n, int64_t count, int64_t stride, double divisor,
                         double *block_sums, double *out, hipStream_t stream);
 void launch_reciprocal(const double *l, int64_t n, double *x, hipStream_t stream);
diff --git a/seekmer_amd/csrc/skm_quant_setup.hip b/seekmer_amd/csrc/skm_quant_setup.hip
--- a/seekmer_amd/csrc/skm_quant_setup.hip
+++ b/seekmer_amd/csrc/skm_quant_setup.hip
@@ -12,7 +12,14 @@
 struct Scratch {
     hipStream_t stream;
     std::vector<void *> held;
-    explicit Scratch(hipStream_t s) : stream(s) {}
+    unsigned int *ticket;
+    explicit Scratch(hipStream_t s, unsigned int *zero_word = nullptr) : stream(s), ticket(zero_word) {}
+    unsigned int *ticket_word()
+    {
+        if (!ticket && (ticket = alloc<unsigned int>(1)) &&
+            hipMemsetAsync(ticket, 0, sizeof(unsigned int), stream) != hipSuccess) ticket = nullptr;
+        return ticket;
+    }
     template <class T>
     T *alloc(size_t n)
     {
@@ -243,12 +250,59 @@
 }
 
 constexpr int SCAN_TILE = 2048;
+constexpr int64_t SCAN_ONE_BLOCK_MAX = 4 * SCAN_TILE;
 
 template <class T>
-__global__ void __launch_bounds__(256)
-scan_tile_sums_kernel(const T *__restrict__ in, int64_t n, T *__restrict__ tile_sums)
+__device__ __forceinline__ T scan_one_tile(const T *in, int64_t n, int64_t first, T base, T *out, T *s_wave)
+{
+    const int64_t at0 = first + threadIdx.x * 8;
+    T v[8], sum = 0;
+#pragma unroll
+    for (int k = 0; k < 8; ++k) { v[k] = at0 + k < n ? in[at0 + k] : (T)0; sum += v[k]; }
+    T incl = sum;
+    const int lane = threadIdx.x & 63, wave = threadIdx.x >> 6;
+#pragma unroll
+    for (int d = 1; d < 64; d <<= 1) {
+        const T up = __shfl_up(incl, d, 64);
+        if (lane >= d) incl += up;
+    }
+    if (lane == 63) s_wave[wave] = incl;
+    __syncthreads();
+    T at = base + incl - sum;
+    for (int w = 0; w < wave; ++w) at += s_wave[w];
+    const T tile_sum = s_wave[0] + s_wave[1] + s_wave[2] + s_wave[3];
+#pragma unroll
+    for (int k = 0; k < 8; ++k) {
+        if (at0 + k < n) out[at0 + k] = at;
+        at += v[k];
+    }
+    __syncthreads();
+    return tile_sum;
+}
+
+template <class T>
+__device__ __forceinline__ T scan_by_one_block(const T *in, int64_t n, T *out, T *s_wave)
+{
+    T carry = 0;
+    for (int64_t first = 0; first < n; first += SCAN_TILE) carry += scan_one_tile(in, n, first, carry, out, s_wave);
+    return carry;
+}
+
+template <class T>
+__global__ void __launch_bounds__(256)
+scan_small_kernel(const T *in, int64_t n, T *out, T *total)
 {
     __shared__ T s_wave[4];
+    const T sum = scan_by_one_block(in, n, out, s_wave);
+    if (total && threadIdx.x == 0) *total = sum;
+}
+
+template <class T>
+__global__ void __launch_bounds__(256)
+scan_tile_sums_kernel(const T *__restrict__ in, int64_t n, T *tile_sums, T *total, unsigned int *ticket)
+{
+    __shared__ T s_wave[4];
+    __shared__ bool s_last;
     const int64_t base = blockIdx.x * (int64_t)SCAN_TILE + threadIdx.x * 8;
     T sum = 0;
 #pragma unroll
@@ -256,56 +310,24 @@
     for (int d = 32; d > 0; d >>= 1) sum += __shfl_xor(sum, d, 64);
     if ((threadIdx.x & 63) == 0) s_wave[threadIdx.x >> 6] = sum;
     __syncthreads();
-    if (threadIdx.x == 0) tile_sums[blockIdx.x] = s_wave[0] + s_wave[1] + s_wave[2] + s_wave[3];
+    if (threadIdx.x == 0) {
+        tile_sums[blockIdx.x] = s_wave[0] + s_wave[1] + s_wave[2] + s_wave[3];
+        __threadfence();
+        s_last = atomicInc(ticket, gridDim.x - 1) == gridDim.x - 1;
+    }
+    __syncthreads();
+    if (!s_last) return;
+    __threadfence();
+    const T all = scan_by_one_block(tile_sums, (int64_t)gridDim.x, tile_sums, s_wave);
+    if (total && threadIdx.x == 0) *total = all;
 }
 
 template <class T>
-__global__ void __launch_bounds__(1024)
-scan_of_sums_kernel(T *tile_sums, int64_t n_tiles, T *total)
-{
-    __shared__ T s_part[1024];
-    const int64_t per = (n_tiles + 1023) / 1024;
-    const int64_t first = threadIdx.x * per, last = min(n_tiles, first + per);
-    T sum = 0;
-    for (int64_t i = first; i < last; ++i) sum += tile_sums[i];
-    s_part[threadIdx.x] = sum;
-    __syncthreads();
-    for (int step = 1; step < 1024; step <<= 1) {
-        const T add = (int)threadIdx.x >= step ? s_part[threadIdx.x - step] : (T)0;
-        __syncthreads();
-        s_part[threadIdx.x] += add;
-        __syncthreads();
-    }
-    T at = s_part[threadIdx.x] - sum;
-    for (int64_t i = first; i < last; ++i) { const T v = tile_sums[i]; tile_sums[i] = at; at += v; }
-    if (total && threadIdx.x == 1023) *total = s_part[1023];
-}
-
-template <class T>
-__global__ void __launch_bounds__(256)
-scan_tiles_kernel(const T *__restrict__ in, int64_t n, const T *__restrict__ tile_base, T *__restrict__ out)
+__global__ void __launch_bounds__(256)
+scan_tiles_kernel(const T *in, int64_t n, const T *__restrict__ tile_base, T *out)
 {
     __shared__ T s_wave[4];
-    const int64_t base = blockIdx.x * (int64_t)SCAN_TILE + threadIdx.x * 8;
-    T v[8], sum = 0;
-#pragma unroll
-    for (int k = 0; k < 8; ++k) { v[k] = base + k < n ? in[base + k] : (T)0; sum += v[k]; }
-    T incl = sum;
-    const int lane = threadIdx.x & 63, wave = threadIdx.x >> 6;
-#pragma unroll
-    for (int d = 1; d < 64; d <<= 1) {
-        const T up = __shfl_up(incl, d, 64);
-        if (lane >= d) incl += up;
-    }
-    if (lane == 63) s_wave[wave] = incl;
-    __syncthreads();
-    T at = tile_base[blockIdx.x] + incl - sum;
-    for (int w = 0; w < wave; ++w) at += s_wave[w];
-#pragma unroll
-    for (int k = 0; k < 8; ++k) {
-        if (base + k < n) out[base + k] = at;
-        at += v[k];
-    }
+    scan_one_tile(in, n, blockIdx.x * (int64_t)SCAN_TILE, tile_base[blockIdx.x], out, s_wave);
 }
 
 template <class T>
@@ -316,10 +338,16 @@
         if (total) QB_TRY(hipMemsetAsync(total, 0, sizeof(T), stream));
         return 0;
     }
+    if (n <= SCAN_ONE_BLOCK_MAX) {
+        hipLaunchKernelGGL(scan_small_kernel<T>, dim3(1), dim3(256), 0, stream, in, n, out, total);
+        return 0;
+    }
     const int64_t n_tiles = (n + SCAN_TILE - 1) / SCAN_TILE;
     QB_ALLOC(tile_sums, T, n_tiles);
-    hipLaunchKernelGGL(scan_tile_sums_kernel<T>, dim3((unsigned)n_tiles), dim3(256), 0, stream, in, n, tile_sums);
-    hipLaunchKernelGGL(scan_of_sums_kernel<T>, dim3(1), dim3(1024), 0, stream, tile_sums, n_tiles, total);
+    unsigned int *ticket = scratch.ticket_word();
+    if (!ticket) { snprintf(g_setup_failure, sizeof(g_setup_failure), "no memory for the scan's ticket"); return -1; }
+    hipLaunchKernelGGL(scan_tile_sums_kernel<T>, dim3((unsigned)n_tiles), dim3(256), 0, stream, in, n, tile_sums, total,
+                       ticket);
     hipLaunchKernelGGL(scan_tiles_kernel<T>, dim3((unsigned)n_tiles), dim3(256), 0, stream, in, n, tile_sums, out);
     return 0;
 }
@@ -424,7 +452,7 @@
         const int64_t at = first + c * 64 + lane;
         const bool valid = at < n;
         key[c] = valid ? keys_in[at] : (K)0;
-        val[c] = valid ? vals_in[at] : 0;
+        val[c] = valid ? (vals_in ? vals_in[at] : (int32_t)at) : 0;
         digit[c] = (uint32_t)((unsigned long long)key[c] >> shift) & (RS_BINS - 1);
         if (valid) atomicAdd(&wave_base[wave][digit[c]], 1u);
     }
@@ -543,16 +571,15 @@
     QB_ALLOC(arena_off, int64_t, n_classes); QB_ALLOC(len, int64_t, n_classes);
     QB_ALLOC(len_sorted, int64_t, n_classes); QB_ALLOC(count, double, n_classes);
     QB_ALLOC(first, unsigned long long, n_classes); QB_ALLOC(first_sorted, unsigned long long, n_classes);
-    QB_ALLOC(iota, int32_t, n_classes); QB_ALLOC(perm, int32_t, n_classes);
+    QB_ALLOC(perm, int32_t, n_classes);
     hipLaunchKernelGGL(table_dump_kernel, dim3(blocks_for(n_classes)), dim3(256), 0, stream,
                        t, n_classes, arena_off, len, count, first, (uint32_t *)nullptr);
-    hipLaunchKernelGGL(iota_kernel, dim3(blocks_for(n_classes)), dim3(256), 0, stream, iota, n_classes);
     int first_bits = 64;
     if (q.first_seen_bound > 0) {
         first_bits = 1;
         while (first_bits < 63 && (1LL << first_bits) <= q.first_seen_bound) ++first_bits;
     }
-    if (sort_pairs(scratch, first, first_sorted, iota, perm, n_classes, first_bits)) return -1;
+    if (sort_pairs(scratch, first, first_sorted, (const int32_t *)nullptr, perm, n_classes, first_bits)) return -1;
     hipLaunchKernelGGL(gather_classes_kernel, dim3(blocks_for(n_classes)), dim3(256), 0, stream, perm,
                        n_classes, len, count, len_sorted, q.cls_count);
     if (exclusive_scan_with_total(scratch, len_sorted, q.cls_offset, n_classes)) return -1;
@@ -590,16 +617,15 @@
 
     QB_ALLOC(word_count, int64_t, n_words); QB_ALLOC(word_base, int64_t, n_words + 1);
     QB_ALLOC(by_rank, int32_t, C); QB_ALLOC(key_by_rank, uint32_t, C); QB_ALLOC(key_sorted, uint32_t, C);
-    QB_ALLOC(iota, int32_t, C); QB_ALLOC(len_sorted, int64_t, C); QB_ALLOC(src_off, int64_t, C);
+    QB_ALLOC(len_sorted, int64_t, C); QB_ALLOC(src_off, int64_t, C);
     hipLaunchKernelGGL(word_popcount_kernel, dim3(blocks_for(n_words)), dim3(256), 0, stream, bits, n_words,
                        word_count);
     if (exclusive_scan_with_total(scratch, word_count, word_base, n_words)) return -1;
     hipLaunchKernelGGL(first_seen_rank_kernel, dim3(blocks_for(C)), dim3(256), 0, stream, first, min_id, C, bound,
                        bits, word_base, by_rank, key_by_rank);
-    hipLaunchKernelGGL(iota_kernel, dim3(blocks_for(C)), dim3(256), 0, stream, iota, C);
     int end_bit = 1;
     while ((1LL << end_bit) < q.n_tx && end_bit < 32) ++end_bit;
-    if (sort_pairs(scratch, key_by_rank, key_sorted, iota, perm, C, end_bit)) return -1;
+    if (sort_pairs(scratch, key_by_rank, key_sorted, (const int32_t *)nullptr, perm, C, end_bit)) return -1;
     hipLaunchKernelGGL(gather_by_rank_kernel, dim3(blocks_for(C)), dim3(256), 0, stream, perm, by_rank, C, len,
                        count, arena_off, len_sorted, q.cls_count, src_off);
     if (exclusive_scan_with_total(scratch, len_sorted, q.cls_offset, C)) return -1;
@@ -614,15 +640,14 @@
     const int64_t C = q.n_classes, M = q.n_ids;
     if (C == 0) return 0;
     if (C >= (1LL << 31) || M >= (1LL << 31)) return -2;
-    QB_ALLOC(key, uint32_t, C); QB_ALLOC(key_sorted, uint32_t, C); QB_ALLOC(iota, int32_t, C);
+    QB_ALLOC(key, uint32_t, C); QB_ALLOC(key_sorted, uint32_t, C);
     QB_ALLOC(ids_copy, int32_t, M); QB_ALLOC(len, int64_t, C); QB_ALLOC(len_sorted, int64_t, C);
     QB_ALLOC(old_offset, int64_t, C + 1); QB_ALLOC(count_copy, double, C);
     hipLaunchKernelGGL(class_min_id_kernel, dim3(blocks_for(C)), dim3(256), 0, stream, q.cls_offset, q.ids, C,
                        key, len);
-    hipLaunchKernelGGL(iota_kernel, dim3(blocks_for(C)), dim3(256), 0, stream, iota, C);
     int end_bit = 1;
     while ((1LL << end_bit) < q.n_tx && end_bit < 32) ++end_bit;
-    if (sort_pairs(scratch, key, key_sorted, iota, perm, C, end_bit)) return -1;
+    if (sort_pairs(scratch, key, key_sorted, (const int32_t *)nullptr, perm, C, end_bit)) return -1;
     QB_TRY(hipMemcpyAsync(old_offset, q.cls_offset, (C + 1) * 8, hipMemcpyDeviceToDevice, stream));
     QB_TRY(hipMemcpyAsync(ids_copy, q.ids, M * 4, hipMemcpyDeviceToDevice, stream));
     QB_TRY(hipMemcpyAsync(count_copy, q.cls_count, C * 8, hipMemcpyDeviceToDevice, stream));
@@ -755,23 +780,24 @@
 tile_pack_kernel(const int32_t *__restrict__ comp, int64_t n_tx, int64_t n_segments, int32_t *__restrict__ root_tile,
                  int64_t *__restrict__ seg_tiles, unsigned long long *__restrict__ oversize)
 {
-    for (int64_t g = blockIdx.x * (int64_t)blockDim.x + threadIdx.x; g < n_segments;
-         g += (int64_t)gridDim.x * blockDim.x) {
-        int tx = 0, pairs = 0, classes = 0, n = 0;
-        const int64_t last = min(n_tx, (g + 1) * EM_TILE_SEGMENT);
-        for (int64_t t0 = g * EM_TILE_SEGMENT; t0 < last; t0 += 8) {
-            int size[24];
-#pragma unroll
-            for (int k = 0; k < 24; ++k) size[k] = 3 * t0 + k < 3 * n_tx ? comp[3 * t0 + k] : 0;
-#pragma unroll
-            for (int k = 0; k < 8; ++k) {
-                const int64_t t = t0 + k;
-                if (t >= last) break;
-                const int c_tx = size[3 * k], c_pairs = size[3 * k + 1], c_classes = size[3 * k + 2];
-                if (c_tx == 0) { root_tile[t] = -1; continue; }
+    __shared__ int s_size[4][3 * EM_TILE_SEGMENT];
+    __shared__ int s_tile[4][EM_TILE_SEGMENT];
+    const int lane = threadIdx.x & 63, wave = threadIdx.x >> 6;
+    for (int64_t g = blockIdx.x * (int64_t)4 + wave; g < n_segments; g += (int64_t)gridDim.x * 4) {
+        const int64_t first = g * EM_TILE_SEGMENT;
+        const int here = (int)min((int64_t)EM_TILE_SEGMENT, n_tx - first);
+        for (int i = lane; i < 3 * here; i += 64) s_size[wave][i] = comp[3 * first + i];
+        __builtin_amdgcn_fence(__ATOMIC_RELEASE, "wavefront");
+        __builtin_amdgcn_fence(__ATOMIC_ACQUIRE, "wavefront");
+        if (lane == 0) {
+            int tx = 0, pairs = 0, classes = 0, n = 0;
+            unsigned long long above = 0;
+            for (int k = 0; k < here; ++k) {
+                const int c_tx = s_size[wave][3 * k], c_pairs = s_size[wave][3 * k + 1], c_classes = s_size[wave][3 * k + 2];
+                if (c_tx == 0) { s_tile[wave][k] = -1; continue; }
                 if (c_tx > EM_TILE_TX || c_pairs > EM_TILE_PAIRS || c_classes > EM_TILE_CLASSES) {
-                    root_tile[t] = -2;
-                    atomicAdd(oversize, 1ULL);
+                    s_tile[wave][k] = -2;
+                    ++above;
                     continue;
                 }
                 if (n == 0 || tx + c_tx > EM_TILE_TX || pairs + c_pairs > EM_TILE_PAIRS ||
@@ -780,10 +806,16 @@
                     tx = pairs = classes = 0;
                 }
                 tx += c_tx; pairs += c_pairs; classes += c_classes;
-                root_tile[t] = n - 1;
+                s_tile[wave][k] = n - 1;
             }
-        }
-        seg_tiles[g] = n;
+            seg_tiles[g] = n;
+            if (above) atomicAdd(oversize, above);
+        }
+        __builtin_amdgcn_fence(__ATOMIC_RELEASE, "wavefront");
+        __builtin_amdgcn_fence(__ATOMIC_ACQUIRE, "wavefront");
+        for (int k = lane; k < here; k += 64) root_tile[first + k] = s_tile[wave][k];
+        __builtin_amdgcn_fence(__ATOMIC_RELEASE, "wavefront");
+        __builtin_amdgcn_fence(__ATOMIC_ACQUIRE, "wavefront");
     }
 }
 
@@ -894,7 +926,7 @@
     QB_ALLOC(parent, int32_t, T); QB_ALLOC(comp, int32_t, 3 * T); QB_ALLOC(root_tile, int32_t, T);
     QB_ALLOC(seg_tiles, int64_t, n_segments); QB_ALLOC(seg_base, int64_t, n_segments + 1);
     QB_ALLOC(oversize, unsigned long long, 1);
-    QB_ALLOC(iota, int32_t, std::max(T, C)); QB_ALLOC(sorted_tile, int32_t, std::max(T, C));
+    QB_ALLOC(sorted_tile, int32_t, std::max(T, C));
     QB_ALLOC(tx_local, int32_t, T); QB_ALLOC(cls_local, int32_t, C);
     QB_ALLOC(len, int64_t, std::max(T, C));
     QB_TRY(hipMemsetAsync(comp, 0, 3 * T * sizeof(int32_t), stream));
@@ -905,7 +937,7 @@
                        q.tx_label, comp);
     hipLaunchKernelGGL(cc_classes_kernel, dim3(blocks_for(C)), dim3(256), 0, stream, q.cls_offset, q.ids, C,
                        q.tx_label, comp);
-    hipLaunchKernelGGL(tile_pack_kernel, dim3(blocks_for(n_segments)), dim3(256), 0, stream, comp, T, n_segments,
+    hipLaunchKernelGGL(tile_pack_kernel, dim3(blocks_for(64 * n_segments)), dim3(256), 0, stream, comp, T, n_segments,
                        root_tile, seg_tiles, oversize);
     if (exclusive_scan_with_total(scratch, seg_tiles, seg_base, n_segments)) return -1;
     int end_bit = 1;
@@ -914,8 +946,7 @@
     QB_ALLOC(tx_key, int32_t, T);
     hipLaunchKernelGGL(tx_tile_kernel, dim3(blocks_for(T)), dim3(256), 0, stream, q.tx_label, root_tile, seg_base, T,
                        q.tx_row, q.row_start, degree_bits, q.tx_tile, tx_key);
-    hipLaunchKernelGGL(iota_kernel, dim3(blocks_for(std::max(T, C))), dim3(256), 0, stream, iota, std::max(T, C));
-    if (sort_pairs(scratch, tx_key, sorted_tile, iota, q.tx_list, T, end_bit + degree_bits)) return -1;
+    if (sort_pairs(scratch, tx_key, sorted_tile, (const int32_t *)nullptr, q.tx_list, T, end_bit + degree_bits)) return -1;
     hipLaunchKernelGGL(tile_starts_kernel, dim3(blocks_for(T + 1)), dim3(256), 0, stream, sorted_tile, degree_bits, T,
                        seg_base + n_segments, q.tile_tx);
     hipLaunchKernelGGL(tile_local_tx_kernel, dim3(blocks_for(T)), dim3(256), 0, stream, q.tx_list, sorted_tile, degree_bits,
@@ -925,7 +956,7 @@
     QB_ALLOC(cls_key, int32_t, C);
     hipLaunchKernelGGL(cls_tile_kernel, dim3(blocks_for(C)), dim3(256), 0, stream, q.cls_offset, q.ids, C, q.tx_tile,
                        length_bits, q.cls_tile, cls_key);
-    if (sort_pairs(scratch, cls_key, sorted_tile, iota, q.cls_list, C, end_bit + length_bits)) return -1;
+    if (sort_pairs(scratch, cls_key, sorted_tile, (const int32_t *)nullptr, q.cls_list, C, end_bit + length_bits)) return -1;
     hipLaunchKernelGGL(tile_starts_kernel, dim3(blocks_for(C + 1)), dim3(256), 0, stream, sorted_tile, length_bits, C,
                        seg_base + n_segments, q.tile_cls);
     hipLaunchKernelGGL(tile_local_cls_kernel, dim3(blocks_for(C)), dim3(256), 0, stream, q.cls_list, sorted_tile, length_bits,
@@ -948,7 +979,7 @@
     for (int attempt = can_rank ? 0 : 1; attempt < 2; ++attempt) {
         int64_t n_rows = -1;
         {
-            Scratch scratch(stream);
+            Scratch scratch(stream, q.ticket);
             if (attempt == 0) {
                 const int rc = build_from_table_ranked(scratch, *table, q, perm);
                 if (rc == 1) continue;
@@ -1042,7 +1073,7 @@
 
 int quant_residual_count(const QuantBuild &q, int64_t counts[3], hipStream_t stream)
 {
-    Scratch scratch(stream);
+    Scratch scratch(stream, q.ticket);
     QB_ALLOC(sums, unsigned long long, 3);
     QB_TRY(hipMemsetAsync(sums, 0, 3 * sizeof(unsigned long long), stream));
     hipLaunchKernelGGL(residual_count_kernel, dim3(blocks_for(std::max(q.n_classes, q.n_tx))), dim3(256), 0, stream,
@@ -1055,7 +1086,7 @@
 
 int quant_residual_build(const QuantBuild &q, QuantResidual &r, hipStream_t stream)
 {
-    Scratch scratch(stream);
+    Scratch scratch(stream, q.ticket);
     const int64_t C = q.n_classes, T = q.n_tx;
     QB_ALLOC(keep, int64_t, C); QB_ALLOC(rank, int64_t, C + 1);
     QB_ALLOC(len, int64_t, std::max(C, T)); QB_ALLOC(new_offset, int64_t, C + 1);
```
